# HiKapok/DAN

Hardware: AMD Instinct MI355X
Metric: 640x640 images/sec/node (train fwd+bwd) (higher is better)
Workload: dtype bf16; 1 GPU; S3FD VGG-16 backbone + 6 detection heads, 640x640 bf16 training (fwd+bwd+SGD), batch 16 per GPU; global_batch=16, parallelism=dp1, anchors_per_image=34125, step_launch=eager, rccl_ranks=1, weight_gradient_stream=True

## Files before the change

### dan_amd/_lib.py

```python
import ctypes
import os

import torch

_HERE = os.path.dirname(os.path.abspath(__file__))
ACT_NAME = os.environ.get("DANHIP_DTYPE", "bf16").lower()
if ACT_NAME not in ("bf16", "fp16"):
    raise ValueError("DANHIP_DTYPE must be bf16 or fp16, got %r" % ACT_NAME)
ACT_DTYPE = torch.float16 if ACT_NAME == "fp16" else torch.bfloat16
SO_PATH = os.path.join(_HERE, "libdanhip_f16.so" if ACT_NAME == "fp16" else "libdanhip.so")
if os.environ.get("DANHIP_LIB_PATH"):
    SO_PATH = os.path.abspath(os.environ["DANHIP_LIB_PATH"])

F32, BF16 = 0, 1
SPLIT3 = 3


class ConvDesc(ctypes.Structure):
    _fields_ = [(n, ctypes.c_int32) for n in ("N", "H", "W", "Cin", "Ho", "Wo", "Cout", "kh", "kw", "stride")]


class ConvPitch(ctypes.Structure):
    _fields_ = [(n, ctypes.c_int32) for n in ("x_pitch", "y_pitch", "aux_pitch")]


class PackEntry(ctypes.Structure):
    _fields_ = [("w_hwio", ctypes.c_void_p), ("wf_packed", ctypes.c_void_p), ("wb_packed", ctypes.c_void_p)] + \
               [(n, ctypes.c_int32) for n in ("kh", "kw", "cin", "cin_real", "cout", "rows_f", "cols_f", "rows_b", "cols_b", "co8", "first_block", "pad_")]


class JpegInfo(ctypes.Structure):
    _fields_ = [(n, ctypes.c_int32) for n in ("width", "height", "ncomp", "mode", "reason", "reserved")] + [("coef_count", ctypes.c_int64)]


class JpegDesc(ctypes.Structure):
    _fields_ = [(n, ctypes.c_int32) for n in ("width", "height", "ncomp", "mode")] + \
               [(n, ctypes.c_int32 * 3) for n in ("blocks_w", "blocks_h", "comp_w", "comp_h", "quant_index")] + \
               [(n, ctypes.c_int32) for n in ("status", "idct_groups", "rgb_groups")] + [("reserved", ctypes.c_int32 * 2)] + \
               [("coef_offset", ctypes.c_int64), ("coef_count", ctypes.c_int64), ("plane_offset", ctypes.c_int64 * 3),
                ("out_offset", ctypes.c_int64), ("quant", (ctypes.c_uint16 * 64) * 4)]


P = ctypes.c_void_p
I32 = ctypes.c_int32
I64 = ctypes.c_int64
FL = ctypes.c_float
DESC = ctypes.POINTER(ConvDesc)

SIGNATURES = {
    "danhip_conv_packed_dims": [DESC, ctypes.c_int, ctypes.POINTER(I64), ctypes.POINTER(I64)],
    "danhip_pack_conv_weight": [DESC, P, I32, P, P, P],
    "danhip_conv2d_fwd_pool": [DESC, P, P, P, P, P, P],
    "danhip_pack_entry_init": [ctypes.POINTER(PackEntry), DESC, P, I32, P, P, I32, ctypes.POINTER(ctypes.c_int32)],
    "danhip_pack_conv_weights_batched": [P, I32, I32, P],
    "danhip_conv2d_fwd": [DESC, P, P, P, P, ctypes.c_int, ctypes.c_int, P, P],
    "danhip_conv2d_fwd_ws": [DESC, P, P, P, P, ctypes.c_int, ctypes.c_int, P, P, ctypes.c_size_t, P],
    "danhip_conv2d_fwd_f32": [DESC, P, P, P, P, ctypes.c_int, P, P],
    "danhip_maxpool2x2_fwd_f32": [P, P, I32, I32, I32, I32, P],
    "danhip_split_set_range_flag": [P],
    "danhip_split3_f32": [P, P, I64, I32, I32, ctypes.c_int, I32, P],
    "danhip_unsplit3_f32": [P, P, I64, I32, I32, P],
    "danhip_unsplit3_scaled_f32": [P, P, I64, I32, I32, I32, P],
    "danhip_maxpool2x2_split3": [P, P, I32, I32, I32, I32, P],
    "danhip_l2norm_split3": [P, P, P, I64, I32, I32, I32, P],
    "danhip_conv3x3_c3_f32_split3": [P, P, P, P, I32, I32, I32, I32, ctypes.c_int, I32, P],
    "danhip_conv2d_fwd_split": [DESC, P, P, P, P, ctypes.c_int, ctypes.c_int, I32, P, ctypes.c_size_t, P],
    "danhip_l2norm_fwd_f32": [P, P, P, I64, I32, P],
    "danhip_resize_bilinear_add_fwd_f32": [P, P, P, I32, I32, I32, I32, I32, I32, P],
    "danhip_avgpool2x2s1_same_fwd_f32": [P, P, I32, I32, I32, I32, P],
    "danhip_deform_sample_fwd_f32": [P, P, P, I32, I32, I32, I32, I32, I32, I32, I32, I32, P],
    "danhip_conv2d_bwd_data": [DESC, P, P, P, P, ctypes.c_int, P],
    "danhip_conv2d_bwd_data_ws": [DESC, P, P, P, P, ctypes.c_int, P, ctypes.c_size_t, P],
    "danhip_conv2d_bwd_data_bits": [DESC, P, P, P, P, ctypes.c_int, P],
    "danhip_conv2d_bwd_data_bits_first": [DESC, P, P, P, P, I32, P, P, P],
    "danhip_relu_bits": [P, P, I64, I32, P],
    "danhip_conv2d_fwd_relu_bits": [DESC, P, P, P, P, P, P, P, P],
    "danhip_conv2d_bwd_weight": [DESC, P, P, P, P, I32, P],
    "danhip_conv2d_bwd_weight_ws": [DESC, P, P, P, P, I32, P, ctypes.c_size_t, P],
    "danhip_avgpool2x2s1_same_fwd_strided": [P, I32, P, I32, I32, I32, I32, I32, ctypes.c_int, P],
    "danhip_avgpool2x2s1_same_bwd_strided": [P, I32, P, I32, I32, I32, I32, I32, P],
    "danhip_add16": [P, P, P, I64, P],
    "danhip_residual_bwd": [P, P, P, P, P, ctypes.c_int, I64, P],
    "danhip_conv2d_fwd_strided": [DESC, P, P, P, P, ctypes.c_int, I32, ctypes.POINTER(ConvPitch), P, ctypes.c_size_t, P],
    "danhip_conv2d_bwd_data_strided": [DESC, P, P, P, P, ctypes.c_int, ctypes.POINTER(ConvPitch), P, ctypes.c_size_t, P],
    "danhip_conv2d_fwd_concat2": [DESC, P, P, I32, I32, P, P, P, ctypes.c_int, P],
    "danhip_conv2d_bwd_weight_strided": [DESC, P, P, P, P, I32, ctypes.POINTER(ConvPitch), P, ctypes.c_size_t, P],
    "danhip_relu_bwd_bias_grad": [P, P, P, I64, I32, P],
    "danhip_maxpool2x2_fwd": [P, P, I32, I32, I32, I32, P],
    "danhip_maxpool2x2_fwd_arg": [P, P, P, I32, I32, I32, I32, P],
    "danhip_maxpool2x2_bwd_arg": [P, P, P, I32, I32, I32, I32, ctypes.c_int, P],
    "danhip_conv2d_fwd_pool_arg": [DESC, P, P, P, P, P, P, P],
    "danhip_conv2d_fwd_relu_bits_arg": [DESC, P, P, P, P, P, P, P, P, P],
    "danhip_maxpool2x2_bwd": [P, P, P, I32, I32, I32, I32, ctypes.c_int, P],
    "danhip_l2norm_fwd": [P, P, P, I64, I32, P],
    "danhip_l2norm_bwd": [P, P, P, P, P, I64, I32, ctypes.c_int, ctypes.c_int, P],
    "danhip_l2norm_bwd_pool_scatter": [P, P, P, P, P, P, P, I32, I32, I32, I32, ctypes.c_int, ctypes.c_int, ctypes.c_int, P],
    "danhip_preprocess_u8": [P, P, I64, P],
    "danhip_resize_bilinear_add_fwd": [P, P, P, I32, I32, I32, I32, I32, I32, P],
    "danhip_resize_bilinear_add_bwd": [P, P, I32, I32, I32, I32, I32, I32, ctypes.c_int, P],
    "danhip_avgpool2x2s1_same_fwd": [P, P, I32, I32, I32, I32, P],
    "danhip_avgpool2x2s1_same_bwd": [P, P, P, I32, I32, I32, I32, ctypes.c_int, P],
    "danhip_slice_deliver": [P, I32, I32, I32, P, I32, P, I32, ctypes.c_int, I64, P],
    "danhip_batchnorm_fwd_train": [P, P, P, P, P, P, P, P, I64, I32, FL, FL, ctypes.c_int, P, P],
    "danhip_batchnorm_fwd_infer": [P, P, P, P, P, P, I64, I32, ctypes.c_int, P],
    "danhip_batchnorm_bwd": [P, P, P, P, P, P, P, P, I64, I32, P],
    "danhip_dynamic_anchor_routing_eval": [P, P, P, P, I64, I32, I32, I32, I32, I32, P, P, P, ctypes.c_size_t, P],
    "danhip_dynamic_anchor_routing_train": [P, P, P, P, I64, I32, I32, I32, I32, I32, FL, FL, ctypes.c_uint64, ctypes.c_uint64, P, P, P, P,
                                            ctypes.c_size_t, P],
    "danhip_nms": [P, I32, I32, I32, FL, P, P, P],
    "danhip_argsort_desc_f32": [P, I64, I32, P, P, ctypes.c_size_t, P],
    "danhip_augment_preprocess": [P, I32, I32, I32, ctypes.POINTER(ctypes.c_int32), ctypes.POINTER(ctypes.c_float), I32, I32, I32, I32, I32, P, I32, I32,
                                  P, ctypes.c_size_t, P],
    "danhip_deform_psroi_pool_fwd": [P, P, P, P, P, I32, I32, I32, I32, I32, I32, I32, I32, I32, FL, FL, I32, I32, P],
    "danhip_deform_psroi_pool_bwd": [P, P, P, P, P, P, P, I32, I32, I32, I32, I32, I32, I32, I32, I32, I32, FL, FL, I32, I32, P],
    "danhip_maxpool3x3s2_same_fwd": [P, P, I32, I32, I32, I32, P],
    "danhip_maxpool3x3s2_same_bwd": [P, P, P, I32, I32, I32, I32, P],
    "danhip_resize_u8_linear": [P, I32, I32, P, I32, I32, I32, ctypes.c_double, ctypes.c_double, P],
    "danhip_bbox_vote": [P, P, I32, I32, ctypes.c_double, I32, P, P, P, ctypes.c_size_t, P],
    "danhip_wider_quantize": [P, ctypes.c_int, P, P, I32, I32, I32, P, P, I32, I32, P, P],
    "danhip_wider_score_range": [P, I64, P, P, ctypes.c_size_t, P],
    "danhip_wider_eval": [P, P, I64, P, P, P, I64, P, I32, I32, I32, I32, ctypes.c_double, P, ctypes.c_size_t, P, P],
    "danhip_wider_ap": [P, ctypes.c_size_t, P, I64, I32, I32, I32, P, P, P, P, P, P],
    "danhip_deform_sample_fwd": [P, P, P, I32, I32, I32, I32, I32, I32, I32, I32, I32, P],
    "danhip_deform_sample_bwd": [P, P, P, P, P, I32, I32, I32, I32, I32, I32, I32, I32, I32, ctypes.c_int, P, ctypes.c_size_t, P],
    "danhip_deform_conv_fwd": [P, P, P, P, P, I32, I32, I32, I32, I32, I32, I32, I32, I32, I32, ctypes.c_int, P, ctypes.c_size_t, P],
    "danhip_deform_conv_bwd": [P, P, P, P, P, P, P, P, I32, I32, I32, I32, I32, I32, I32, I32, I32, I32, ctypes.c_int, P, ctypes.c_size_t, P],
    "danhip_deform_conv_bwd_with_col": [P, P, P, P, P, P, P, P, P, I32, I32, I32, I32, I32, I32, I32, I32, I32, I32, ctypes.c_int, P, ctypes.c_size_t, P],
    "danhip_deform_conv_bwd_deliver": [P, P, P, P, P, P, P, P, P, I32, I32, I32, I32, I32, I32, I32, I32, I32, I32, ctypes.c_int, ctypes.c_int, P, ctypes.c_size_t, P],
    "danhip_cast_pad_f32_to_bf16": [P, P, P, I64, I32, I32, P],
    "danhip_head_split_fwd": [P, P, P, I32, I32, I32, I32, I32, I32, I32, P],
    "danhip_head_split_bwd": [P, P, P, P, I32, I32, I32, I32, I32, I32, I32, P],
    "danhip_hard_neg_select": [P, P, P, P, P, P, I32, I32, FL, ctypes.c_int, P],
    "danhip_detection_loss_fwd": [P, P, P, P, P, P, P, P, I32, I32, P],
    "danhip_detection_loss_bwd": [P, P, P, P, P, P, P, FL, FL, I32, I32, P],
    "danhip_sgd_momentum_flat": [P, P, P, P, P, P, I32, I64, FL, FL, FL, P, P],
    "danhip_sgd_momentum_flat_dynamic": [P, P, P, P, P, P, I32, I64, FL, FL, P, P, P],
    "danhip_anchors_generate": [P, P, P, P, P, P, I32, I32, I32, FL, FL, FL, I32, P],
    "danhip_iou_matrix": [P, P, P, P, P, P, P, I32, I32, P],
    "danhip_dual_max_match": [P, I32, I32, FL, FL, ctypes.c_int, P, P, P, ctypes.c_size_t, P],
    "danhip_small_mining_match": [P, I32, I32, FL, FL, FL, I32, FL, P, P, P, ctypes.c_size_t, P],
    "danhip_encode_anchors": [P, P, P, P, P, P, P, P, P, I32, FL, FL, FL, FL, FL, P],
    "danhip_decode_anchors": [P, P, P, P, P, P, I32, I32, FL, FL, FL, FL, P],
    "danhip_face_scores": [P, P, P, FL, I64, P],
    "danhip_comm_load": [ctypes.c_char_p],
    "danhip_comm_rccl_version": [ctypes.POINTER(ctypes.c_int)],
    "danhip_comm_unique_id": [P],
    "danhip_comm_create": [P, I32, I32, I32, ctypes.POINTER(ctypes.c_void_p)],
    "danhip_comm_destroy": [P],
    "danhip_comm_info": [P, ctypes.POINTER(I32), ctypes.POINTER(I32), ctypes.POINTER(I32)],
    "danhip_comm_async_error": [P, ctypes.POINTER(I32)],
    "danhip_comm_abort": [P],
    "danhip_comm_allreduce_sum": [P, P, I64, ctypes.c_int, P],
    "danhip_comm_reduce_scatter_sum": [P, P, P, I64, ctypes.c_int, P],
    "danhip_comm_allgather": [P, P, P, I64, ctypes.c_int, P],
    "danhip_jpeg_entropy_decode_batch": [P, P, I32, I32, P, I64, P, P],
    "danhip_jpeg_entropy_decode_batch_ex": [P, P, I32, I32, ctypes.c_uint32, P, I64, P, P],
    "danhip_jpeg_scan_prepare_batch_ex": [P, P, I32, ctypes.c_uint32, P, ctypes.c_size_t, I64, P, P],
    "danhip_jpeg_reconstruct_batch": [P, I64, P, P, I32, P, I64, P, ctypes.c_size_t, P, P],
    "danhip_jpeg_scan_prepare_batch": [P, P, I32, P, ctypes.c_size_t, I64, P, P],
    "danhip_jpeg_huffman_decode_batch": [P, P, ctypes.c_size_t, I32, P, I64, P, P, P, ctypes.c_size_t, P, P, P],
    "danhip_jpeg_entropy_emulate_batch": [P, ctypes.c_size_t, I32, P, P, I64, I32, P, P],
    "danhip_encode_anchors_batched": [P] * 11 + [I32, I32, I32, I32, I32, FL, FL, FL, I32, FL, FL, FL, FL, FL, FL, P, P, P, P, P,
                                                 ctypes.c_size_t, P],
}

_lib = None


class DanhipError(RuntimeError):
    pass


def lib():
    global _lib
    if _lib is None:
        _lib = _load(SO_PATH, ACT_NAME)
    return _lib


_lib_f16 = None


def lib_f16():
    global _lib_f16
    if _lib_f16 is None:
        _lib_f16 = lib() if ACT_NAME == "fp16" else _load(os.path.join(_HERE, "libdanhip_f16.so"), "fp16")
    return _lib_f16


def call_f16(name, *args):
    L = lib_f16()
    rc = getattr(L, name)(*args)
    if rc != 0:
        raise DanhipError("%s (fp16 build) failed (%d): %s" % (name, rc, L.danhip_last_error().decode()))


def _load(so_path, act_name):
    if True:
        if not os.path.exists(so_path):
            raise DanhipError("libdanhip.so not found at %s — run `python -m dan_amd.build` (there is no fallback path)" % so_path)
        L = ctypes.CDLL(so_path)
        L.danhip_last_error.restype = ctypes.c_char_p
        L.danhip_last_error.argtypes = []
        L.danhip_version.restype = ctypes.c_int
        L.danhip_act_dtype.restype = ctypes.c_int
        if L.danhip_act_dtype() != (2 if act_name == "fp16" else 1):
            raise DanhipError("%s was built for another activation dtype than %s" % (so_path, act_name))
        L.danhip_match_workspace_bytes.restype = ctypes.c_size_t
        L.danhip_conv_kernel_label.restype = ctypes.c_char_p
        L.danhip_conv_kernel_label.argtypes = [DESC, ctypes.c_int]
        L.danhip_conv_wgrad_kernel_label.restype = ctypes.c_char_p
        L.danhip_conv_wgrad_kernel_label.argtypes = [DESC]
        L.danhip_conv_last_launch_label.restype = ctypes.c_char_p
        L.danhip_conv_last_launch_label.argtypes = []
        L.danhip_match_workspace_bytes.argtypes = [I32, I32]
        L.danhip_encode_anchors_batched_workspace_bytes.restype = ctypes.c_size_t
        L.danhip_encode_anchors_batched_workspace_bytes.argtypes = [I32, I32, I32]
        L.danhip_routing_workspace_bytes.restype = ctypes.c_size_t
        L.danhip_routing_workspace_bytes.argtypes = [I64, I32, ctypes.c_int]
        L.danhip_bbox_vote_workspace_bytes.restype = ctypes.c_size_t
        L.danhip_augment_workspace_bytes.restype = ctypes.c_size_t
        L.danhip_argsort_workspace_bytes.argtypes = [I64]
        L.danhip_argsort_workspace_bytes.restype = ctypes.c_size_t
        L.danhip_augment_workspace_bytes.argtypes = []
        L.danhip_set_option.restype = ctypes.c_int
        L.danhip_set_option.argtypes = [ctypes.c_char_p, ctypes.c_int]
        L.danhip_get_option.restype = ctypes.c_int
        L.danhip_get_option.argtypes = [ctypes.c_char_p]
        L.danhip_conv2d_workspace_bytes.restype = ctypes.c_size_t
        L.danhip_conv2d_workspace_bytes.argtypes = [DESC, ctypes.c_int]
        L.danhip_conv2d_bwd_weight_workspace_bytes.restype = ctypes.c_size_t
        L.danhip_conv2d_bwd_weight_workspace_bytes.argtypes = [DESC]
        L.danhip_deform_conv_workspace_bytes.restype = ctypes.c_size_t
        L.danhip_deform_conv_workspace_bytes.argtypes = [I32, I32, I32, I32, I32, I32, I32, ctypes.c_int]
        L.danhip_deform_sample_bwd_workspace_bytes.restype = ctypes.c_size_t
        L.danhip_deform_sample_bwd_workspace_bytes.argtypes = [I32, I32, I32, I32]
        L.danhip_conv2d_fwd_pool_only.restype = ctypes.c_int
        L.danhip_conv2d_fwd_pool_only.argtypes = [DESC]
        L.danhip_conv2d_fwd_concat2_supported.restype = ctypes.c_int
        L.danhip_conv2d_fwd_concat2_supported.argtypes = [DESC, I32, I32]
        L.danhip_conv2d_fwd_emits_bits.restype = ctypes.c_int
        L.danhip_conv2d_fwd_emits_bits.argtypes = [DESC, ctypes.c_int]
        L.danhip_conv2d_bwd_data_takes_bits.restype = ctypes.c_int
        L.danhip_conv2d_bwd_data_takes_bits.argtypes = [DESC]
        L.danhip_conv2d_bwd_data_first_supported.restype = ctypes.c_int
        L.danhip_conv2d_bwd_data_first_supported.argtypes = [DESC]
        L.danhip_deform_conv_fused.restype = ctypes.c_int
        L.danhip_deform_conv_fused.argtypes = [I32] * 9
        L.danhip_bbox_vote_workspace_bytes.argtypes = [I32, I32]
        L.danhip_wider_score_range_workspace_bytes.restype = ctypes.c_size_t
        L.danhip_wider_score_range_workspace_bytes.argtypes = []
        L.danhip_wider_eval_workspace_bytes.restype = ctypes.c_size_t
        L.danhip_wider_eval_workspace_bytes.argtypes = [I32, I32, I32]
        L.danhip_jpeg_inspect.restype = ctypes.c_int
        L.danhip_jpeg_inspect.argtypes = [P, I64, ctypes.POINTER(JpegInfo)]
        L.danhip_jpeg_inspect_ex.restype = ctypes.c_int
        L.danhip_jpeg_inspect_ex.argtypes = [P, I64, ctypes.c_uint32, ctypes.POINTER(JpegInfo)]
        L.danhip_jpeg_workspace_bytes.restype = ctypes.c_size_t
        L.danhip_jpeg_workspace_bytes.argtypes = [P, I32]
        L.danhip_jpeg_output_bytes.restype = I64
        L.danhip_jpeg_output_bytes.argtypes = [P, I32]
        L.danhip_jpeg_scan_staging_bytes.restype = ctypes.c_size_t
        L.danhip_jpeg_scan_staging_bytes.argtypes = [P, P, I32]
        L.danhip_jpeg_scan_device_bytes.restype = ctypes.c_size_t
        L.danhip_jpeg_scan_device_bytes.argtypes = [P]
        L.danhip_jpeg_scan_workspace_bytes.restype = ctypes.c_size_t
        L.danhip_jpeg_scan_workspace_bytes.argtypes = [P]
        for name, args in SIGNATURES.items():
            fn = getattr(L, name)
            fn.restype = ctypes.c_int
            fn.argtypes = args
    return L


def check(rc, what):
    if rc != 0:
        raise DanhipError("%s failed (%d): %s" % (what, rc, lib().danhip_last_error().decode()))


def ptr(t):
    if t is None:
        return None
    assert t.is_contiguous(), "danhip needs contiguous tensors"
    return ctypes.c_void_p(t.data_ptr())


def stream():
    return ctypes.c_void_p(torch.cuda.current_stream().cuda_stream)


def call(name, *args):
    check(getattr(lib(), name)(*args), name)
```

### dan_amd/csrc/conv_common.h

```cpp
#pragma once
#include "common.h"

struct ConvArgs {
  const bf16_t* x;
  const bf16_t* w;
  const float* bias;
  const bf16_t* mask;
  const unsigned char* mask_bits;
  const bf16_t* resid;
  void* y;
  unsigned char* bits_out;
  unsigned char* pool_bits_out;
  bf16_t* pool_y;
  unsigned char* pool_arg_out;
  int N, H, W, C;
  int Ho, Wo, Co;
  int kh, kw, stride, pad_t, pad_l;
  int M, Kpad, ktiles, taps, cpt;
  FastDiv div_wo, div_howo, div_c, div_kw;
  int relu, out_f32, accumulate;
  int dshift;
  float* splitk_ws;
  int splits, kt_per_split;
  int dstride;
  int ldx, ldy, ldm;
  int relu_co;
  bool strided() const { return ldx != C || ldy != Co || (mask && ldm != Co) || (relu && relu_co < Co); }
  const bf16_t* x2;
  int ksplit;
  int split_out;
  const bf16_t* fuse_x8;
  float* fuse_dw;
  float* fuse_db;
  int fuse_cin_real;
  int acc_exp;
  int* range_flag;
};

__device__ __forceinline__ float dh_acc_scale(const ConvArgs& a) { return __builtin_bit_cast(float, (a.acc_exp + 127) << 23); }

template <int N>
__device__ __forceinline__ void dh_range_check(const float* v, int* flag) {
  float m = fabsf(v[0]);
#pragma unroll
  for (int r = 1; r < N; ++r) m = fmaxf(m, fabsf(v[r]));
  if (!(m < 65520.f) && flag) *flag = 1;
}

__device__ __forceinline__ void dh_split4(const float v[4], uint2& hi, uint2& lo) {
  hi.x = pack2bf(v[0], v[1]);
  hi.y = pack2bf(v[2], v[3]);
  float h[4];
  unpack2bf(hi.x, h[0], h[1]);
  unpack2bf(hi.y, h[2], h[3]);
  lo.x = pack2bf(v[0] - h[0], v[1] - h[1]);
  lo.y = pack2bf(v[2] - h[2], v[3] - h[3]);
}

int* danhip_split_range_flag();

typedef __attribute__((ext_vector_type(2))) short s16x2;
__device__ __forceinline__ unsigned pkmax_relu(unsigned a, unsigned b) {
  return __builtin_bit_cast(unsigned, __builtin_elementwise_max(__builtin_bit_cast(s16x2, a), __builtin_bit_cast(s16x2, b)));
}

__device__ __forceinline__ float dh_relu(float v) {
  float r;
  asm("v_max_f32 %0, 0, %1" : "=v"(r) : "v"(v));
  return r;
}
typedef __attribute__((ext_vector_type(2))) unsigned short dh_u16x2;
typedef __attribute__((ext_vector_type(2))) unsigned dh_u32x2;
typedef __attribute__((ext_vector_type(4))) unsigned dh_u32x4;
__device__ __forceinline__ dh_u16x2 dh_pos2(unsigned packed) {
  unsigned r;
  asm("v_pk_min_u16 %0, %1, %2" : "=v"(r) : "v"(packed), "s"(0x00010001u));
  return __builtin_bit_cast(dh_u16x2, r);
}
template <int SHIFT>
__device__ __forceinline__ unsigned dh_pos_bits8_acc(const dh_u32x4& t, unsigned bits) {
  static_assert(SHIFT == 0 || SHIFT == 8, "16-bit weights");
#pragma unroll
  for (int e = 0; e < 4; ++e)
    bits = __builtin_amdgcn_udot2(dh_pos2(t[e]), dh_u16x2{(unsigned short)(1u << (SHIFT + 2 * e)), (unsigned short)(2u << (SHIFT + 2 * e))}, bits, false);
  return bits;
}
__device__ __forceinline__ unsigned dh_pk_ne(unsigned m, unsigned x) {
  unsigned d, r;
  asm("v_pk_sub_u16 %0, %1, %2" : "=v"(d) : "v"(m), "v"(x));
  asm("v_pk_min_u16 %0, %1, %2" : "=v"(r) : "v"(d), "s"(0x00010001u));
  return r;
}
__device__ __forceinline__ unsigned dh_argmax2x2_pk(unsigned a, unsigned b, unsigned c, unsigned m) {
  const unsigned na = dh_pk_ne(m, a), nb = dh_pk_ne(m, b), nc = dh_pk_ne(m, c);
  unsigned t, r;
  asm("v_pk_mad_u16 %0, %1, %2, %1" : "=v"(t) : "v"(nb), "v"(nc));
  asm("v_pk_mad_u16 %0, %1, %2, %1" : "=v"(r) : "v"(na), "v"(t));
  return r;
}
__device__ __forceinline__ unsigned dh_argmax2x2_codes16(const dh_u32x4& a, const dh_u32x4& b, const dh_u32x4& c, const dh_u32x4& m) {
  unsigned out = 0;
#pragma unroll
  for (int e = 0; e < 4; ++e) {
    const unsigned w = dh_argmax2x2_pk(a[e], b[e], c[e], m[e]);
    out |= ((w | (w >> 14)) & 0xFu) << (4 * e);
  }
  return out;
}

__device__ __forceinline__ unsigned dh_or_rows(unsigned x) {
  const dh_u32x2 a = __builtin_amdgcn_permlane16_swap(x, x, false, false);
  const unsigned y = a[0] | a[1];
  const dh_u32x2 b = __builtin_amdgcn_permlane32_swap(y, y, false, false);
  return b[0] | b[1];
}
__device__ __forceinline__ unsigned dh_lane_xor1(unsigned v) { return (unsigned)__builtin_amdgcn_mov_dpp((int)v, 0xB1, 0xF, 0xF, true); }

struct ConvInstance {
  const char* label = nullptr;
  int (*launch)(const ConvArgs&, hipStream_t) = nullptr;
  bool fuses_pool = false;
  bool skips_y = false;
  bool emits_bits = false;
  bool takes_bits = false;
  bool folds_first = false;
  explicit operator bool() const { return launch != nullptr; }
};
ConvInstance conv_c8_select(const ConvArgs& a);
ConvInstance conv_c64_select(const ConvArgs& a);
ConvInstance conv_halo_select(const ConvArgs& a);
ConvInstance conv_pointwise_select(const ConvArgs& a);

struct WgradCall {
  const danhip_conv_desc* d;
  const bf16_t* x;
  const bf16_t* dy;
  float* dw;
  float* db;
  int cin_real, ldx, ldy;
  void* ws;
  size_t ws_bytes;
};
struct WgradInstance {
  const char* label = nullptr;
  int (*launch)(const WgradCall&, hipStream_t) = nullptr;
  explicit operator bool() const { return launch != nullptr; }
};
WgradInstance wgrad_rows_select(const WgradCall& c);
WgradInstance wgrad_pw_select(const WgradCall& c);
WgradInstance wgrad_c8_select(const WgradCall& c);
size_t wgrad_rows_workspace_bytes(const danhip_conv_desc* d);
size_t wgrad_pw_workspace_bytes(const danhip_conv_desc* d);

inline const char*& dh_last_launch_label() {
  static thread_local const char* label = "";
  return label;
}
template <class Instance, class Args>
int dh_run_instance(const Instance& inst, const Args& a, hipStream_t s) {
  if (!inst) return 1;
  dh_last_launch_label() = inst.label;
  return inst.launch(a, s);
}

__device__ __forceinline__ void conv_store4(const ConvArgs& a, float v[4], size_t m, int co) {
  if (co >= a.Co) return;
  const size_t o = m * (size_t)(a.split_out ? 3 * a.ldy : a.ldy) + co;
  const size_t om = m * (size_t)a.ldm + co;
  const size_t orr = m * (size_t)a.Co + co;
  const bool full = (co + 4 <= a.Co) && ((a.Co & 3) == 0);
  if (a.bias) {
    const float sc = dh_acc_scale(a);
#pragma unroll
    for (int r = 0; r < 4; ++r) if (co + r < a.Co) v[r] = fmaf(v[r], sc, a.bias[co + r]);
  } else if (a.acc_exp) {
#pragma unroll
    for (int r = 0; r < 4; ++r) v[r] *= dh_acc_scale(a);
  }
  if (a.relu && co < a.relu_co) {
#pragma unroll
    for (int r = 0; r < 4; ++r) v[r] = fmaxf(v[r], 0.f);
  }
  if (a.out_f32) {
    float* y = reinterpret_cast<float*>(a.y) + o;
    if (full) {
      float4 t = make_float4(v[0], v[1], v[2], v[3]);
      if (a.accumulate) { float4 u = *reinterpret_cast<float4*>(y); t.x += u.x; t.y += u.y; t.z += u.z; t.w += u.w; }
      *reinterpret_cast<float4*>(y) = t;
    } else {
#pragma unroll
      for (int r = 0; r < 4; ++r) if (co + r < a.Co) y[r] = a.accumulate ? y[r] + v[r] : v[r];
    }
  } else {
    bf16_t* y = reinterpret_cast<bf16_t*>(a.y) + o;
    if (a.split_out) {
      dh_range_check<4>(v, a.range_flag);
      uint2 hi, lo;
      dh_split4(v, hi, lo);
      *reinterpret_cast<uint2*>(y) = hi;
      *reinterpret_cast<uint2*>(y + a.Co) = lo;
      *reinterpret_cast<uint2*>(y + 2 * a.Co) = hi;
      return;
    }
    if (full) {
      if (a.mask) {
        const uint2 mk = *reinterpret_cast<const uint2*>(a.mask + om);
        const bf16_t* mp = reinterpret_cast<const bf16_t*>(&mk);
#pragma unroll
        for (int r = 0; r < 4; ++r) if (!(bf2f(mp[r]) > 0.f)) v[r] = 0.f;
      }
      if (a.resid) {
        const uint2 rs = *reinterpret_cast<const uint2*>(a.resid + orr);
        const bf16_t* rp = reinterpret_cast<const bf16_t*>(&rs);
#pragma unroll
        for (int r = 0; r < 4; ++r) v[r] += bf2f(rp[r]);
      }
      if (a.accumulate) {
        const uint2 old = *reinterpret_cast<const uint2*>(y);
        const bf16_t* op = reinterpret_cast<const bf16_t*>(&old);
#pragma unroll
        for (int r = 0; r < 4; ++r) v[r] += bf2f(op[r]);
      }
      uint2 t;
      t.x = pack2bf(v[0], v[1]);
// ... 17 lines not shown
```

### dan_amd/csrc/conv_halo_c64.hip

```cpp
#include <type_traits>

#include "conv_common.h"

namespace {

struct C64Geom {
  int tiles_x, tiles_y, sp_items;
  FastDiv div_tx, div_txy;
};

template <int N>
__device__ __forceinline__ void c64_wait_vmcnt() {
  asm volatile("s_waitcnt vmcnt(%0)" ::"n"(N) : "memory");
}

template <bool DGRAD, bool FUSE8 = false>
__global__ __launch_bounds__(512, 2) __attribute__((amdgpu_waves_per_eu(2, 2))) void conv3x3_c64_kernel(const ConvArgs a, const C64Geom g) {
  static_assert(DGRAD || !FUSE8, "the folded first-layer weight gradient belongs to the data gradient");
  constexpr int TH = 8, TW = 32, PW = TW + 2;
  constexpr int PROWS = (TH + 2) * PW, PPIECES = (PROWS + 7) / 8, PBYTES = PPIECES * 1024, PL = (PPIECES + 7) / 8;
  constexpr int NPT = 4, NCT = 2;
  extern __shared__ __attribute__((aligned(16))) char smem[];

  const int tid = threadIdx.x, lane = tid & 63;
  const int wave = __builtin_amdgcn_readfirstlane(tid >> 6);
  const int wm = wave >> 1, wn = wave & 1;
  const int frow = lane & 15, fq = lane >> 4;
  const int G = gridDim.x;

  bf16x8 wr[9][2][NCT];
#pragma unroll
  for (int t = 0; t < 9; ++t)
#pragma unroll
    for (int ks = 0; ks < 2; ++ks)
#pragma unroll
      for (int ct = 0; ct < NCT; ++ct)
        wr[t][ks][ct] = *reinterpret_cast<const bf16x8*>(a.w + (size_t)(wn * 32 + (frow >> 2) * 8 + ct * 4 + (frow & 3)) * a.Kpad + t * 64 + ks * 32 + fq * 8);

  auto sp_coords = [&](int sp, int& n, int& y0, int& x0) __attribute__((always_inline)) {
    n = (int)fdiv((unsigned)sp, g.div_txy);
    const int rem = sp - n * (g.tiles_x * g.tiles_y);
    const int ty = (int)fdiv((unsigned)rem, g.div_tx);
    y0 = ty * TH;
    x0 = (rem - ty * g.tiles_x) * TW;
  };

  const unsigned npix1 = (unsigned)(a.N * a.H * a.W) - 1u;
  const unsigned px_x = (unsigned)a.ldx * 2u, px_y = (unsigned)a.ldy * 2u, px_m = (unsigned)a.ldm * 2u;
  const __amdgpu_buffer_rsrc_t rsrc_x = __builtin_amdgcn_make_buffer_rsrc(const_cast<bf16_t*>(a.x), 0, (int)(npix1 * px_x + 128u), 0x00020000);
  auto issue_patch = [&](int sp, int buf) __attribute__((always_inline)) {
    int n, y0, x0;
    sp_coords(sp, n, y0, x0);
    int ln = lane;
    asm volatile("" : "+v"(ln));
#pragma unroll
    for (int k = 0; k < PL; ++k) {
      int piece = k * 8 + wave;
      if (piece > PPIECES - 1) piece = PPIECES - 1;
      const int row = piece * 8 + (ln >> 3);
      const int hy = row / PW, hx = row - hy * PW;
      const int y = y0 - 1 + hy, x = x0 - 1 + hx;
      const bool ok = row < PROWS && (unsigned)y < (unsigned)a.H && (unsigned)x < (unsigned)a.W;
      const unsigned off = ok ? (unsigned)((n * a.H + y) * a.W + x) * px_x + (unsigned)(((ln & 7) ^ (hx & 7)) << 4) : 0xFFFFFFFFu;
      __builtin_amdgcn_raw_ptr_buffer_load_lds(rsrc_x, (LDS_AS void*)(smem + buf * PBYTES + piece * 1024), 16, off, 0, 0, 0);
    }
  };

  constexpr int RWBASE = 2 * PBYTES;
  [[maybe_unused]] const __amdgpu_buffer_rsrc_t rsrc_m =
      __builtin_amdgcn_make_buffer_rsrc(const_cast<bf16_t*>(a.mask ? a.mask : a.x), 0, (int)(npix1 * (a.mask ? px_m : px_x) + 128u), 0x00020000);
  [[maybe_unused]] const __amdgpu_buffer_rsrc_t rsrc_o =
      __builtin_amdgcn_make_buffer_rsrc(reinterpret_cast<bf16_t*>(a.y), 0, (int)(npix1 * px_y + 128u), 0x00020000);
  [[maybe_unused]] const __amdgpu_buffer_rsrc_t rsrc_b = __builtin_amdgcn_make_buffer_rsrc(
      const_cast<unsigned char*>(a.mask_bits ? a.mask_bits : reinterpret_cast<const unsigned char*>(a.x)), 0, (int)((unsigned)(a.N * a.H * a.W) * 8u),
      0x00020000);
  auto issue_bits = [&](int sp, int bbuf) __attribute__((always_inline)) {
    if (wave >= 2) return;
    int n, y0, x0;
    sp_coords(sp, n, y0, x0);
    int ln = lane;
    if constexpr (FUSE8) asm volatile("" : "+v"(ln));
    const int t = (wave * 64 + ln) * 2;
    const int y = y0 + t / TW, x = x0 + t % TW;
    const unsigned off = (y < a.H && x < a.W) ? (unsigned)((n * a.H + y) * a.W + x) * 8u : 0xFFFFFFFFu;
    __builtin_amdgcn_raw_ptr_buffer_load_lds(rsrc_b, (LDS_AS void*)(smem + RWBASE + bbuf * 2048 + wave * 1024), 16, off, 0, 0, 0);
  };
  constexpr int IMGBASE = RWBASE + 4096, IMGBYTES = 6144, DXBASE = RWBASE + 16384, C1BASE = RWBASE + 49152, FACCBASE = RWBASE + 49216;
  [[maybe_unused]] const __amdgpu_buffer_rsrc_t rsrc_i = __builtin_amdgcn_make_buffer_rsrc(
      const_cast<bf16_t*>(FUSE8 ? a.fuse_x8 : a.x), 0, (int)((unsigned)(a.N * a.H * a.W) * 16u), 0x00020000);
  [[maybe_unused]] auto issue_img = [&](int sp, int ibuf) __attribute__((always_inline)) {
    if (wave >= 6) return;
    int n, y0, x0;
    sp_coords(sp, n, y0, x0);
    int ln = lane;
    asm volatile("" : "+v"(ln));
    const int e = wave * 64 + ln;
    const int r = e / PW, c = e - r * PW;
    const int y = y0 - 1 + r, x = x0 - 1 + c;
    const bool ok = e < PROWS && (unsigned)y < (unsigned)a.H && (unsigned)x < (unsigned)a.W;
    __builtin_amdgcn_raw_ptr_buffer_load_lds(rsrc_i, (LDS_AS void*)(smem + IMGBASE + ibuf * IMGBYTES + wave * 1024), 16,
                                             ok ? (unsigned)((n * a.H + y) * a.W + x) * 16u : 0xFFFFFFFFu, 0, 0, 0);
  };
  auto issue_rw = [&](int sp) __attribute__((always_inline)) {
    int n, y0, x0;
    sp_coords(sp, n, y0, x0);
    int ln = lane;
    asm volatile("" : "+v"(ln));
#pragma unroll
    for (int k = 0; k < NPT; ++k) {
      const int t = wm * 64 + k * 16 + (ln >> 2);
      const int y = y0 + t / TW, x = x0 + t % TW;
      const bool ok = y < a.H && x < a.W;
      const unsigned pix = (unsigned)((n * a.H + y) * a.W + x), ch = (unsigned)((wn * 4 + (ln & 3)) << 4);
      if (a.mask)
        __builtin_amdgcn_raw_ptr_buffer_load_lds(rsrc_m, (LDS_AS void*)(smem + RWBASE + wave * 4096 + k * 1024), 16, ok ? pix * px_m + ch : 0xFFFFFFFFu, 0, 0, 0);
      if (a.accumulate)
        __builtin_amdgcn_raw_ptr_buffer_load_lds(rsrc_o, (LDS_AS void*)(smem + RWBASE + 32768 + wave * 4096 + k * 1024), 16, ok ? pix * px_y + ch : 0xFFFFFFFFu,
                                                 0, 0, 0);
    }
  };
  const int rwaddr = RWBASE + wave * 4096 + ((frow * 4 + fq) << 4);

  int pxaddr[3][NPT];
#pragma unroll
  for (int p = 0; p < NPT; ++p) {
    const int t = wm * 64 + p * 16 + frow;
    const int ty = t / TW, tx = t % TW;
#pragma unroll
    for (int j = 0; j < 3; ++j) pxaddr[j][p] = (ty * PW + tx + j) * 128 + ((fq ^ ((tx + j) & 7)) << 4);
  }

  f32x4 acc[NCT][NPT];
#pragma unroll
  for (int c = 0; c < NCT; ++c)
#pragma unroll
    for (int p = 0; p < NPT; ++p) acc[c][p] = f32x4{0.f, 0.f, 0.f, 0.f};

  [[maybe_unused]] const int faddr = FACCBASE + (wave * 3 * 64 + lane) * 16;
  if constexpr (FUSE8) {
#pragma unroll
    for (int mt = 0; mt < 3; ++mt) *reinterpret_cast<f32x4*>(smem + faddr + mt * 1024) = f32x4{0.f, 0.f, 0.f, 0.f};
    if (tid < 16) reinterpret_cast<bf16_t*>(smem + C1BASE)[tid] = tid == 0 ? f2bf(1.0f) : (bf16_t)0;
  }

  bf16x8 xa[NPT], xb[NPT], xc[NPT];
  auto read_px = [&](bf16x8 (&x)[NPT], auto tapc, int ks) __attribute__((always_inline)) {
    constexpr int TAP = decltype(tapc)::value;
    constexpr int TI = TAP / 3, TJ = TAP % 3;
#pragma unroll
    for (int p = 0; p < NPT; ++p) x[p] = *reinterpret_cast<const bf16x8*>(smem + (ks ? (pxaddr[TJ][p] ^ 64) : pxaddr[TJ][p]) + TI * PW * 128);
  };
  auto mma = [&](const bf16x8 (&w)[NCT], const bf16x8 (&x)[NPT]) __attribute__((always_inline)) {
#pragma unroll
    for (int c = 0; c < NCT; ++c)
#pragma unroll
      for (int p = 0; p < NPT; ++p) acc[c][p] = DH_MFMA_16x16x32(w[c], x[p], acc[c][p]);
  };

  const bool xcd_walk = (G & 7) == 0;
  const int GS = xcd_walk ? (G >> 3) : G;
  const int per_xcd = (g.sp_items + 7) >> 3;
  const int xbase = xcd_walk ? (int)(blockIdx.x & 7u) * per_xcd : 0;
  const int xend = xcd_walk ? (xbase + per_xcd < g.sp_items ? xbase + per_xcd : g.sp_items) : g.sp_items;
  int sp = xcd_walk ? xbase + (int)(blockIdx.x >> 3) : (int)blockIdx.x;
  if (sp >= xend) return;
  issue_patch(sp, 0);
  if constexpr (!DGRAD) {
    if (tid < 64) reinterpret_cast<float*>(smem + RWBASE)[tid] = a.bias ? a.bias[tid] : 0.f;
    __builtin_amdgcn_s_waitcnt(0xC07F);
  }
  c64_wait_vmcnt<0>();
  __builtin_amdgcn_s_barrier();
  int buf = 0;
  for (;;) {
    const int nsp = sp + GS;
    const bool has_next = nsp < xend;
    if constexpr (DGRAD) {
      issue_rw(sp);
      if (a.mask_bits) issue_bits(sp, buf);
      if constexpr (FUSE8) issue_img(sp, buf);
    }
    if (has_next) issue_patch(nsp, buf ^ 1);
    auto rd = [&](bf16x8 (&x)[NPT], auto hc) __attribute__((always_inline)) {
      constexpr int H = decltype(hc)::value;
      read_px(x, std::integral_constant<int, H / 2>{}, H & 1);
    };
    auto half = [&](auto hc, bf16x8 (&cur)[NPT], bf16x8 (&)[NPT]) __attribute__((always_inline)) {
      constexpr int H = decltype(hc)::value;
      mma(wr[H / 2][H & 1], cur);
      if constexpr (H + 3 < 18) rd(cur, std::integral_constant<int, H + 3>{});
    };
    rd(xa, std::integral_constant<int, 0>{});
    rd(xb, std::integral_constant<int, 1>{});
    rd(xc, std::integral_constant<int, 2>{});
#define C64_H(H, X) half(std::integral_constant<int, H>{}, X, X)
    C64_H(0, xa); C64_H(1, xb); C64_H(2, xc); C64_H(3, xa); C64_H(4, xb); C64_H(5, xc);
    C64_H(6, xa); C64_H(7, xb); C64_H(8, xc); C64_H(9, xa); C64_H(10, xb); C64_H(11, xc);
    C64_H(12, xa); C64_H(13, xb); C64_H(14, xc); C64_H(15, xa); C64_H(16, xb); C64_H(17, xc);
#undef C64_H
    c64_wait_vmcnt<0>();
    __builtin_amdgcn_s_barrier();
    {
      int n, y0, x0;
      sp_coords(sp, n, y0, x0);
      static_assert(NCT == 2, "epilogue packs the two channel tiles of a lane into one 16-byte vector");
      const int cbase = wn * 32 + fq * 8;
      float bv[8];
#pragma unroll
      for (int r = 0; r < 8; ++r) bv[r] = DGRAD ? 0.f : reinterpret_cast<const float*>(smem + RWBASE)[cbase + r];
      typedef __attribute__((ext_vector_type(4))) unsigned u32x4;
      u32x4 pk[NPT];
#pragma unroll
      for (int p = 0; p < NPT; ++p) pk[p] = u32x4{0u, 0u, 0u, 0u};
      if constexpr (DGRAD) {
        if (a.mask_bits) {
          unsigned w4[NPT];
#pragma unroll
          for (int p = 0; p < NPT; ++p) w4[p] = *reinterpret_cast<const unsigned*>(smem + RWBASE + buf * 2048 + (wm * 64 + p * 16 + frow) * 8 + wn * 4);
#pragma unroll
          for (int p = 0; p < NPT; ++p) {
            const int byte = (int)(w4[p] >> (8 * fq));
#pragma unroll
            for (int r = 0; r < 8; ++r) {
              const float v = acc[r >> 2][p][r & 3];
              acc[r >> 2][p][r & 3] = __builtin_bit_cast(float, __builtin_bit_cast(int, v) & __builtin_amdgcn_sbfe(byte, r, 1));
            }
          }
        }
        if (a.mask) {
          uint4 m[NPT];
#pragma unroll
          for (int p = 0; p < NPT; ++p) m[p] = *reinterpret_cast<const uint4*>(smem + rwaddr + p * 1024);
#pragma unroll
          for (int p = 0; p < NPT; ++p) {
            const bf16_t* mp = reinterpret_cast<const bf16_t*>(&m[p]);
#pragma unroll
            for (int r = 0; r < 8; ++r) if (!(bf2f(mp[r]) > 0.f)) acc[r >> 2][p][r & 3] = 0.f;
          }
        }
        if (a.accumulate) {
          uint4 o[NPT];
#pragma unroll
          for (int p = 0; p < NPT; ++p) o[p] = *reinterpret_cast<const uint4*>(smem + rwaddr + 32768 + p * 1024);
#pragma unroll
          for (int p = 0; p < NPT; ++p) {
            const bf16_t* op = reinterpret_cast<const bf16_t*>(&o[p]);
#pragma unroll
            for (int r = 0; r < 8; ++r) acc[r >> 2][p][r & 3] += bf2f(op[r]);
          }
        }
        __builtin_amdgcn_sched_barrier(0);
      }
#pragma unroll
      for (int p = 0; p < NPT; ++p) {
        const int t = wm * 64 + p * 16 + frow;
        const int y = y0 + t / TW, x = x0 + t % TW;
        const bool ok = y < a.H && x < a.W;
        const size_t o0 = (size_t)((n * a.H + y) * a.W + x) * (size_t)a.ldy + cbase;
        if (ok) {
          float v[8] = {acc[0][p][0], acc[0][p][1], acc[0][p][2], acc[0][p][3], acc[1][p][0], acc[1][p][1], acc[1][p][2], acc[1][p][3]};
          if (!DGRAD) {
#pragma unroll
            for (int r = 0; r < 8; ++r) v[r] += bv[r];
            if (a.relu) {
#pragma unroll
              for (int r = 0; r < 8; ++r) v[r] = dh_relu(v[r]);
            }
            if (a.resid) {
              const uint4 in = *reinterpret_cast<const uint4*>(a.resid + o0);
              const bf16_t* rp = reinterpret_cast<const bf16_t*>(&in);
#pragma unroll
              for (int r = 0; r < 8; ++r) v[r] += bf2f(rp[r]);
            }
          } else {
          }
          const u32x4 tt = {pack2bf(v[0], v[1]), pack2bf(v[2], v[3]), pack2bf(v[4], v[5]), pack2bf(v[6], v[7])};
          if (a.y)
            __builtin_nontemporal_store(tt, reinterpret_cast<u32x4*>(reinterpret_cast<bf16_t*>(a.y) + o0));
          pk[p] = tt;
        }
        if constexpr (FUSE8) {
          const int fz = (t & 7) ^ (((t >> 3) & 1) << 2);
          *reinterpret_cast<u32x4*>(smem + DXBASE + t * 128 + (((cbase >> 3) ^ fz) << 4)) = pk[p];
// ... 20 lines not shown
#pragma unroll
          for (int h = 0; h < 2; ++h) {
#pragma unroll
            for (int mt = 0; mt < 3; ++mt) {
              const int tap = mt * 4 + pp;
              const int ti = tap / 3, tj = tap - ti * 3;
              const char* ad = tap < 9 ? im + ((row + ti) * PW + 8 * gg + qq + tj + 4 * h) * 16 : smem + C1BASE + (tap == 9 ? 0 : 8);
              xh[rr][h][mt] = __builtin_amdgcn_ds_read_tr16_b64_v4i16((LDS_AS s16x4*)ad);
            }
            const int pix = row * 32 + ypix + 4 * h;
            const int fz = (pix & 7) ^ (((pix >> 3) & 1) << 2);
            yh[rr][h] = __builtin_amdgcn_ds_read_tr16_b64_v4i16((LDS_AS s16x4*)(smem + DXBASE + pix * 128 + (((2 * nt + (pp >> 1)) ^ fz) << 4) + (pp & 1) * 8));
          }
        }
#pragma unroll
        for (int rr = 0; rr < 4; ++rr) {
          const bf16x8 yf = __builtin_bit_cast(bf16x8, __builtin_shufflevector(yh[rr][0], yh[rr][1], 0, 1, 2, 3, 4, 5, 6, 7));
#pragma unroll
          for (int mt = 0; mt < 3; ++mt) {
            const bf16x8 xf = __builtin_bit_cast(bf16x8, __builtin_shufflevector(xh[rr][0][mt], xh[rr][1][mt], 0, 1, 2, 3, 4, 5, 6, 7));
            facc[mt] = DH_MFMA_16x16x32(xf, yf, facc[mt]);
          }
        }
#pragma unroll
        for (int mt = 0; mt < 3; ++mt) *reinterpret_cast<f32x4*>(smem + faddr + mt * 1024) = facc[mt];
      }
      if (!DGRAD && a.pool_y) {
        const int Hp = (a.H + 1) >> 1, Wp = (a.W + 1) >> 1;
#pragma unroll
        for (int p = 0; p < 2; ++p) {
          const int t = wm * 64 + p * 16 + frow;
          const int y = y0 + t / TW, x = x0 + t % TW;
          u32x4 m;
#pragma unroll
          for (int e = 0; e < 4; ++e) {
            const unsigned v = pkmax_relu(pk[p][e], pk[p + 2][e]);
            m[e] = pkmax_relu(v, dh_lane_xor1(v));
          }
          if (y < a.H && x < a.W && (frow & 1) == 0)
            *reinterpret_cast<u32x4*>(a.pool_y + ((size_t)((n * Hp + (y >> 1)) * Wp + (x >> 1))) * 64 + cbase) = m;
          if (a.pool_arg_out) {
            u32x4 tr;
#pragma unroll
            for (int e = 0; e < 4; ++e) tr[e] = dh_lane_xor1(pk[p][e]);
            const unsigned codes = dh_argmax2x2_codes16(pk[p], tr, pk[p + 2], m);
            if (y < a.H && x < a.W && (frow & 1) == 0)
              *reinterpret_cast<unsigned short*>(a.pool_arg_out + ((size_t)((n * Hp + (y >> 1)) * Wp + (x >> 1))) * 16 + cbase / 4) = (unsigned short)codes;
          }
        }
      }
    }
    if (!has_next) break;
    sp = nsp;
    buf ^= 1;
    const int dir = buf ? PBYTES : -PBYTES;
#pragma unroll
    for (int j = 0; j < 3; ++j)
#pragma unroll
      for (int p = 0; p < NPT; ++p) pxaddr[j][p] += dir;
  }
  if constexpr (FUSE8) {
    f32x4 facc[3];
#pragma unroll
    for (int mt = 0; mt < 3; ++mt) facc[mt] = *reinterpret_cast<const f32x4*>(smem + faddr + mt * 1024);
    __builtin_amdgcn_s_waitcnt(0xC07F);
    __builtin_amdgcn_s_barrier();
    float* red = reinterpret_cast<float*>(smem);
    for (int i = tid; i < 12 * 4 * 64; i += 512) red[i] = 0.f;
    __syncthreads();
    const int gg = lane >> 4;
#pragma unroll
    for (int mt = 0; mt < 3; ++mt)
#pragma unroll
      for (int r = 0; r < 4; ++r) atomicAdd(&red[((mt * 4 + gg) * 4 + r) * 64 + (wave & 3) * 16 + (lane & 15)], facc[mt][r]);
    __syncthreads();
    for (int i = tid; i < 9 * 4 * 64; i += 512) {
      const int co = i & 63, c = (i >> 6) & 3, slot = i >> 8;
      if (c < a.fuse_cin_real) atomicAdd(a.fuse_dw + (size_t)(slot * a.fuse_cin_real + c) * 64 + co, red[i]);
    }
    if (a.fuse_db && tid < 64) atomicAdd(a.fuse_db + tid, red[(9 * 4 + 0) * 64 + tid]);
  }
}

bool c64_eligible(const ConvArgs& a) {
  if (!(a.kh == 3 && a.kw == 3 && a.stride == 1 && a.dstride == 1 && a.pad_t == 1 && a.pad_l == 1)) return false;
  if (a.H != a.Ho || a.W != a.Wo || a.C != 64 || a.Co != 64 || a.out_f32 || a.Kpad != 576) return false;
  if (a.relu && a.relu_co < a.Co) return false;
  if (a.strided() && (a.resid || a.pool_y || a.mask_bits || a.bits_out)) return false;
  const int ldmax = a.ldx > a.ldy ? (a.ldx > a.ldm ? a.ldx : a.ldm) : (a.ldy > a.ldm ? a.ldy : a.ldm);
  if ((a.ldx | a.ldy | a.ldm) & 7) return false;
  const double util = (double)a.H * a.W / ((double)((a.H + 7) / 8 * 8) * (double)((a.W + 31) / 32 * 32));
  return util >= 0.78 && (int64_t)a.N * a.H * a.W * ldmax * 2 < (1ll << 32);
}

template <bool DGRAD, bool FUSE8 = false>
int launch_c64(const ConvArgs& a, hipStream_t s) {
  constexpr int LDS = 2 * ((10 * 34 + 7) / 8) * 1024 + (FUSE8 ? 75776 : (DGRAD ? 65536 : 256));
  static_assert(LDS <= 160 * 1024, "LDS budget");
  static const bool attr_ok =
      hipFuncSetAttribute(reinterpret_cast<const void*>(&conv3x3_c64_kernel<DGRAD, FUSE8>), hipFuncAttributeMaxDynamicSharedMemorySize, LDS) == hipSuccess;
  (void)attr_ok;
  C64Geom g{};
  g.tiles_x = (a.W + 31) / 32;
  g.tiles_y = (a.H + 7) / 8;
  g.sp_items = a.N * g.tiles_x * g.tiles_y;
  g.div_tx = make_fastdiv(g.tiles_x);
  g.div_txy = make_fastdiv(g.tiles_x * g.tiles_y);
  int G = dh_cu_count();
  if (g.sp_items < G) G = g.sp_items;
  hipLaunchKernelGGL((conv3x3_c64_kernel<DGRAD, FUSE8>), dim3(G), dim3(512), LDS, s, a, g);
  DH_LAUNCH_CHECK();
  return DANHIP_OK;
}

template <bool DGRAD, bool FUSE8 = false>
ConvInstance c64_instance(const char* label) {
  ConvInstance i;
  i.label = label;
  i.launch = &launch_c64<DGRAD, FUSE8>;
  return i;
}

}

ConvInstance conv_c64_select(const ConvArgs& a) {
  if (!c64_eligible(a)) return {};
  const bool dgrad = !a.bias && !a.relu && !a.resid;
  if (!dgrad && (a.accumulate || a.mask || a.mask_bits)) return {};
  if (a.mask && a.mask_bits) return {};
  ConvInstance i;
  if (a.fuse_dw) {
    if (!dgrad || !a.mask_bits || a.accumulate || a.strided() || !a.fuse_x8 || a.fuse_cin_real < 1 || a.fuse_cin_real > 4) return {};
    i = c64_instance<true, true>("conv3x3_c64_kernel<true, true>");
    i.folds_first = a.W % 2 == 0 && (int64_t)a.N * a.H * a.W * 16 < (1ll << 31);
  } else {
    i = dgrad ? c64_instance<true>("conv3x3_c64_kernel<true>") : c64_instance<false>("conv3x3_c64_kernel<false>");
  }
  i.takes_bits = dgrad && a.W % 2 == 0;
  i.fuses_pool = i.skips_y = !dgrad && a.pool_y && a.bias && a.relu && !a.resid;
  return i;
}
```

### dan_amd/csrc/conv_igemm.hip

```cpp
#include <cstdlib>

#include "conv_common.h"

namespace {


template <int BM, int BN, int WN_WAVES, bool FAST>
__global__ __launch_bounds__(256, 2) void conv_igemm_kernel(const ConvArgs a) {
  constexpr int RA = BM / 32;
  constexpr int RB = (BN + 31) / 32;
  constexpr int STAGE = (BM + BN) * 128;
  constexpr int WM_WAVES = 4 / WN_WAVES;
  constexpr int TP = BM / WM_WAVES;
  constexpr int TC = BN / WN_WAVES;
  constexpr int NPT = TP / 16, NCT = TC / 16;
  static_assert(TP % 16 == 0 && TC % 16 == 0, "wave tile must be MFMA-tile aligned");

  extern __shared__ __attribute__((aligned(16))) char smem[];

  const int tid = threadIdx.x;
  const int lane = tid & 63;
  const int wave = __builtin_amdgcn_readfirstlane(tid >> 6);
  const int wm = wave / WN_WAVES, wn = wave % WN_WAVES;

// ... 303 lines not shown
  if (co % 64 == 0) return 64;
  if (co <= 16) return 16;
  if (co <= 32) return 32;
  return 64;
}

inline int igemm_bm(const ConvArgs& a) {
  const int bn = pick_bn(a.Co);
  if (bn == 128) return 128;
  if (bn == 16) return a.M <= 256 * 128 ? 64 : 256;
  return 256;
}

int plan_splitk(const ConvArgs& a, int* kt_per_split) {
  *kt_per_split = a.ktiles;
  if (!danhip_option("splitk") || a.pool_y || a.bits_out || a.mask_bits) return 1;
  const int bm = igemm_bm(a), bn = pick_bn(a.Co);
  const long tiles = (long)cdiv(a.M, bm) * cdiv(a.Co, bn);
  const int cus = dh_cu_count();
  const long target = (bn == 16 ? 8l : 2l) * cus;
  if (tiles * 2 > target || a.ktiles < 8) return 1;
  int splits = (int)((target + tiles - 1) / tiles);
  if (splits > a.ktiles / 4) splits = a.ktiles / 4;
  if (splits > 36) splits = 36;
  if (splits < 2) return 1;
  const int per = (a.ktiles + splits - 1) / splits;
  *kt_per_split = per;
  return (a.ktiles + per - 1) / per;
}

bool wants_splitk(const ConvArgs& a) {
  int per;
  if (plan_splitk(a, &per) < 2) return false;
  return (long)cdiv(a.M, 128) * cdiv(a.Co, 128) * 2 <= dh_cu_count();
}
bool prefer_splitk(const ConvArgs& a) { return a.splitk_ws && wants_splitk(a); }

template <int BM, int BN, int WN_WAVES>
int launch_cfg(const ConvArgs& a0, hipStream_t s) {
  ConvArgs a = a0;
  const bool fast = (a.C % 64 == 0);
  int per = a.ktiles;
  const int splits = a.splitk_ws ? plan_splitk(a, &per) : 1;
  if (splits < 2) a.splitk_ws = nullptr;
  a.splits = splits; a.kt_per_split = per;
  dim3 grid((unsigned)cdiv(a.M, BM), (unsigned)cdiv(a.Co, BN), (unsigned)splits);
  const size_t lds = 2 * (size_t)(BM + BN) * 128;
  static const bool attr_ok =
      hipFuncSetAttribute(reinterpret_cast<const void*>(&conv_igemm_kernel<BM, BN, WN_WAVES, true>), hipFuncAttributeMaxDynamicSharedMemorySize,
                          (int)(2 * (BM + BN) * 128)) == hipSuccess &&
      hipFuncSetAttribute(reinterpret_cast<const void*>(&conv_igemm_kernel<BM, BN, WN_WAVES, false>), hipFuncAttributeMaxDynamicSharedMemorySize,
                          (int)(2 * (BM + BN) * 128)) == hipSuccess;
  (void)attr_ok;
  if (fast)
    hipLaunchKernelGGL((conv_igemm_kernel<BM, BN, WN_WAVES, true>), grid, dim3(256), lds, s, a);
  else
    hipLaunchKernelGGL((conv_igemm_kernel<BM, BN, WN_WAVES, false>), grid, dim3(256), lds, s, a);
  DH_LAUNCH_CHECK();
  if (a.splitk_ws) {
    const long threads = (long)a.M * ((a.Co + 3) / 4);
    hipLaunchKernelGGL(conv_splitk_finish_kernel, dim3((unsigned)((threads + 255) / 256)), dim3(256), 0, s, a);
    DH_LAUNCH_CHECK();
  }
  return DANHIP_OK;
}

template <int BM, int BN, int WN_WAVES>
ConvInstance flat_instance(const ConvArgs& a, const char* fast_label, const char* slow_label) {
  ConvInstance i;
  i.label = a.C % 64 == 0 ? fast_label : slow_label;
  i.launch = &launch_cfg<BM, BN, WN_WAVES>;
  return i;
}

int launch_direct_dgrad(const ConvArgs& a, hipStream_t s);

ConvInstance select_conv(const ConvArgs& a) {
  if (a.dstride & (a.dstride - 1)) {
    ConvInstance i;
    i.label = "conv_bwd_data_strided_kernel";
    i.launch = &launch_direct_dgrad;
    return i;
  }
  const bool view = a.strided();
  const bool limbs = a.split_out != 0;
  if (!view && !limbs)
    if (ConvInstance i = conv_c8_select(a)) return i;
  if (!limbs)
    if (ConvInstance i = conv_c64_select(a)) return i;
  if (!prefer_splitk(a)) {
    if (!view)
      if (ConvInstance i = conv_halo_select(a)) return i;
    if (!limbs)
      if (ConvInstance i = conv_pointwise_select(a)) return i;
  }
  switch (pick_bn(a.Co)) {
    case 128: return flat_instance<128, 128, 2>(a, "conv_igemm_kernel<128, 128, 2, true>", "conv_igemm_kernel<128, 128, 2, false>");
    case 64: return flat_instance<256, 64, 1>(a, "conv_igemm_kernel<256, 64, 1, true>", "conv_igemm_kernel<256, 64, 1, false>");
    case 32: return flat_instance<256, 32, 1>(a, "conv_igemm_kernel<256, 32, 1, true>", "conv_igemm_kernel<256, 32, 1, false>");
    default:
      if (a.M <= 256 * 128) return flat_instance<64, 16, 1>(a, "conv_igemm_kernel<64, 16, 1, true>", "conv_igemm_kernel<64, 16, 1, false>");
      return flat_instance<256, 16, 1>(a, "conv_igemm_kernel<256, 16, 1, true>", "conv_igemm_kernel<256, 16, 1, false>");
  }
}

int launch_conv(const ConvArgs& a, hipStream_t s) { return dh_run_instance(select_conv(a), a, s); }

inline int same_pad_before(int in, int out, int k, int s) {
  int total = (out - 1) * s + k - in;
  if (total < 0) total = 0;
  return total / 2;
}

int check_desc(const danhip_conv_desc* d) {
  DH_REQUIRE(d != nullptr, DANHIP_EINVAL, "conv: null descriptor");
  DH_REQUIRE(d->N > 0 && d->H > 0 && d->W > 0 && d->Cin > 0 && d->Cout > 0, DANHIP_EINVAL, "conv: non-positive dims");
  DH_REQUIRE(d->Cin % 8 == 0, DANHIP_EINVAL, "conv: Cin=%d must be a multiple of 8 (pad the activation)", d->Cin);
  DH_REQUIRE(d->kh >= 1 && d->kh <= 7 && d->kw >= 1 && d->kw <= 7, DANHIP_EINVAL, "conv: kernel %dx%d unsupported", d->kh, d->kw);
  DH_REQUIRE(d->stride >= 1 && d->stride <= 4, DANHIP_EINVAL, "conv: stride %d unsupported", d->stride);
  {
    const bool same = d->Ho == (d->H + d->stride - 1) / d->stride && d->Wo == (d->W + d->stride - 1) / d->stride;
    const bool valid = d->H >= d->kh && d->W >= d->kw && d->Ho == (d->H - d->kh) / d->stride + 1 && d->Wo == (d->W - d->kw) / d->stride + 1;
    DH_REQUIRE(same || valid, DANHIP_EINVAL, "conv: Ho/Wo (%d,%d) is neither the 'same' nor the 'valid' output size", d->Ho, d->Wo);
  }
  DH_REQUIRE((int64_t)d->N * d->H * d->W * d->Cin < (1ll << 31) && (int64_t)d->N * d->Ho * d->Wo * (int64_t)((d->Cout + 7) / 8 * 8) < (1ll << 31),
             DANHIP_EINVAL, "conv: tensor exceeds 2^31 elements");
  return DANHIP_OK;
}

inline int round_up(int v, int m) { return (v + m - 1) / m * m; }

}

extern "C" int danhip_conv_packed_dims(const danhip_conv_desc* d, int which, int64_t* rows, int64_t* cols) {
  int rc = check_desc(d);
  if (rc) return rc;
  DH_REQUIRE(rows && cols, DANHIP_EINVAL, "conv_packed_dims: null output");
  const int taps = d->kh * d->kw;
  if (which == 0) {
    *rows = round_up(d->Cout, pick_bn(d->Cout));
    *cols = round_up(taps * d->Cin, 64);
  } else {
    const int co8 = round_up(d->Cout, 8);
    *rows = round_up(d->Cin, pick_bn(d->Cin));
    *cols = round_up(taps * co8, 64);
  }
  return DANHIP_OK;
}

namespace {
__device__ __forceinline__ void pack_entry_block(const danhip_pack_entry& e, int lb, int nb, float (*tile)[33]) {
  const float* __restrict__ w = e.w_hwio;
  const int taps = e.kh * e.kw;
  const int tid = threadIdx.x;
  if (lb < e.pad_) {
    bf16_t* __restrict__ wf = e.wf_packed;
    const int ctiles = (e.rows_f + 31) / 32;
    const int tco = lb % ctiles, tk = lb / ctiles;
    const int co0 = tco * 32, k0 = tk * 64;
    const int tx = tid & 31, ty = tid >> 5;
#pragma unroll
    for (int r = 0; r < 8; ++r) {
      const int kl = ty + 8 * r, k = k0 + kl;
      const int tap = k / e.cin, c = k - tap * e.cin;
      float v = 0.f;
      if (co0 + tx < e.cout && tap < taps && c < e.cin_real) v = w[((long)tap * e.cin_real + c) * e.cout + co0 + tx];
// ... 379 lines not shown
        const int wo = wn / stride;
        if (wo >= Wo) continue;
        const bf16_t* g = dy + ((long)(n * Ho + ho) * Wo + wo) * co8;
        const int tapf = (kh - 1 - i) * kw + (kw - 1 - j);
        for (int co = 0; co < co8; ++co) {
          const float gv = bf2f(g[co]);
#pragma unroll
          for (int r = 0; r < 8; ++r) acc[r] += gv * bf2f(wb[(long)(cg * 8 + r) * kpad_b + tapf * co8 + co]);
        }
      }
    }
    const long o = ((long)(n * H + hi) * W + wi) * Cin + cg * 8;
#pragma unroll
    for (int r = 0; r < 8; ++r) {
      float v = acc[r];
      if (mask && !(bf2f(mask[o + r]) > 0.f)) v = 0.f;
      if (accumulate) v += bf2f(dx[o + r]);
      dx[o + r] = f2bf(v);
    }
  }
}

int launch_direct_dgrad(const ConvArgs& a, hipStream_t s) {
  const long total = (long)a.N * a.Ho * a.Wo * (a.Co / 8);
  int blocks = (int)((total + 255) / 256);
  if (blocks > 8192) blocks = 8192;
  hipLaunchKernelGGL(conv_bwd_data_strided_kernel, dim3(blocks), dim3(256), 0, s, a.x, a.w, a.mask, reinterpret_cast<bf16_t*>(a.y), a.N, a.Ho, a.Wo, a.Co,
                     a.H, a.W, a.C, a.kh, a.kw, a.dstride, a.kh - 1 - a.pad_t, a.kw - 1 - a.pad_l, a.Kpad, a.accumulate);
  DH_LAUNCH_CHECK();
  return DANHIP_OK;
}
}

extern "C" int danhip_conv2d_bwd_data(const danhip_conv_desc* d, const uint16_t* dy, const uint16_t* wb_packed, const uint16_t* relu_mask,
                                      uint16_t* dx, int accumulate, void* stream) {
  return danhip_conv2d_bwd_data_ws(d, dy, wb_packed, relu_mask, dx, accumulate, nullptr, 0, stream);
}

extern "C" int danhip_conv2d_bwd_data_ws(const danhip_conv_desc* d, const uint16_t* dy, const uint16_t* wb_packed, const uint16_t* relu_mask,
                                         uint16_t* dx, int accumulate, void* ws, size_t ws_bytes, void* stream) {
  int rc = check_desc(d);
  if (rc) return rc;
  DH_REQUIRE(dy && wb_packed && dx, DANHIP_EINVAL, "conv2d_bwd_data: null pointer");
  ConvArgs a = bwd_args(d);
  a.x = dy; a.w = wb_packed; a.bias = nullptr; a.mask = relu_mask; a.resid = nullptr; a.y = dx;
  a.relu = 0; a.out_f32 = 0; a.accumulate = accumulate;
  if (ws && ws_bytes >= danhip_conv2d_workspace_bytes(d, 1) && ws_bytes > 0) a.splitk_ws = reinterpret_cast<float*>(ws);
  return launch_conv(a, (hipStream_t)stream);
}

extern "C" int danhip_conv2d_bwd_data_takes_bits(const danhip_conv_desc* d) {
  if (!d || check_desc(d) != DANHIP_OK) return 0;
  if (d->stride != 1) return 0;
  ConvArgs a = bwd_args(d);
  a.mask_bits = &g_rep_bits;
  return select_conv(a).takes_bits ? 1 : 0;
}

extern "C" int danhip_conv2d_bwd_data_first_supported(const danhip_conv_desc* d) {
  if (!d || check_desc(d) != DANHIP_OK || d->stride != 1) return 0;
  ConvArgs a = bwd_args(d);
  a.mask_bits = &g_rep_bits;
  a.fuse_x8 = &g_rep_act; a.fuse_dw = &g_rep_f32; a.fuse_cin_real = 3;
  return select_conv(a).folds_first ? 1 : 0;
}

extern "C" int danhip_conv2d_bwd_data_bits_first(const danhip_conv_desc* d, const uint16_t* dy, const uint16_t* wb_packed, const uint8_t* relu_bits,
                                                 const uint16_t* x8, int32_t cin_real, float* dw8, float* db8, void* stream) {
  int rc = check_desc(d);
  if (rc) return rc;
  DH_REQUIRE(dy && wb_packed && relu_bits && x8 && dw8, DANHIP_EINVAL, "conv2d_bwd_data_bits_first: null pointer");
  DH_REQUIRE(cin_real >= 1 && cin_real <= 4, DANHIP_EINVAL, "conv2d_bwd_data_bits_first: cin_real = %d (1..4 real channels of the 8-channel image)", cin_real);
  DH_REQUIRE(danhip_conv2d_bwd_data_first_supported(d), DANHIP_EINVAL, "conv2d_bwd_data_bits_first: not the 64 -> 64 3x3 shape the folded kernel takes "
             "(ask danhip_conv2d_bwd_data_first_supported first)");
  ConvArgs a = bwd_args(d);
  a.x = dy; a.w = wb_packed; a.bias = nullptr; a.mask = nullptr; a.mask_bits = relu_bits; a.resid = nullptr; a.y = nullptr;
  a.relu = 0; a.out_f32 = 0; a.accumulate = 0;
  a.fuse_x8 = x8; a.fuse_dw = dw8; a.fuse_db = db8; a.fuse_cin_real = cin_real;
  rc = dh_run_instance(conv_c64_select(a), a, (hipStream_t)stream);
  DH_REQUIRE(rc <= 0, DANHIP_EINVAL, "conv2d_bwd_data_bits_first: the folded kernel declined the call");
  return rc;
}

extern "C" int danhip_conv2d_bwd_data_bits(const danhip_conv_desc* d, const uint16_t* dy, const uint16_t* wb_packed, const uint8_t* relu_bits,
                                           uint16_t* dx, int accumulate, void* stream) {
  int rc = check_desc(d);
  if (rc) return rc;
  DH_REQUIRE(dy && wb_packed && dx && relu_bits, DANHIP_EINVAL, "conv2d_bwd_data_bits: null pointer");
  DH_REQUIRE(danhip_conv2d_bwd_data_takes_bits(d), DANHIP_EINVAL, "conv2d_bwd_data_bits: the data-gradient kernel of this shape takes the 16-bit mask "
             "(ask danhip_conv2d_bwd_data_takes_bits first)");
  ConvArgs a = bwd_args(d);
  a.x = dy; a.w = wb_packed; a.bias = nullptr; a.mask = nullptr; a.mask_bits = relu_bits; a.resid = nullptr; a.y = dx;
  a.relu = 0; a.out_f32 = 0; a.accumulate = accumulate;
  const ConvInstance c64 = conv_c64_select(a);
  return dh_run_instance(c64 ? c64 : conv_halo_select(a), a, (hipStream_t)stream);
}
```

### dan_amd/csrc/conv_wgrad.hip

```cpp
#include <cstdlib>

#include "conv_common.h"

namespace {

struct WgradArgs {
  const bf16_t* x;
  const bf16_t* dy;
  float* dw;
  float* db;
  int N, H, W, C, Ho, Wo, Co8, Cout, cin_real;
  int ldx, ldy;
  int kh, kw, stride, pad_t, pad_l;
  int M, ktiles, kt_per_split;
  int linear;
  int ci_tiles;
  int tapcols;
  FastDiv div_wo, div_howo;
};

template <int RB>
__device__ __forceinline__ int swz(int pix) {
  if (RB == 256) return ((pix & 3) | (((pix >> 3) & 1) << 2)) << 1;
  if (RB == 128) return (((pix >> 1) & 1) | (((pix >> 3) & 1) << 1)) << 1;
// ... 133 lines not shown
      if (do_bias) {
#pragma unroll
        for (int o = 0; o < NO; ++o) accb[o] = DH_MFMA_16x16x32(ones, yf[o], accb[o]);
      }
    }
  }
  if (do_bias && g == 0) {
#pragma unroll
    for (int o = 0; o < NO; ++o) {
      const int co = co0 + wco * TCO + o * 16 + (lane & 15);
      if (co < a.Cout) atomicAdd(a.db + co, accb[o][0]);
    }
  }

#pragma unroll
  for (int i = 0; i < NI; ++i) {
#pragma unroll
    for (int r = 0; r < 4; ++r) {
      const int cil = wci * TCI + i * 16 + g * 4 + r;
      int t = tap, ci = ci0 + cil;
      if (a.tapcols) { t = cil / 8; ci = cil % 8; if (t >= a.kh * a.kw) continue; }
      if (ci >= a.cin_real) continue;
#pragma unroll
      for (int o = 0; o < NO; ++o) {
        const int co = co0 + wco * TCO + o * 16 + (lane & 15);
        if (co < a.Cout) atomicAdd(a.dw + ((size_t)(t * a.cin_real + ci) * a.Cout + co), acc[i][o][r]);
      }
    }
  }
}

bool wgrad_tapcols(const WgradCall& c) {
  return c.d->Cin == 8 && c.d->kh * c.d->kw <= 16 && c.ldx == c.d->Cin && c.ldy == (c.d->Cout + 7) / 8 * 8;
}

template <int BCI, int BCO, int WCI_WAVES>
int launch_wgrad(const WgradCall& c, hipStream_t s) {
  const danhip_conv_desc* d = c.d;
  WgradArgs a{};
  a.x = c.x; a.dy = c.dy; a.dw = c.dw; a.db = c.db;
  a.N = d->N; a.H = d->H; a.W = d->W; a.C = d->Cin; a.Ho = d->Ho; a.Wo = d->Wo; a.Cout = d->Cout; a.Co8 = (d->Cout + 7) / 8 * 8;
  a.ldx = c.ldx; a.ldy = c.ldy;
  a.cin_real = c.cin_real;
  a.kh = d->kh; a.kw = d->kw; a.stride = d->stride;
  int total = (d->Ho - 1) * d->stride + d->kh - d->H; if (total < 0) total = 0; a.pad_t = total / 2;
  total = (d->Wo - 1) * d->stride + d->kw - d->W; if (total < 0) total = 0; a.pad_l = total / 2;
  a.M = d->N * d->Ho * d->Wo;
  a.ktiles = (a.M + 63) / 64;
  a.div_wo = make_fastdiv(a.Wo); a.div_howo = make_fastdiv(a.Ho * a.Wo);
  a.tapcols = wgrad_tapcols(c) ? 1 : 0;
  a.linear = !a.tapcols && d->kh == 1 && d->kw == 1 && d->stride == 1 && d->Ho == d->H && d->Wo == d->W;
  static const bool attr_ok = (hipFuncSetAttribute(reinterpret_cast<const void*>(&conv_wgrad_kernel<BCI, BCO, WCI_WAVES>),
                                                   hipFuncAttributeMaxDynamicSharedMemorySize, 2 * 64 * (BCI + BCO) * 2) == hipSuccess);
  (void)attr_ok;
  const int co_tiles = cdiv(a.Co8, BCO);
  a.ci_tiles = a.tapcols ? 1 : cdiv(a.C, BCI);
  const int taps = a.tapcols ? 1 : a.kh * a.kw;
  const int base_blocks = co_tiles * a.ci_tiles * taps;
  const int lds_block = 2 * 64 * (BCI + BCO) * 2;
  int per_cu = (160 * 1024) / lds_block;
  if (per_cu > 4) per_cu = 4;
  const int slots = per_cu * dh_cu_count();
  int splits = slots / base_blocks;
  const int max_splits = (a.ktiles + 7) / 8;
  if (splits > max_splits) splits = max_splits;
  if (splits < 1) splits = 1;
  a.kt_per_split = (a.ktiles + splits - 1) / splits;
  splits = (a.ktiles + a.kt_per_split - 1) / a.kt_per_split;
  dim3 grid((unsigned)(co_tiles * a.ci_tiles), (unsigned)taps, (unsigned)splits);
  hipLaunchKernelGGL((conv_wgrad_kernel<BCI, BCO, WCI_WAVES>), grid, dim3(256), 2 * 64 * (BCI + BCO) * 2, s, a);
  DH_LAUNCH_CHECK();
  return DANHIP_OK;
}

template <int BCI, int BCO, int WCI_WAVES>
WgradInstance wgrad_instance(const char* label) {
  WgradInstance i;
  i.label = label;
  i.launch = &launch_wgrad<BCI, BCO, WCI_WAVES>;
  return i;
}

WgradInstance select_wgrad(const WgradCall& c) {
  if (WgradInstance i = wgrad_rows_select(c)) return i;
  if (WgradInstance i = wgrad_pw_select(c)) return i;
  if (WgradInstance i = wgrad_c8_select(c)) return i;
  const int co8 = (c.d->Cout + 7) / 8 * 8;
  const bool ci_wide = c.d->Cin > 64 || wgrad_tapcols(c), co_wide = co8 > 64;
  if (ci_wide && co_wide) return wgrad_instance<128, 128, 2>("conv_wgrad_kernel<128, 128, 2>");
  if (ci_wide) return wgrad_instance<128, 64, 2>("conv_wgrad_kernel<128, 64, 2>");
  if (!co_wide) return wgrad_instance<64, 64, 2>("conv_wgrad_kernel<64, 64, 2>");
  return wgrad_instance<64, 128, 2>("conv_wgrad_kernel<64, 128, 2>");
}

}

extern "C" const char* danhip_conv_wgrad_kernel_label(const danhip_conv_desc* d) {
  if (!d) return "";
  const WgradCall c{d, nullptr, nullptr, nullptr, nullptr, 3, d->Cin, (d->Cout + 7) / 8 * 8, nullptr, 0};
  return select_wgrad(c).label;
}

extern "C" size_t danhip_conv2d_bwd_weight_workspace_bytes(const danhip_conv_desc* d) {
  if (!d) return 0;
  if (!danhip_option("wgrad_slab")) return 0;
  const size_t r = wgrad_rows_workspace_bytes(d);
  return r ? r : wgrad_pw_workspace_bytes(d);
}

static int bwd_weight_impl(const danhip_conv_desc* d, const uint16_t* x, const uint16_t* dy, float* dw_hwio, float* db, int32_t cin_real, int ldx, int ldy,
                           void* ws, size_t ws_bytes, void* stream) {
  DH_REQUIRE(d && x && dy && dw_hwio, DANHIP_EINVAL, "conv2d_bwd_weight: null pointer");
  DH_REQUIRE(d->Cin % 8 == 0, DANHIP_EINVAL, "conv2d_bwd_weight: Cin=%d must be a multiple of 8", d->Cin);
  DH_REQUIRE(cin_real > 0 && cin_real <= d->Cin, DANHIP_EINVAL, "conv2d_bwd_weight: cin_real out of range");
  const int co8 = (d->Cout + 7) / 8 * 8;
  DH_REQUIRE(ldx >= d->Cin && ldy >= co8 && ((ldx | ldy) & 7) == 0, DANHIP_EINVAL, "conv2d_bwd_weight: pitches must be multiples of 8 and cover the channels");
  DH_REQUIRE((int64_t)d->N * d->H * d->W * ldx < (1ll << 31) && (int64_t)d->N * d->Ho * d->Wo * (int64_t)ldy < (1ll << 31),
             DANHIP_EINVAL, "conv2d_bwd_weight: tensor exceeds 2^31 elements (4 GiB): split the batch");
  {
    const bool same = d->Ho == (d->H + d->stride - 1) / d->stride && d->Wo == (d->W + d->stride - 1) / d->stride;
    const bool valid = d->H >= d->kh && d->W >= d->kw && d->Ho == (d->H - d->kh) / d->stride + 1 && d->Wo == (d->W - d->kw) / d->stride + 1;
    DH_REQUIRE(same || valid, DANHIP_EINVAL, "conv: Ho/Wo (%d,%d) is neither the 'same' nor the 'valid' output size", d->Ho, d->Wo);
  }
  const WgradCall c{d, x, dy, dw_hwio, db, cin_real, ldx, ldy, ws, ws_bytes};
  return dh_run_instance(select_wgrad(c), c, (hipStream_t)stream);
}

extern "C" int danhip_conv2d_bwd_weight(const danhip_conv_desc* d, const uint16_t* x, const uint16_t* dy, float* dw_hwio, float* db,
                                        int32_t cin_real, void* stream) {
  return danhip_conv2d_bwd_weight_ws(d, x, dy, dw_hwio, db, cin_real, nullptr, 0, stream);
}

extern "C" int danhip_conv2d_bwd_weight_ws(const danhip_conv_desc* d, const uint16_t* x, const uint16_t* dy, float* dw_hwio, float* db,
                                           int32_t cin_real, void* ws, size_t ws_bytes, void* stream) {
  DH_REQUIRE(d != nullptr, DANHIP_EINVAL, "conv2d_bwd_weight: null pointer");
  return bwd_weight_impl(d, x, dy, dw_hwio, db, cin_real, d->Cin, (d->Cout + 7) / 8 * 8, ws, ws_bytes, stream);
}

extern "C" int danhip_conv2d_bwd_weight_strided(const danhip_conv_desc* d, const uint16_t* x, const uint16_t* dy, float* dw_hwio, float* db,
                                                int32_t cin_real, const danhip_conv_pitch* pitch, void* ws, size_t ws_bytes, void* stream) {
  DH_REQUIRE(d != nullptr && pitch != nullptr, DANHIP_EINVAL, "conv2d_bwd_weight_strided: null pointer");
  return bwd_weight_impl(d, x, dy, dw_hwio, db, cin_real, pitch->x_pitch, pitch->y_pitch, ws, ws_bytes, stream);
}
```

### dan_amd/csrc/conv_wgrad_rows.hip

```cpp
#include <cstdlib>
#include <type_traits>

#include "conv_common.h"

namespace {

struct WgRowsArgs {
  const bf16_t* x;
  const bf16_t* dy;
  float* dw;
  float* db;
  int N, H, W, C, Co8, Cout, cin_real;
  int ldx, ldy;
  int tiles_x, total_rows, rows_per_split;
  int ci_tiles, co_tiles, xcd_grouped;
  int ablate;
  int b2;
  float* slab;
  int splits;
  FastDiv div_tx, div_h, div_ci, div_pairs;
#ifdef WR_TRACE
  unsigned* trace;
#endif
#ifdef WR_CLOCK
  unsigned long long* clk;
#endif
};

#ifdef WR_CLOCK
#define WR_CLK(slot)                                                                                                   \
  do {                                                                                                                 \
    if (tid == 0) {                                                                                                    \
      a.clk[(size_t)blockIdx.x * 8 + 2 * (slot)] = __builtin_amdgcn_s_memtime();                                       \
      a.clk[(size_t)blockIdx.x * 8 + 2 * (slot) + 1] = __builtin_amdgcn_s_memrealtime();                               \
    }                                                                                                                  \
  } while (0)
#else
#define WR_CLK(slot) do { } while (0)
#endif

#ifdef WR_TRACE
#define WR_STAMP(slot)                                                                                              \
  do {                                                                                                              \
    if (blockIdx.x == 0 && (wave & 3) == 0 && tr_step < 128) {                                                       \
      const unsigned t_ = (unsigned)__builtin_readcyclecounter();                                                   \
      const unsigned sa_ = (unsigned)(XBASE + DEPTH * XS + (((wave >> 2) * 128 + tr_step) * 4 + (slot)) * 4);       \
      unsigned va_, vd_;                                                                                            \
      asm volatile("v_mov_b32 %0, %2\n\tv_mov_b32 %1, %3\n\tds_write_b32 %0, %1" : "=&v"(va_), "=&v"(vd_) : "s"(sa_), "s"(t_) : "memory"); \
    }                                                                                                               \
  } while (0)
#define WR_STEP_DONE() (++tr_step)
#else
#define WR_STAMP(slot) do { } while (0)
#define WR_STEP_DONE() do { } while (0)
#endif

template <int N>
__device__ __forceinline__ void wr_wait_vmcnt() {
  asm volatile("s_waitcnt vmcnt(%0)" ::"n"(N) : "memory");
}
typedef __attribute__((ext_vector_type(4))) unsigned wr_u32x4;
__device__ __forceinline__ void wr_dma16(wr_u32x4 rsrc, unsigned voff, unsigned lds_addr) {
  unsigned keep;
  asm volatile("s_mov_b32 %0, m0\n\ts_mov_b32 m0, %3\n\ts_nop 0\n\tbuffer_load_dwordx4 %1, %2, 0 offen lds\n\ts_mov_b32 m0, %0"
               : "=&s"(keep) : "v"(voff), "s"(rsrc), "s"(lds_addr) : "memory");
}
__device__ __forceinline__ wr_u32x4 wr_make_rsrc(const void* p, unsigned bytes) {
  const unsigned long long a = (unsigned long long)p;
  return wr_u32x4{(unsigned)a, (unsigned)(a >> 32) & 0xFFFFu, bytes, 0x00020000u};
}
__device__ __forceinline__ int wr_f128(int pc) { return ((pc >> 1) & 1) | (((pc >> 3) & 1) << 1); }
__device__ __forceinline__ int wr_f256(int px) { return (px & 3) | (((px >> 3) & 1) << 2); }

struct RowGen {
  int strip, n, x0, y, warm, left;
};
struct RowStep {
  int n, x0, xrow, yrow;
  bool xvalid, yvalid;
};

template <int COT>
__global__ __launch_bounds__(512, 2) __attribute__((amdgpu_waves_per_eu(2, 2))) void conv_wgrad_rows_kernel(const WgRowsArgs a) {
  constexpr int TW = 32;
  constexpr int PITCH = 40;
  constexpr int XS = PITCH * 128;
  constexpr int RBY = COT * 2;
  constexpr int YS = TW * RBY;
  constexpr int DEPTH = 6;
  constexpr int P = 4;
  constexpr int YBASE = 0, XBASE = DEPTH * YS;
  constexpr int NO = COT / 32;
  constexpr int YPIECES = YS / 1024;
  static_assert(XBASE + DEPTH * XS <= 160 * 1024, "LDS budget");

  extern __shared__ __attribute__((aligned(16))) char smem[];
  const int tid = threadIdx.x, lane = tid & 63;
  const int wave = __builtin_amdgcn_readfirstlane(tid >> 6);
  const int wci = wave & 3;
  const int grp = wave >> 2;
  const int wco = grp;
  WR_CLK(0);

  const int pairs = a.ci_tiles * a.co_tiles;
  int split, pair;
  if (a.xcd_grouped) {
    const int xcd = blockIdx.x & 7, slot = blockIdx.x >> 3;
    const int sq = (int)fdiv((unsigned)slot, a.div_pairs);
    pair = slot - sq * pairs;
    split = sq * 8 + xcd;
  } else {
    split = (int)fdiv(blockIdx.x, a.div_pairs);
    pair = (int)blockIdx.x - split * pairs;
  }
  const int co_tile = (int)fdiv((unsigned)pair, a.div_ci);
  const int ci_tile = pair - co_tile * a.ci_tiles;
  const int ci0 = ci_tile * 64, co0 = co_tile * COT;
  const int k_begin = split * a.rows_per_split;
  const int k_end = min(a.total_rows, k_begin + a.rows_per_split);
  if (k_begin >= k_end) return;
  const int strip_first = (int)fdiv((unsigned)k_begin, a.div_h), strip_last = (int)fdiv((unsigned)(k_end - 1), a.div_h);
  const int steps = (k_end - k_begin) + 2 * (strip_last - strip_first + 1);
  const int V = (steps + DEPTH - 1) / DEPTH * DEPTH;

  const wr_u32x4 rsrc_x = wr_make_rsrc(a.x, ((unsigned)(a.N * a.H * a.W - 1) * (unsigned)a.ldx + (unsigned)a.C) * 2u);
  const wr_u32x4 rsrc_y = wr_make_rsrc(a.dy, ((unsigned)(a.N * a.H * a.W - 1) * (unsigned)a.ldy + (unsigned)a.Co8) * 2u);
  const unsigned lds0 = __builtin_amdgcn_readfirstlane((unsigned)(size_t)(LDS_AS char*)smem);

  RowGen gen;
  auto gen_strip = [&](RowGen& g) __attribute__((always_inline)) {
    g.n = (int)fdiv((unsigned)g.strip, a.div_tx);
    g.x0 = (g.strip - g.n * a.tiles_x) * TW;
  };
  gen.strip = strip_first;
  gen.y = k_begin - strip_first * a.H;
  gen.warm = 2;
  gen.left = k_end - k_begin;
  gen_strip(gen);
  unsigned long long flags = 0;
  auto gen_next = [&](RowStep& s, int bit) __attribute__((always_inline)) {
    s.n = gen.n; s.x0 = gen.x0;
    if (gen.left == 0) {
      s.xvalid = false; s.yvalid = false; s.xrow = 0; s.yrow = 0;
    } else if (gen.warm > 0) {
      s.xrow = gen.y - gen.warm + 1; s.xvalid = true; s.yvalid = false; s.yrow = 0;
      gen.warm -= 1;
    } else {
      s.xrow = gen.y + 1; s.yrow = gen.y; s.xvalid = true; s.yvalid = true;
      flags |= 1ull << bit;
      gen.y += 1; gen.left -= 1;
      if (gen.y == a.H) { gen.strip += 1; gen.y = 0; gen.warm = 2; gen_strip(gen); }
    }
  };

  const int pc5 = wave < 4 ? wave : 4;
  constexpr int CPP = RBY / 16;
  constexpr int PXP = 1024 / RBY;
  const int ypiece = wave & (YPIECES - 1);
  const int l8 = lane >> 3, lp = lane / CPP;
  unsigned vx, vy;
  {
    const int xA = (lane & 7) ^ (((l8 >> 1) & 1) << 1);
    const int chunk = xA ^ ((pc5 & 1) << 2);
    vx = __umul24((unsigned)l8, (unsigned)(a.ldx * 2)) + (unsigned)(chunk << 4);
    const int cpos = lane % CPP, pxb = ypiece * PXP;
    const int yB = COT == 128 ? (cpos ^ (lp << 1)) : (cpos ^ (((lp >> 1) & 1) << 1));
    const int sb = (pxb >> 3) & 1;
    const int ychunk = yB ^ (COT == 128 ? (sb << 3) : (sb << 2));
    vy = __umul24((unsigned)lp, (unsigned)(a.ldy * 2)) + (unsigned)(ychunk << 4);
    if (!(co0 + ychunk * 8 < a.Co8)) vy = 0xFFFFFFFFu;
  }
  unsigned vxbad = 0, vybad = 0;
  int dma_x0 = -1;
  auto dma_step = [&](auto slc, const RowStep& s) __attribute__((always_inline)) {
    constexpr int SL = decltype(slc)::value;
    if (s.x0 != dma_x0) {
      dma_x0 = s.x0;
      const int x = s.x0 - 1 + pc5 * 8 + l8;
      vxbad = (l8 < (pc5 == 4 ? 2 : 8) && (unsigned)x < (unsigned)a.W) ? 0u : 0xFFFFFFFFu;
      vybad = (s.x0 + ypiece * PXP + lp < a.W) ? 0u : 0xFFFFFFFFu;
    }
    {
      const int xs = s.x0 - 1 + pc5 * 8;
      const unsigned bady = (s.xvalid && (unsigned)s.xrow < (unsigned)a.H) ? 0u : 0xFFFFFFFFu;
      const unsigned sbase = (unsigned)(((s.n * a.H + s.xrow) * a.W + xs) * a.ldx + ci0) * 2u;
      const unsigned voff = (vx + sbase) | vxbad | bady;
      wr_dma16(rsrc_x, voff, lds0 + XBASE + SL * XS + pc5 * 1024);
    }
    {
      const int xs = s.x0 + ypiece * PXP;
      const unsigned bady = (s.yvalid && (unsigned)s.yrow < (unsigned)a.H) ? 0u : 0xFFFFFFFFu;
      const unsigned sbase = (unsigned)(((s.n * a.H + s.yrow) * a.W + xs) * a.ldy + co0) * 2u;
      const unsigned voff = (vy + sbase) | vybad | bady;
      wr_dma16(rsrc_y, voff, lds0 + YBASE + SL * YS + ypiece * 1024);
    }
  };

  const int g = lane >> 4, q = (lane & 15) >> 2, p = lane & 3;
  int xaddr[3][2];
#pragma unroll
  for (int j = 0; j < 3; ++j)
#pragma unroll
    for (int h = 0; h < 2; ++h) {
      const int pcol = j + 8 * g + 4 * h + q;
      const int ch = (wci * 2 + (p >> 1)) ^ (wr_f128(pcol) << 1);
      xaddr[j][h] = XBASE + pcol * 128 + (ch << 4) + (p & 1) * 8;
    }
  int yaddr[NO];
#pragma unroll
  for (int o = 0; o < NO; ++o) {
    const int px = 8 * g + q;
    const int ch = ((wco * NO + o) * 2 + (p >> 1)) ^ ((COT == 128 ? wr_f256(px) : wr_f128(px)) << 1);
    yaddr[o] = YBASE + px * RBY + (ch << 4) + (p & 1) * 8;
  }

  f32x4 acc[9][NO];
#pragma unroll
  for (int t = 0; t < 9; ++t)
#pragma unroll
    for (int o = 0; o < NO; ++o) acc[t][o] = f32x4{0.f, 0.f, 0.f, 0.f};
  const bool do_bias = a.db != nullptr && ci_tile == 0 && wci < NO;
  f32x4 accb = f32x4{0.f, 0.f, 0.f, 0.f};

  bf16x8 win[3][3], yf[NO];
#pragma unroll
  for (int s = 0; s < 3; ++s)
#pragma unroll
    for (int j = 0; j < 3; ++j) win[s][j] = bf16x8{0, 0, 0, 0, 0, 0, 0, 0};
  auto tr2 = [&](int addr) __attribute__((always_inline)) {
    const s16x4 lo = __builtin_amdgcn_ds_read_tr16_b64_v4i16((LDS_AS s16x4*)(smem + addr));
    return lo;
  };
  auto mem = [&](auto uc) __attribute__((always_inline)) {
    constexpr int U = decltype(uc)::value;
#pragma unroll
    for (int o = 0; o < NO; ++o) {
      const s16x4 lo = tr2(yaddr[o] + U * YS), hi = tr2(yaddr[o] + 4 * RBY + U * YS);
      yf[o] = __builtin_bit_cast(bf16x8, __builtin_shufflevector(lo, hi, 0, 1, 2, 3, 4, 5, 6, 7));
    }
#pragma unroll
    for (int j = 0; j < 3; ++j) {
      const s16x4 lo = tr2(xaddr[j][0] + U * XS), hi = tr2(xaddr[j][1] + U * XS);
      win[U % 3][j] = __builtin_bit_cast(bf16x8, __builtin_shufflevector(lo, hi, 0, 1, 2, 3, 4, 5, 6, 7));
    }
  };
  auto mma = [&](auto uc) __attribute__((always_inline)) {
    constexpr int U = decltype(uc)::value;
#pragma unroll
    for (int i = 0; i < 3; ++i)
#pragma unroll
      for (int j = 0; j < 3; ++j)
#pragma unroll
        for (int o = 0; o < NO; ++o) acc[i * 3 + j][o] = DH_MFMA_16x16x32(win[(U + 1 + i) % 3][j], yf[o], acc[i * 3 + j][o]);
    if (do_bias) {
      const act16_t one = (act16_t)1.0f;
      const bf16x8 ones = {one, one, one, one, one, one, one, one};
#pragma unroll
      for (int o = 0; o < NO; ++o)
        if (wci == o) {
          accb = DH_MFMA_16x16x32(ones, yf[o], accb);
          asm volatile("" : "+v"(accb));
        }
    }
  };

  {
    RowStep s;
    gen_next(s, 0); dma_step(std::integral_constant<int, 0>{}, s);
    gen_next(s, 1); dma_step(std::integral_constant<int, 1>{}, s);
    gen_next(s, 2); dma_step(std::integral_constant<int, 2>{}, s);
    gen_next(s, 3); dma_step(std::integral_constant<int, 3>{}, s);
    static_assert(P == 4, "prologue issues P steps");
  }
  WR_CLK(1);
  wr_wait_vmcnt<0>();
  __builtin_amdgcn_s_barrier();

  RowStep nxt;
  [[maybe_unused]] int tr_step = 0;
  if (grp == 0) {
    gen_next(nxt, P);
    for (int v = 0; v < V; v += DEPTH) {
      auto step = [&](auto uc) __attribute__((always_inline)) {
        constexpr int U = decltype(uc)::value;
        WR_STAMP(0);
        dma_step(std::integral_constant<int, (U + P) % DEPTH>{}, nxt);
        __builtin_amdgcn_sched_barrier(0);
        mem(uc);
        __builtin_amdgcn_sched_barrier(0);
        gen_next(nxt, P + 1);
        wr_wait_vmcnt<2 * (P - 1)>();
        __builtin_amdgcn_s_waitcnt(0xC07F);
        WR_STAMP(1);
        __builtin_amdgcn_s_barrier();
        WR_STAMP(2);
        __builtin_amdgcn_sched_barrier(0);
        if (flags & 1ull) mma(uc);
        flags >>= 1;
        __builtin_amdgcn_sched_barrier(0);
        WR_STAMP(3);
        if (a.b2) __builtin_amdgcn_s_barrier();
        WR_STEP_DONE();
      };
      step(std::integral_constant<int, 0>{}); step(std::integral_constant<int, 1>{}); step(std::integral_constant<int, 2>{});
      step(std::integral_constant<int, 3>{}); step(std::integral_constant<int, 4>{}); step(std::integral_constant<int, 5>{});
    }
  } else {
    {
      mem(std::integral_constant<int, 0>{});
      gen_next(nxt, P);
      dma_step(std::integral_constant<int, P % DEPTH>{}, nxt);
      gen_next(nxt, P + 1);
    }
    for (int v = 0; v < V; v += DEPTH) {
      auto step = [&](auto uc) __attribute__((always_inline)) {
        constexpr int U = decltype(uc)::value;
        __builtin_amdgcn_s_waitcnt(0xC07F);
        WR_STAMP(0);
        __builtin_amdgcn_sched_barrier(0);
        if (flags & 1ull) mma(uc);
        flags >>= 1;
        __builtin_amdgcn_sched_barrier(0);
        WR_STAMP(1);
        wr_wait_vmcnt<2 * (P - 1)>();
        __builtin_amdgcn_s_barrier();
        WR_STAMP(2);
        dma_step(std::integral_constant<int, (U + 1 + P) % DEPTH>{}, nxt);
        __builtin_amdgcn_sched_barrier(0);
        mem(std::integral_constant<int, (U + 1) % DEPTH>{});
        __builtin_amdgcn_sched_barrier(0);
        gen_next(nxt, P + 1);
        __builtin_amdgcn_s_waitcnt(0xC07F);
        WR_STAMP(3);
        if (a.b2) __builtin_amdgcn_s_barrier();
        WR_STEP_DONE();
      };
      step(std::integral_constant<int, 0>{}); step(std::integral_constant<int, 1>{}); step(std::integral_constant<int, 2>{});
      step(std::integral_constant<int, 3>{}); step(std::integral_constant<int, 4>{}); step(std::integral_constant<int, 5>{});
    }
  }
  wr_wait_vmcnt<0>();
  WR_CLK(2);
#ifdef WR_TRACE
  __syncthreads();
  if (blockIdx.x == 0)
    for (int i = tid; i < 1024; i += 512) a.trace[i] = reinterpret_cast<const unsigned*>(smem + XBASE + DEPTH * XS)[i];
#endif

  if (a.ablate) {
#pragma unroll
    for (int t = 0; t < 9; ++t)
#pragma unroll
      for (int o = 0; o < NO; ++o) asm volatile("" ::"v"(acc[t][o]));
    WR_CLK(3);
    return;
  }
  if (a.slab) {
    f32x4* dst = reinterpret_cast<f32x4*>(a.slab) + (size_t)blockIdx.x * (9 * NO * 512) + wave * 64 + lane;
#pragma unroll
    for (int t = 0; t < 9; ++t)
#pragma unroll
      for (int o = 0; o < NO; ++o) __builtin_nontemporal_store(acc[t][o], dst + (t * NO + o) * 512);
    if (do_bias) {
      const int co = co0 + wco * NO * 16 + wci * 16 + (lane & 15);
      if (lane < 16 && co < a.Cout) atomicAdd(a.db + co, accb[0]);
    }
    WR_CLK(3);
    return;
  }
#pragma unroll
  for (int t = 0; t < 9; ++t)
#pragma unroll
    for (int r = 0; r < 4; ++r) {
      const int ci = ci0 + wci * 16 + g * 4 + r;
      if (ci >= a.cin_real) continue;
#pragma unroll
      for (int o = 0; o < NO; ++o) {
        const int co = co0 + wco * NO * 16 + o * 16 + (lane & 15);
        if (co < a.Cout) atomicAdd(a.dw + ((size_t)(t * a.cin_real + ci) * a.Cout + co), acc[t][o][r]);
      }
    }
  if (do_bias) {
    const int co = co0 + wco * NO * 16 + wci * 16 + (lane & 15);
    if (lane < 16 && co < a.Cout) atomicAdd(a.db + co, accb[0]);
  }
#ifdef WR_CLOCK
  asm volatile("s_waitcnt vmcnt(0)" ::: "memory");
  WR_CLK(3);
#endif
}

template <int COT>
__global__ __launch_bounds__(256) void wg_rows_reduce_kernel(const WgRowsArgs a) {
  constexpr int NO = COT / 32, TILE = 9 * NO * 512;
  __shared__ f32x4 part[4][64];
  const int pairs = a.ci_tiles * a.co_tiles;
  const int lane = threadIdx.x & 63, w = threadIdx.x >> 6;
  const int chunk = blockIdx.x;
  const int pair = chunk / (TILE / 64), q = (chunk - pair * (TILE / 64)) * 64 + lane;
  const f32x4* src = reinterpret_cast<const f32x4*>(a.slab) + q;
  auto blk = [&](int split) -> size_t {
    return a.xcd_grouped ? (size_t)(((split >> 3) * pairs + pair) * 8 + (split & 7)) : (size_t)(split * pairs + pair);
  };
  f32x4 s0 = {0.f, 0.f, 0.f, 0.f}, s1 = s0;
  int sp = w;
  for (; sp + 28 < a.splits; sp += 32) {
    f32x4 v[8];
#pragma unroll
    for (int e = 0; e < 8; ++e) v[e] = __builtin_nontemporal_load(src + blk(sp + 4 * e) * TILE);
    s0 += (v[0] + v[1]) + (v[2] + v[3]);
    s1 += (v[4] + v[5]) + (v[6] + v[7]);
  }
  for (; sp < a.splits; sp += 4) s0 += __builtin_nontemporal_load(src + blk(sp) * TILE);
  part[w][lane] = s0 + s1;
  __syncthreads();
  if (w != 0) return;
  const f32x4 sum = (part[0][lane] + part[1][lane]) + (part[2][lane] + part[3][lane]);
  const int to = q >> 9, wave = (q >> 6) & 7;
  const int t = to / NO, o = to - t * NO;
  const int wci = wave & 3, wco = wave >> 2, g = lane >> 4;
  const int co_tile = pair / a.ci_tiles, ci_tile = pair - co_tile * a.ci_tiles;
  const int co = co_tile * COT + wco * NO * 16 + o * 16 + (lane & 15);
  if (co >= a.Cout) return;
#pragma unroll
  for (int r = 0; r < 4; ++r) {
    const int ci = ci_tile * 64 + wci * 16 + g * 4 + r;
    if (ci < a.cin_real) a.dw[(size_t)(t * a.cin_real + ci) * a.Cout + co] += sum[r];
  }
}

#ifdef WR_CLOCK
static int g_wr_clock_blocks = 0, g_wr_clock_steps = 0;
unsigned long long* wr_clock_buffer() {
  static unsigned long long* p = [] { void* q = nullptr; (void)hipMalloc(&q, 4096 * 64); (void)hipMemset(q, 0, 4096 * 64); return (unsigned long long*)q; }();
  return p;
}
int wr_clock_blocks() { return g_wr_clock_blocks; }
int wr_clock_steps() { return g_wr_clock_steps; }
#endif

#ifdef WR_TRACE
unsigned* wr_trace_buffer() {
  static unsigned* p = [] { void* q = nullptr; (void)hipMalloc(&q, 4096 + 64); (void)hipMemset(q, 0, 4096 + 64); return (unsigned*)q; }();
  return p;
}
#endif

int wg_rows_cot(const danhip_conv_desc* d) { return ((d->Cout + 63) / 64 * 64) % 128 == 0 ? 128 : 64; }

bool wg_rows_eligible(const danhip_conv_desc* d) {
  if (!(d->kh == 3 && d->kw == 3 && d->stride == 1 && d->Ho == d->H && d->Wo == d->W)) return false;
  if (d->Cin % 64 != 0) return false;
  const int tw = 32;
  const double util = (double)d->W / (double)((d->W + tw - 1) / tw * tw);
  return util >= 0.6;
}

struct WgRowsPlan {
  int co8, ci_tiles, co_tiles, pairs, tiles_x, total_rows, splits, rows_per_split;
  bool slab;
  size_t slab_bytes;
};
WgRowsPlan plan_wg_rows(const danhip_conv_desc* d) {
  WgRowsPlan p{};
  const int cot = wg_rows_cot(d);
  p.co8 = (d->Cout + 7) / 8 * 8;
  p.ci_tiles = d->Cin / 64;
  p.co_tiles = (p.co8 + cot - 1) / cot;
  p.pairs = p.ci_tiles * p.co_tiles;
  p.tiles_x = (d->W + 31) / 32;
  p.total_rows = d->N * p.tiles_x * d->H;
  int splits = dh_cu_count() / p.pairs;
  if (splits < 1) splits = 1;
  if (splits > p.total_rows) splits = p.total_rows;
  p.rows_per_split = (p.total_rows + splits - 1) / splits;
  p.splits = (p.total_rows + p.rows_per_split - 1) / p.rows_per_split;
  p.slab = p.splits >= 2 && (danhip_option("wgrad_slab") == 2 || p.rows_per_split <= 192);
  p.slab_bytes = (size_t)dh_cu_count() * 9 * (cot / 32) * 512 * 16;
  return p;
}

template <int COT>
int launch_wg_rows(const WgradCall& c, hipStream_t s) {
  const danhip_conv_desc* d = c.d;
  const WgRowsPlan p = plan_wg_rows(d);
  WgRowsArgs a{};
  a.x = c.x; a.dy = c.dy; a.dw = c.dw; a.db = c.db;
  a.N = d->N; a.H = d->H; a.W = d->W; a.C = d->Cin; a.Co8 = p.co8; a.Cout = d->Cout; a.cin_real = c.cin_real;
  a.ldx = c.ldx ? c.ldx : d->Cin; a.ldy = c.ldy ? c.ldy : p.co8;
  a.tiles_x = p.tiles_x;
  a.total_rows = p.total_rows;
  a.div_tx = make_fastdiv(a.tiles_x);
  a.div_h = make_fastdiv(d->H);
  a.slab = (c.ws && p.slab && c.ws_bytes >= p.slab_bytes) ? reinterpret_cast<float*>(c.ws) : nullptr;
#ifdef WR_TRACE
  constexpr int LDS = 6 * (32 * COT * 2) + 6 * 40 * 128 + 4096;
  a.trace = wr_trace_buffer();
#else
  constexpr int LDS = 6 * (32 * COT * 2) + 6 * 40 * 128;
#endif
  static const bool attr_ok = hipFuncSetAttribute(reinterpret_cast<const void*>(&conv_wgrad_rows_kernel<COT>),
                                                  hipFuncAttributeMaxDynamicSharedMemorySize, LDS) == hipSuccess;
  (void)attr_ok;
  a.ci_tiles = p.ci_tiles;
  a.co_tiles = p.co_tiles;
  const int pairs = p.pairs, splits = p.splits;
  a.rows_per_split = p.rows_per_split;
  a.div_ci = make_fastdiv(a.ci_tiles);
  a.div_pairs = make_fastdiv(pairs);
  a.xcd_grouped = (splits % 8 == 0 && pairs > 1) ? 1 : 0;
  static const int ablate = [] { const char* e = getenv("DANHIP_WGRAD_ABLATE"); return e ? atoi(e) : 0; }();
  a.ablate = ablate;
  a.b2 = danhip_option("wgrad_b2");
  a.splits = splits;
#ifdef WR_CLOCK
  a.clk = wr_clock_buffer();
  g_wr_clock_blocks = pairs * splits;
  g_wr_clock_steps = a.rows_per_split;
#endif
  hipLaunchKernelGGL((conv_wgrad_rows_kernel<COT>), dim3(pairs * splits), dim3(512), LDS, s, a);
  DH_LAUNCH_CHECK();
  if (a.slab) {
    const int chunks = pairs * 9 * (COT / 32) * 512 / 64;
    hipLaunchKernelGGL((wg_rows_reduce_kernel<COT>), dim3(chunks), dim3(256), 0, s, a);
    DH_LAUNCH_CHECK();
  }
  return DANHIP_OK;
}

}

size_t wgrad_rows_workspace_bytes(const danhip_conv_desc* d) {
  if (!wg_rows_eligible(d)) return 0;
  const WgRowsPlan p = plan_wg_rows(d);
  return p.slab ? p.slab_bytes : 0;
}

WgradInstance wgrad_rows_select(const WgradCall& c) {
  if (!wg_rows_eligible(c.d)) return {};
  if (c.ldx > 0xFFFF || c.ldy > 0xFFFF) return {};
  WgradInstance i;
  if (wg_rows_cot(c.d) == 128) { i.label = "conv_wgrad_rows_kernel<128>"; i.launch = &launch_wg_rows<128>; }
  else { i.label = "conv_wgrad_rows_kernel<64>"; i.launch = &launch_wg_rows<64>; }
  return i;
}
```

### dan_amd/ops.py

```python
import contextlib
import ctypes
import os

import torch

from . import _lib
from ._lib import ACT_DTYPE as ACT, BF16, F32, SPLIT3, ConvDesc, call, ptr, stream


class OpsContext(object):
    __slots__ = ("USE_SPLITK", "USE_SLOTS", "USE_RELU_BITS", "USE_POOL_ARG", "USE_JUNCTION", "POOL_ONLY_TRAIN", "KEEP_DEFORM_COL", "WGRAD_STREAM", "WGRAD_FIRST", "FUSE_FIRST_WGRAD", "SPLIT_EVAL", "TRACE",
                 "PROFILE", "PROFILE_BYTES", "GRAD_READY_HOOK", "LOSS_SCALE_DEV", "wgrad")

    def __init__(self, **overrides):
        env = os.environ.get
        self.USE_SPLITK = True
        self.USE_SLOTS = True
        self.USE_RELU_BITS = env("DANHIP_RELU_BITS", "1") == "1"
        self.USE_POOL_ARG = env("DANHIP_POOL_ARG", "1") == "1"
        self.USE_JUNCTION = env("DANHIP_JUNCTION", "1") == "1"
        self.POOL_ONLY_TRAIN = env("DANHIP_POOL_ONLY_TRAIN", "1") == "1"
        self.KEEP_DEFORM_COL = True
        self.WGRAD_STREAM = env("DANHIP_WGRAD_STREAM", "1") == "1"
        self.WGRAD_FIRST = env("DANHIP_WGRAD_FIRST", "0") == "1"
        self.FUSE_FIRST_WGRAD = env("DANHIP_FUSE_FIRST_WGRAD", "1") == "1"
        self.SPLIT_EVAL = False
        self.TRACE = self.PROFILE = self.PROFILE_BYTES = None
        self.GRAD_READY_HOOK = self.LOSS_SCALE_DEV = None
        self.wgrad = {"on": False, "side": None, "main": None, "keep": []}
        for k, v in overrides.items():
            setattr(self, k, v)


_CTX = OpsContext()
_CTX_FIELDS = frozenset(OpsContext.__slots__) - {"wgrad"}


def context():
    return _CTX


@contextlib.contextmanager
def use_context(ctx):
    global _CTX
    prev, _CTX = _CTX, ctx
    try:
        yield ctx
    finally:
        _CTX = prev



def _desc(N, H, W, Cin, Cout, kh, kw, stride, valid=False):
    d = ConvDesc()
    d.N, d.H, d.W, d.Cin, d.Cout, d.kh, d.kw, d.stride = N, H, W, Cin, Cout, kh, kw, stride
    if valid:
        d.Ho, d.Wo = (H - kh) // stride + 1, (W - kw) // stride + 1
    else:
        d.Ho, d.Wo = -(-H // stride), -(-W // stride)
    return d


def packed_dims(d, which):
    r, c = ctypes.c_int64(), ctypes.c_int64()
    call("danhip_conv_packed_dims", ctypes.byref(d), which, ctypes.byref(r), ctypes.byref(c))
    return r.value, c.value


def pack_conv_weight(d, w_hwio, need_bwd=True):
    assert w_hwio.dtype == torch.float32 and w_hwio.is_contiguous()
    rf, cf = packed_dims(d, 0)
    wf = torch.empty((rf, cf), dtype=ACT, device=w_hwio.device)
    wb = None
    if need_bwd:
        rb, cb = packed_dims(d, 1)
        wb = torch.empty((rb, cb), dtype=ACT, device=w_hwio.device)
    call("danhip_pack_conv_weight", ctypes.byref(d), ptr(w_hwio), w_hwio.shape[2], ptr(wf), ptr(wb), stream())
    return wf, wb


WEIGHT_EPOCH = 0
_PACKED = {}
_PACK_TABLE_OF = {}


class _Packed(object):
    __slots__ = ("ref", "key", "d", "wf", "wb", "stamp")


def _stamp(p):
    return (WEIGHT_EPOCH, p._version, p.data_ptr())


def _drop_packed(pid):
    _PACKED.pop(pid, None)
    _PACK_TABLE_OF.clear()


def packed_weights(d, w, w_param, need_bwd):
    if w_param is None:
        return pack_conv_weight(d, w.detach(), need_bwd=need_bwd)
    import weakref
    key = (d.kh, d.kw, d.Cin, d.Cout, w.shape[2])
    pid = id(w_param)
    e = _PACKED.get(pid)
    if e is None or e.key != key or e.ref() is not w_param:
        e = _Packed()
        e.ref = weakref.ref(w_param, lambda _r, pid=pid: _drop_packed(pid))
        e.key, e.stamp, e.wb = key, None, None
        e.d = _desc(1, 8, 8, d.Cin, d.Cout, d.kh, d.kw, 1)
        rf, cf = packed_dims(e.d, 0)
        e.wf = torch.empty((rf, cf), dtype=ACT, device=w.device)
        _PACKED[pid] = e
        _PACK_TABLE_OF.clear()
    if need_bwd and e.wb is None:
        rb, cb = packed_dims(e.d, 1)
        e.wb = torch.empty((rb, cb), dtype=ACT, device=w.device)
        e.stamp = None
        _PACK_TABLE_OF.clear()
    st = _stamp(w_param)
    if e.stamp != st:
        wd = w_param.detach()
        if not (wd.dtype == torch.float32 and wd.is_contiguous()):
            raise RuntimeError("packed_weights: a kernel variable of shape %s arrives as a non-contiguous view (strides %s): it is a member of a "
                               "fused parameter block, which only the fused op consumes - set the fused / unfused switches BEFORE the "
                               "trainer (FlatParams) is built, not between calls" % (tuple(wd.shape), tuple(wd.stride())))
        call("danhip_pack_conv_weight", ctypes.byref(e.d), ptr(wd), wd.shape[2], ptr(e.wf), ptr(e.wb), stream())
        e.stamp = st
    return e.wf, (e.wb if need_bwd else None)


def repack_all(key=None, select=None):
    entries = [(e, e.ref()) for e in _PACKED.values()]
    entries = [(e, p) for e, p in entries if p is not None and (select is None or select(p))]
    if not entries:
        return
    tabs = _PACK_TABLE_OF
    tab = tabs.get(key)
    ids, ptrs = [id(p) for _, p in entries], [p.data_ptr() for _, p in entries]
    if tab is None or tab[3] != ids or tab[4] != ptrs:
        arr = (_lib.PackEntry * len(entries))()
        first = 0
        nb = ctypes.c_int32()
        for i, (e, p) in enumerate(entries):
            call("danhip_pack_entry_init", ctypes.byref(arr[i]), ctypes.byref(e.d), ptr(p.detach()), p.shape[2], ptr(e.wf), ptr(e.wb), first,
                 ctypes.byref(nb))
            first += nb.value
        host = torch.frombuffer(bytearray(bytes(arr)), dtype=torch.uint8)
        tab = tabs[key] = (len(entries), host.to(entries[0][1].device), first, ids, ptrs)
    n, dev_tab, blocks, _, _ = tab
    call("danhip_pack_conv_weights_batched", ptr(dev_tab), n, blocks, stream())
    for e, p in entries:
        e.stamp = _stamp(p)


def _grad_sink(p):
    return getattr(p, "_danhip_grad", None)


def _sink_trainable(t):
    ms = getattr(t, "_danhip_members", None)
    return ms is not None and any(m.requires_grad for m in ms)




def _prof_begin(st=None):
    if _CTX.PROFILE is None:
        return None
    e = torch.cuda.Event(enable_timing=True)
    e.record(st if st is not None else torch.cuda.current_stream())
    return e


def _prof_end(e0, d, which, st=None, wrote_y=True, pooled=False):
    if e0 is None:
        return
    e1 = torch.cuda.Event(enable_timing=True)
    e1.record(st if st is not None else torch.cuda.current_stream())
    if which == 2:
        label = _lib.lib().danhip_conv_wgrad_kernel_label(ctypes.byref(d)).decode()
    else:
        label = _lib.lib().danhip_conv_kernel_label(ctypes.byref(d), which).decode()
    cin = d.Cin
    flops = 2.0 * d.N * d.Ho * d.Wo * cin * d.Cout * d.kh * d.kw
    _CTX.PROFILE.setdefault(label, []).append((e0, e1, flops))
    if _CTX.PROFILE_BYTES is not None:
        co8 = (d.Cout + 7) // 8 * 8
        out_px = (d.Ho * d.Wo if wrote_y else 0) + (((d.Ho + 1) // 2) * ((d.Wo + 1) // 2) if pooled else 0)
        nbytes = 2.0 * d.N * (d.H * d.W * cin + out_px * co8) + 2.0 * d.kh * d.kw * cin * d.Cout
        _CTX.PROFILE_BYTES.setdefault(label, []).append(nbytes)




def wgrad_overlap_begin():
    if not torch.cuda.is_available():
        return
    if not _CTX.WGRAD_STREAM:
        return
    if _CTX.wgrad["side"] is None:
        _CTX.wgrad["side"] = torch.cuda.Stream()
    _CTX.wgrad["main"] = torch.cuda.current_stream()
    _CTX.wgrad["on"] = True


def wgrad_overlap_join():
    if _CTX.wgrad["on"]:
        torch.cuda.current_stream().wait_stream(_CTX.wgrad["side"])
    _CTX.wgrad["on"] = False
    _CTX.wgrad["keep"].clear()


def wgrad_streams():
    return [_CTX.wgrad["main"], _CTX.wgrad["side"]] if _CTX.wgrad["on"] else []





class GradSlot(object):

    __slots__ = ("shape", "dtype", "device", "is_relu", "buf", "count", "taps", "pending")

    def __init__(self, t, is_relu, channels=None):
        self.shape, self.dtype, self.device, self.is_relu = t.shape, t.dtype, t.device, is_relu
        if channels is not None:
            self.shape = tuple(t.shape[:-1]) + (channels,)
        self.buf, self.count = None, 0
        self.taps, self.pending = 0, None

    def defer(self, kind, alone, payload):
        buf, acc = self.target()
        self.pending = (kind, acc, alone, payload)

    def pop_pending(self, kind):
        p = self.pending
        if p is None or p[0] != kind:
            return None
        self.pending = None
        return p[1], p[3]

    def flush(self):
        p, self.pending = self.pending, None
        if p is not None:
            p[2](self.buf, p[1])

    def target(self):
        self.flush()
        if self.buf is None:
            self.buf = torch.empty(self.shape, dtype=self.dtype, device=self.device)
            self.count = 0
        acc = 1 if self.count > 0 else 0
        self.count += 1
        return self.buf, acc

    def take(self):
        self.flush()
        b, n = self.buf, self.count
        self.buf, self.count = None, 0
        return b if n > 0 else None




TAP_L2NORM, TAP_POOL = 1, 2


def _junction_ok(slot, dy, C):
    return _CTX.USE_JUNCTION and slot.taps == (TAP_L2NORM | TAP_POOL) and dy is None and C in (64, 128, 256, 512)


def _slot_of(t):
    return getattr(t, "_dh_slot", None) if _CTX.USE_SLOTS else None


def _new_slot(track):
    return GradSlot.__new__(GradSlot) if (track and _CTX.USE_SLOTS) else None


def _attach_slot(t, is_relu):
    s = GradSlot(t, is_relu)
    t._dh_slot = s
    return s




def _bits_holder(x):
    h = getattr(x, "_dh_bits", None)
    if h is None:
        h = [None]
        x._dh_bits = h
    return h


def relu_bits(x, holder):
    if holder[0] is None:
        C = x.shape[-1]
        M = x.numel() // C
        b = torch.empty((M, C // 8), dtype=torch.uint8, device=x.device)
        call("danhip_relu_bits", ptr(x), ptr(b), M, C, stream())
        holder[0] = b
    return holder[0]





def _conv_scratch(d, which, dev):
    M, co = (d.N * d.Ho * d.Wo, d.Cout) if which == 0 else (d.N * d.H * d.W, d.Cin)
    if not _CTX.USE_SPLITK or -(-M // 128) * -(-co // 128) > 160:
        return None, 0
    key = (which, d.N, d.H, d.W, d.Cin, d.Cout, d.kh, d.kw, d.stride, d.Ho)
    n = _SCRATCH_BYTES.get(key)
    if n is None:
        n = _SCRATCH_BYTES[key] = _lib.lib().danhip_conv2d_workspace_bytes(ctypes.byref(d), which)
    return (torch.empty(n, dtype=torch.uint8, device=dev), n) if n else (None, 0)


_SCRATCH_BYTES = {}


def _wgrad_scratch(d, dev):
    key = (2, d.N, d.H, d.W, d.Cin, d.Cout, d.kh, d.kw, d.stride, d.Ho)
    n = _SCRATCH_BYTES.get(key)
    if n is None:
        n = _SCRATCH_BYTES[key] = _lib.lib().danhip_conv2d_bwd_weight_workspace_bytes(ctypes.byref(d))
    return (torch.empty(n, dtype=torch.uint8, device=dev), n) if n else (None, 0)






def _pool_arg_buffer(pooled, need_bwd):
    if not (_CTX.USE_POOL_ARG and need_bwd):
        return None
    c = pooled.shape[-1]
    return torch.empty((pooled.numel() // c, c // 4), dtype=torch.uint8, device=pooled.device)


class _Conv2d(torch.autograd.Function):

    @staticmethod
    def forward(ctx, x, w, b, stride, relu, out_f32, residual, w_param, b_param, xslot, yslot, pool_out=None, valid=False, block_grads=0, xbits=None, bits_out=None,
                pool_only=False, tracked=True, first=None):
        N, H, W, C = x.shape
        kh, kw, cin_real, cout = w.shape
        ctx.first = first
        assert x.dtype == ACT and x.is_contiguous(), "conv input must be contiguous NHWC bf16"
        assert C % 8 == 0 and cin_real <= C
        d = _desc(N, H, W, C, cout, kh, kw, stride, valid)
        need_bwd = w.requires_grad or x.requires_grad or bool(block_grads)
        wf, wb = packed_weights(d, w, w_param, need_bwd)
        if pool_only == 1 and pool_out is not None and _lib.lib().danhip_conv2d_fwd_pool_only(ctypes.byref(d)):
            pooled = torch.empty((N, (d.Ho + 1) // 2, (d.Wo + 1) // 2, cout), dtype=ACT, device=x.device)
            e0 = _prof_begin()
            call("danhip_conv2d_fwd_pool", ctypes.byref(d), ptr(x), ptr(wf), ptr(b.detach()), None, ptr(pooled), stream())
            _prof_end(e0, d, 4, wrote_y=False, pooled=True)
            pooled._dh_already_pooled = True
            return pooled
        skip_y = (pool_only == 2 and pool_out is not None and _CTX.USE_POOL_ARG and need_bwd and b is not None
                  and bool(_lib.lib().danhip_conv2d_fwd_pool_only(ctypes.byref(d)))
                  and _conv_scratch(d, 0, x.device)[1] == 0)
        if skip_y:
            y = torch.empty((1,), dtype=ACT, device=x.device).expand(N, d.Ho, d.Wo, cout)
        else:
            y = torch.empty((N, d.Ho, d.Wo, cout), dtype=torch.float32 if out_f32 else ACT, device=x.device)
        yp = None if skip_y else ptr(y)
        e0 = _prof_begin()
        emit = (bits_out is not None and relu and not out_f32 and residual is None and b is not None
                and _lib.lib().danhip_conv2d_fwd_emits_bits(ctypes.byref(d), 1 if pool_out is not None else 0))
        if emit:
            ybits = torch.empty((N * d.Ho * d.Wo, cout // 8), dtype=torch.uint8, device=x.device)
            pooled = pbits = parg = None
            if pool_out is not None:
                pooled = torch.empty((N, (d.Ho + 1) // 2, (d.Wo + 1) // 2, cout), dtype=ACT, device=x.device)
                pbits = torch.empty((pooled.numel() // cout, cout // 8), dtype=torch.uint8, device=x.device)
                parg = _pool_arg_buffer(pooled, need_bwd and tracked)
                pool_out.extend([pooled, parg])
            call("danhip_conv2d_fwd_relu_bits_arg", ctypes.byref(d), ptr(x), ptr(wf), ptr(b.detach()), yp, ptr(ybits), ptr(pooled), ptr(pbits), ptr(parg),
                 stream())
            bits_out.extend([ybits, pbits])
        elif pool_out is not None:
            assert relu and not out_f32 and residual is None and b is not None and cout % 8 == 0
            pooled = torch.empty((N, (d.Ho + 1) // 2, (d.Wo + 1) // 2, cout), dtype=ACT, device=x.device)
            parg = _pool_arg_buffer(pooled, need_bwd and tracked)
            ws, nws = _conv_scratch(d, 0, x.device)
            if nws:
                assert not skip_y
                call("danhip_conv2d_fwd_ws", ctypes.byref(d), ptr(x), ptr(wf), ptr(b.detach()), ptr(y), BF16, 1, None, ptr(ws), nws, stream())
                call("danhip_maxpool2x2_fwd_arg", ptr(y), ptr(pooled), ptr(parg), N, d.Ho, d.Wo, cout, stream())
            else:
                call("danhip_conv2d_fwd_pool_arg", ctypes.byref(d), ptr(x), ptr(wf), ptr(b.detach()), yp, ptr(pooled), ptr(parg), stream())
            pool_out.extend([pooled, parg])
        else:
            ws, nws = _conv_scratch(d, 0, x.device)
            call("danhip_conv2d_fwd_ws", ctypes.byref(d), ptr(x), ptr(wf), ptr(b.detach()) if b is not None else None, ptr(y),
                 F32 if out_f32 else BF16, int(relu), ptr(residual), ptr(ws), nws, stream())
        _prof_end(e0, d, 4 if pool_out is not None else 0, wrote_y=not skip_y, pooled=pool_out is not None)
        ctx.d, ctx.relu, ctx.cin_real = d, relu, cin_real
        ctx.xslot, ctx.yslot, ctx.xbits = xslot, yslot, xbits
        ctx.set_materialize_grads(False)
        ctx.has_res = residual is not None
        ctx.w_param, ctx.b_param = w_param, b_param
        ctx.save_for_backward(x, wb, y if (relu and not skip_y) else None)
        ctx.y_unwritten = skip_y
        ctx.has_bias = b is not None
        ctx.block_w, ctx.block_b = bool(block_grads & 1), bool(block_grads & 2)
        return y

    @staticmethod
    def backward(ctx, dy):
        x, wb, y = ctx.saved_tensors
        d = ctx.d
        co8 = (d.Cout + 7) // 8 * 8
        M = d.N * d.Ho * d.Wo
        wp, bp = ctx.w_param, ctx.b_param
        need_dw = ctx.needs_input_grad[1] or ctx.block_w
        need_db = ctx.has_bias and (ctx.needs_input_grad[2] or ctx.block_b)
        db_sink = _grad_sink(bp) if bp is not None else None
        db = None
        if need_db:
            db = db_sink if db_sink is not None else torch.zeros(d.Cout, dtype=torch.float32, device=x.device)
        g = ctx.yslot.take() if ctx.yslot is not None else None
        dres = None
        if dy is not None and ctx.y_unwritten:
            raise RuntimeError("conv2d(pool_only=True): the full-resolution activation was never written, but a gradient reached it outside the "
                               "fused pool's direct hand-off (some op other than max_pool_2x2 consumed it)")
        if dy is not None:
            if ctx.has_res:
                dres = dy
            if dy.dtype != ACT or dy.shape[-1] != co8:
                src = dy.contiguous().to(torch.float32)
                dyp = torch.empty((d.N, d.Ho, d.Wo, co8), dtype=ACT, device=dy.device)
                call("danhip_cast_pad_f32_to_bf16", ptr(src), ptr(y) if (ctx.relu and d.Cout != co8) else None, ptr(dyp), M, d.Cout, co8, stream())
                dy, owned = dyp, True
                masked = ctx.relu and d.Cout != co8
            else:
                dy, owned = dy.contiguous(), False
                masked = False
            if ctx.relu and not masked:
                if not owned:
                    dy = dy.clone()
                call("danhip_relu_bwd_bias_grad", ptr(dy), ptr(y), None, M, co8, stream())
            g = dy if g is None else g.add_(dy)
        if g is None:
            return (None,) * 19
        db_in_wgrad = need_db and need_dw
        if need_db and not db_in_wgrad:
            if co8 == d.Cout:
                call("danhip_relu_bwd_bias_grad", ptr(g), None, ptr(db), M, co8, stream())
            else:
                db.add_(g.view(M, co8)[:, :d.Cout].to(torch.float32).sum(0))
        dx = None
        dw = None
        hooked = False
        fused_first = False

        def launch_dx():
            nonlocal dx, fused_first
            if ctx.needs_input_grad[0]:
                xs = ctx.xslot
                fi = ctx.first
                if (fi is not None and _CTX.FUSE_FIRST_WGRAD and xs is not None and xs.is_relu and xs.count == 0 and ctx.xbits is not None
                        and _grad_sink(fi[1]) is not None and (fi[2] is None or _grad_sink(fi[2]) is not None)
                        and _lib.lib().danhip_conv2d_bwd_data_first_supported(ctypes.byref(d))):
                    e0 = _prof_begin()
                    call("danhip_conv2d_bwd_data_bits_first", ctypes.byref(d), ptr(g), ptr(wb), ptr(relu_bits(x, ctx.xbits)), ptr(fi[0]), int(fi[3]),
                         ptr(_grad_sink(fi[1])), ptr(_grad_sink(fi[2])) if fi[2] is not None else None, stream())
                    _prof_end(e0, d, 5, wrote_y=False)
                    fused_first = True
                    return
                if xs is not None:
                    buf, acc = xs.target()
                    e0 = _prof_begin()
                    if xs.is_relu and ctx.xbits is not None and _lib.lib().danhip_conv2d_bwd_data_takes_bits(ctypes.byref(d)):
                        call("danhip_conv2d_bwd_data_bits", ctypes.byref(d), ptr(g), ptr(wb), ptr(relu_bits(x, ctx.xbits)), ptr(buf), acc, stream())
                    else:
                        ws, nws = _conv_scratch(d, 1, g.device)
                        call("danhip_conv2d_bwd_data_ws", ctypes.byref(d), ptr(g), ptr(wb), ptr(x) if xs.is_relu else None, ptr(buf), acc, ptr(ws), nws,
                             stream())
                    _prof_end(e0, d, 5 if xs.is_relu else 1)
                else:
                    dx = torch.empty_like(x)
                    e0 = _prof_begin()
                    ws, nws = _conv_scratch(d, 1, g.device)
                    call("danhip_conv2d_bwd_data_ws", ctypes.byref(d), ptr(g), ptr(wb), None, ptr(dx), 0, ptr(ws), nws, stream())
                    _prof_end(e0, d, 1)

        def launch_dw():
            nonlocal dw, hooked
            if need_dw:
                sink = _grad_sink(wp) if wp is not None else None
                dw = sink if sink is not None else torch.zeros((d.kh, d.kw, ctx.cin_real, d.Cout), dtype=torch.float32, device=g.device)
                ws, nws = _wgrad_scratch(d, g.device)
                if _CTX.wgrad["on"] and sink is not None:
                    side = _CTX.wgrad["side"]
                    ev = torch.cuda.Event()
                    ev.record(torch.cuda.current_stream())
                    side.wait_event(ev)
                    e0 = _prof_begin(side)
                    call("danhip_conv2d_bwd_weight_ws", ctypes.byref(d), ptr(x), ptr(g), ptr(dw), ptr(db) if db_in_wgrad else None, ctx.cin_real,
                         ptr(ws), nws, ctypes.c_void_p(side.cuda_stream))
                    _prof_end(e0, d, 2, side)
                    if _CTX.GRAD_READY_HOOK is not None and wp is not None:
                        _CTX.GRAD_READY_HOOK(wp)
                    _CTX.wgrad["keep"].append((g, x, ws))
                    hooked = True
                else:
                    e0 = _prof_begin()
                    call("danhip_conv2d_bwd_weight_ws", ctypes.byref(d), ptr(x), ptr(g), ptr(dw), ptr(db) if db_in_wgrad else None, ctx.cin_real,
                         ptr(ws), nws, stream())
                    _prof_end(e0, d, 2)
                if sink is not None:
                    dw = None

        if _CTX.WGRAD_FIRST:
            launch_dw()
            launch_dx()
        else:
            launch_dx()
            launch_dw()
        if db_sink is not None:
            db = None
        if _CTX.GRAD_READY_HOOK is not None and wp is not None and not hooked:
            _CTX.GRAD_READY_HOOK(wp)
        if fused_first and _CTX.GRAD_READY_HOOK is not None:
            _CTX.GRAD_READY_HOOK(ctx.first[1])
        return dx, dw, db, None, None, None, dres, None, None, None, None, None, None, None, None, None, None, None, None


def _f32_infer(x):
    if x.dtype != torch.float32:
        return False
    if torch.is_grad_enabled() and x.requires_grad:
        raise RuntimeError("the fp32 path is inference only (run it under torch.no_grad())")
    return True


def _conv2d_f32(x, w, b, stride, relu, residual, padding):
    N, H, W, C = x.shape
    kh, kw, cin, cout = w.shape
    assert cin == C and x.is_contiguous(), "fp32 conv: input channels must match the kernel (no channel padding on this path)"
    d = _desc(N, H, W, C, cout, kh, kw, stride, padding == "valid")
    y = torch.empty((N, d.Ho, d.Wo, cout), dtype=torch.float32, device=x.device)
    call("danhip_conv2d_fwd_f32", ctypes.byref(d), ptr(x), ptr(w.detach().contiguous()), ptr(b.detach()) if b is not None else None, ptr(y), int(relu),
         ptr(residual.contiguous()) if residual is not None else None, stream())
    return y


LIMB_EXP = 2
_SPLIT_W = {}
_RANGE_FLAG = [None]


class SplitRangeError(FloatingPointError):
    """A split-operand evaluation met a value outside the limbs' range (|x| >= 65520 * 2^exponent of its map, or NaN): its result is void."""


def _range_flag(device):
    f = _RANGE_FLAG[0]
    if f is None or f.device != device:
        f = torch.zeros(1, dtype=torch.int32, device=device)
        call("danhip_split_set_range_flag", ptr(f))
        _lib.call_f16("danhip_split_set_range_flag", ptr(f))
        _RANGE_FLAG[0] = f
    return f


def split_range_reset():
    f = _RANGE_FLAG[0]
    if f is not None:
        f.zero_()


def split_range_check():
    f = _RANGE_FLAG[0]
    if f is not None and int(f.item()):
        f.zero_()
        raise SplitRangeError("split-operand evaluation: a value outside the half limbs' range (|x| >= 65520 * 2^exponent of its map, or NaN); "
                              "the result would be silently wrong - evaluate with precision='fp32'")


def _weight_exp(w):
    import math
    m = float(w.detach().abs().max())
    if m == 0.0 or not math.isfinite(m):
        return 0
    return 14 - math.frexp(m)[1]


def _split_weight(d3, w, cin):
    import weakref
    key = id(w)
    stamp = (WEIGHT_EPOCH, w._version, w.data_ptr(), d3.Cin)
    e = _SPLIT_W.get(key)
# ... 136 lines not shown
    if _f32_infer(x):
        return _conv2d_f32(x, w, b, stride, relu, _f32_in(residual), padding)
    wp = w if (isinstance(w, torch.nn.Parameter) or hasattr(w, "_danhip_grad")) else None
    bp = b if (isinstance(b, torch.nn.Parameter) or hasattr(b, "_danhip_grad")) else None
    track = torch.is_grad_enabled() and (x.requires_grad or w.requires_grad or _sink_trainable(w))
    if track and relu and residual is not None:
        raise NotImplementedError("relu + fused residual needs a separate ReLU mask in backward (y > 0 is not the mask)")
    yslot = _new_slot(track and not out_f32)
    pool_out = [] if (pool and relu and not out_f32 and residual is None and b is not None and w.shape[-1] % 8 == 0) else None
    if padding not in ("same", "valid"):
        raise ValueError("padding must be 'same' or 'valid'")
    blk = 0
    if torch.is_grad_enabled():
        blk = (1 if _sink_trainable(w) else 0) | (2 if (b is not None and _sink_trainable(b)) else 0)
    xs = _slot_of(x) if track else None
    xbits = _bits_holder(x) if (xs is not None and xs.is_relu and _CTX.USE_RELU_BITS) else None
    bits_out = [] if (track and relu and _CTX.USE_RELU_BITS) else None
    po = (1 if not track else (2 if (_CTX.POOL_ONLY_TRAIN and _CTX.TRACE is None and _CTX.USE_SLOTS and yslot is not None) else 0)) if pool_only else 0
    y = _Conv2d.apply(x, w, b, stride, relu, out_f32, residual, wp, bp, xs, yslot, pool_out, padding == "valid", blk, xbits, bits_out,
                      po, bool(track), getattr(x, "_dh_first", None) if track else None)
    if (track and relu and not x.requires_grad and wp is not None and x.shape[-1] == 8 and w.shape[2] <= 4 and w.shape[3] == 64 and w.shape[0] == 3
            and w.shape[1] == 3 and stride == 1 and padding == "same" and residual is None and not out_f32):
        y._dh_first = (x, wp, bp, w.shape[2])
    if getattr(y, "_dh_already_pooled", False):
        return y
    if _CTX.TRACE is not None and relu and wp is not None:
        _CTX.TRACE[id(wp)] = y.detach()
    if bits_out:
        y._dh_bits = [bits_out[0]]
    if yslot is not None:
        cout = w.shape[-1]
        if cout % 8 == 0:
            yslot.__init__(y, relu)
            y._dh_slot = yslot
        else:
            yslot.__init__(y, relu, (cout + 7) // 8 * 8)
            y._dh_pslot = yslot
    if pool_out:
        y._dh_pooled = pool_out[0]
        y._dh_pool_arg = pool_out[1]
        if bits_out and bits_out[1] is not None:
            y._dh_pooled_bits = bits_out[1]
    return y


class _MaxPool(torch.autograd.Function):

    @staticmethod
    def forward(ctx, x, xslot, yslot, pre=None, arg=None):
        N, H, W, C = x.shape
        if pre is not None:
            y = pre
        else:
            y = torch.empty((N, (H + 1) // 2, (W + 1) // 2, C), dtype=x.dtype, device=x.device)
            arg = _pool_arg_buffer(y, x.requires_grad and C % 8 == 0)
            call("danhip_maxpool2x2_fwd_arg", ptr(x), ptr(y), ptr(arg), N, H, W, C, stream())
        ctx.arg = arg
        ctx.save_for_backward(x if arg is None else None)
        ctx.dims = (N, H, W, C)
        ctx.xslot, ctx.yslot = xslot, yslot
        if xslot is not None and arg is not None:
            xslot.taps |= TAP_POOL
        ctx.set_materialize_grads(False)
        return y

    @staticmethod
    def backward(ctx, dy):
        (x,) = ctx.saved_tensors
        N, H, W, C = ctx.dims
        g = ctx.yslot.take() if ctx.yslot is not None else None
        if dy is not None:
            g = dy.contiguous() if g is None else g.add_(dy)
        if g is None:
            return None, None, None, None, None

        def scatter(dst, acc):
            if ctx.arg is not None:
                call("danhip_maxpool2x2_bwd_arg", ptr(ctx.arg), ptr(g), ptr(dst), N, H, W, C, acc, stream())
            else:
                call("danhip_maxpool2x2_bwd", ptr(x), ptr(g), ptr(dst), N, H, W, C, acc, stream())

        if ctx.xslot is not None:
            xs = ctx.xslot
            if ctx.arg is not None and _pool_deliver_ok(ctx, dy) and _junction_ok(xs, dy, C):
                first = xs.pop_pending(TAP_L2NORM)
                if first is not None:
                    buf, _ = xs.target()
                    _junction(first[1], (ctx.arg, g, (N, H, W, C)), buf, first[0], xs.is_relu, 0)
                elif xs.pending is None:
                    xs.defer(TAP_POOL, scatter, (ctx.arg, g, (N, H, W, C)))
                else:
                    scatter(*xs.target())
                return None, None, None, None, None
            buf, acc = xs.target() if _pool_deliver_ok(ctx, dy) else (None, 0)
            if buf is not None:
                scatter(buf, acc)
                return None, None, None, None, None
        dx = torch.empty((N, H, W, C), dtype=g.dtype, device=g.device)
        scatter(dx, 0)
        return dx, None, None, None, None


def _junction(l2, pool, buf, acc, is_relu, pool_first):
    x, gamma, g, dg = l2
    arg, pg, (N, H, W, C) = pool
    call("danhip_l2norm_bwd_pool_scatter", ptr(x), ptr(gamma), ptr(g), ptr(arg), ptr(pg), ptr(buf), ptr(dg), N, H, W, C, acc, 1 if is_relu else 0,
         pool_first, stream())


def _pool_deliver_ok(ctx, dy):
    return not (ctx.xslot.is_relu and dy is not None)


def max_pool_2x2(x):
    if getattr(x, "_dh_already_pooled", False):
        return x
    if _is_limbs(x):
        N, H, W, C = x.shape
        if C % 8 == 0 and x._dh_split3.shape[-1] == 3 * C:
            y3 = torch.empty((N, (H + 1) // 2, (W + 1) // 2, 3 * C), dtype=torch.float16, device=x.device)
            call("danhip_maxpool2x2_split3", ptr(x._dh_split3), ptr(y3), N, H, W, C, stream())
            return _limb_view(y3, C, _limb_exp(x))
        x = unsplit3(x)
    if _f32_infer(x):
        N, H, W, C = x.shape
        y = torch.empty((N, (H + 1) // 2, (W + 1) // 2, C), dtype=torch.float32, device=x.device)
        call("danhip_maxpool2x2_fwd_f32", ptr(x.contiguous()), ptr(y), N, H, W, C, stream())
        return y
    if _CTX.TRACE is not None:
        _CTX.TRACE.setdefault("pools", []).append(x.detach())
    track = torch.is_grad_enabled() and x.requires_grad
    xs = _slot_of(x) if track else None
    yslot = _new_slot(track)
    y = _MaxPool.apply(x, xs, yslot, getattr(x, "_dh_pooled", None), getattr(x, "_dh_pool_arg", None))
    pbits = getattr(x, "_dh_pooled_bits", None)
    if pbits is not None and getattr(x, "_dh_pooled", None) is not None:
        y._dh_bits = [pbits]
    if yslot is not None:
        yslot.__init__(y, xs.is_relu if xs is not None else False)
        y._dh_slot = yslot
    return y


class _MaxPool3x3S2(torch.autograd.Function):

    @staticmethod
    def forward(ctx, x):
        N, H, W, C = x.shape
        y = torch.empty((N, (H + 1) // 2, (W + 1) // 2, C), dtype=x.dtype, device=x.device)
        call("danhip_maxpool3x3s2_same_fwd", ptr(x), ptr(y), N, H, W, C, stream())
        ctx.save_for_backward(x)
        return y

    @staticmethod
    def backward(ctx, dy):
        (x,) = ctx.saved_tensors
        N, H, W, C = x.shape
        dx = torch.empty_like(x)
        call("danhip_maxpool3x3s2_same_bwd", ptr(x), ptr(dy.contiguous()), ptr(dx), N, H, W, C, stream())
        return dx


def max_pool_3x3_s2(x):
    return _MaxPool3x3S2.apply(_f32_in(x))


# ... 874 lines not shown
```

### include/danhip.h

```cpp
#ifndef DANHIP_H_
#define DANHIP_H_
#include <stddef.h>
#include <stdint.h>

#ifdef __cplusplus
extern "C" {
#endif

#define DANHIP_OK 0
#define DANHIP_EINVAL (-1)
#define DANHIP_ELAUNCH (-2)
#define DANHIP_EWORKSPACE (-3)

#define DANHIP_F32 0
#define DANHIP_BF16 1
#define DANHIP_F16 2
#define DANHIP_SPLIT3 3

const char* danhip_last_error(void);
int danhip_version(void);
int danhip_set_option(const char* name, int value);
int danhip_get_option(const char* name);
int danhip_act_dtype(void);

typedef struct {
  int32_t N, H, W, Cin;
  int32_t Ho, Wo, Cout;
  int32_t kh, kw, stride;
} danhip_conv_desc;

int danhip_conv_packed_dims(const danhip_conv_desc* d, int which, int64_t* rows, int64_t* cols);
int danhip_pack_conv_weight(const danhip_conv_desc* d, const float* w_hwio, int32_t cin_real,
                            uint16_t* wf_packed, uint16_t* wb_packed, void* stream);

typedef struct {
  const float* w_hwio;
  uint16_t* wf_packed;
  uint16_t* wb_packed;
  int32_t kh, kw, cin, cin_real, cout, rows_f, cols_f, rows_b, cols_b, co8, first_block, pad_;
} danhip_pack_entry;
int danhip_pack_entry_init(danhip_pack_entry* e, const danhip_conv_desc* d, const float* w_hwio, int32_t cin_real,
                           uint16_t* wf_packed, uint16_t* wb_packed, int32_t first_block, int32_t* blocks);
int danhip_pack_conv_weights_batched(const danhip_pack_entry* table_dev, int32_t n, int32_t total_blocks, void* stream);

int danhip_conv2d_fwd(const danhip_conv_desc* d, const uint16_t* x, const uint16_t* wf_packed, const float* bias,
                      void* y, int out_dtype, int relu, const uint16_t* residual, void* stream);

int danhip_conv2d_fwd_pool(const danhip_conv_desc* d, const uint16_t* x, const uint16_t* wf_packed, const float* bias, uint16_t* y,
                           uint16_t* pool_y, void* stream);
int danhip_conv2d_fwd_pool_arg(const danhip_conv_desc* d, const uint16_t* x, const uint16_t* wf_packed, const float* bias, uint16_t* y,
                               uint16_t* pool_y, uint8_t* pool_arg, void* stream);
int danhip_conv2d_fwd_relu_bits_arg(const danhip_conv_desc* d, const uint16_t* x, const uint16_t* wf_packed, const float* bias, uint16_t* y,
                                    uint8_t* y_bits, uint16_t* pool_y, uint8_t* pool_bits, uint8_t* pool_arg, void* stream);
int danhip_conv2d_fwd_pool_only(const danhip_conv_desc* d);

int danhip_conv2d_bwd_data(const danhip_conv_desc* d, const uint16_t* dy, const uint16_t* wb_packed,
                           const uint16_t* relu_mask, uint16_t* dx, int accumulate, void* stream);

size_t danhip_conv2d_workspace_bytes(const danhip_conv_desc* d, int which);
int danhip_conv2d_fwd_ws(const danhip_conv_desc* d, const uint16_t* x, const uint16_t* wf_packed, const float* bias, void* y,
                         int out_dtype, int relu, const uint16_t* residual, void* ws, size_t ws_bytes, void* stream);
int danhip_conv2d_bwd_data_ws(const danhip_conv_desc* d, const uint16_t* dy, const uint16_t* wb_packed, const uint16_t* relu_mask,
                              uint16_t* dx, int accumulate, void* ws, size_t ws_bytes, void* stream);
int danhip_relu_bits(const uint16_t* x, uint8_t* bits, int64_t M, int32_t C, void* stream);
int danhip_conv2d_fwd_emits_bits(const danhip_conv_desc* d, int with_pool);
int danhip_conv2d_fwd_relu_bits(const danhip_conv_desc* d, const uint16_t* x, const uint16_t* wf_packed, const float* bias, uint16_t* y,
                                uint8_t* y_bits, uint16_t* pool_y, uint8_t* pool_bits, void* stream);
int danhip_conv2d_bwd_data_takes_bits(const danhip_conv_desc* d);
int danhip_conv2d_bwd_data_first_supported(const danhip_conv_desc* d);
int danhip_conv2d_bwd_data_bits_first(const danhip_conv_desc* d, const uint16_t* dy, const uint16_t* wb_packed, const uint8_t* relu_bits,
                                      const uint16_t* x8, int32_t cin_real, float* dw8, float* db8, void* stream);
int danhip_conv2d_bwd_data_bits(const danhip_conv_desc* d, const uint16_t* dy, const uint16_t* wb_packed, const uint8_t* relu_bits,
                                uint16_t* dx, int accumulate, void* stream);

int danhip_conv2d_fwd_concat2_supported(const danhip_conv_desc* d, int32_t c1, int32_t src_pitch);
int danhip_conv2d_fwd_concat2(const danhip_conv_desc* d, const uint16_t* x1, const uint16_t* x2, int32_t c1, int32_t src_pitch,
                              const uint16_t* wf_packed, const float* bias, uint16_t* y, int relu, void* stream);

typedef struct { int32_t x_pitch, y_pitch, aux_pitch; } danhip_conv_pitch;
int danhip_conv2d_fwd_strided(const danhip_conv_desc* d, const uint16_t* x, const uint16_t* wf_packed, const float* bias, uint16_t* y,
                              int relu, int32_t relu_channels, const danhip_conv_pitch* pitch, void* ws, size_t ws_bytes, void* stream);
int danhip_conv2d_bwd_data_strided(const danhip_conv_desc* d, const uint16_t* dy, const uint16_t* wb_packed, const uint16_t* relu_mask,
                                   uint16_t* dx, int accumulate, const danhip_conv_pitch* pitch, void* ws, size_t ws_bytes, void* stream);
int danhip_conv2d_bwd_weight_strided(const danhip_conv_desc* d, const uint16_t* x, const uint16_t* dy, float* dw_hwio, float* db,
                                     int32_t cin_real, const danhip_conv_pitch* pitch, void* ws, size_t ws_bytes, void* stream);

int danhip_conv2d_bwd_weight(const danhip_conv_desc* d, const uint16_t* x, const uint16_t* dy, float* dw_hwio, float* db,
                             int32_t cin_real, void* stream);
size_t danhip_conv2d_bwd_weight_workspace_bytes(const danhip_conv_desc* d);
int danhip_conv2d_bwd_weight_ws(const danhip_conv_desc* d, const uint16_t* x, const uint16_t* dy, float* dw_hwio, float* db,
                                int32_t cin_real, void* ws, size_t ws_bytes, void* stream);

int danhip_relu_bwd_bias_grad(uint16_t* dy, const uint16_t* y, float* db, int64_t M, int32_t C, void* stream);

const char* danhip_conv_kernel_label(const danhip_conv_desc* d, int which);
const char* danhip_conv_wgrad_kernel_label(const danhip_conv_desc* d);
const char* danhip_conv_last_launch_label(void);

int danhip_maxpool2x2_fwd(const uint16_t* x, uint16_t* y, int32_t N, int32_t H, int32_t W, int32_t C, void* stream);
int danhip_maxpool2x2_bwd(const uint16_t* x, const uint16_t* dy, uint16_t* dx, int32_t N, int32_t H, int32_t W, int32_t C,
                          int accumulate, void* stream);
int danhip_maxpool2x2_fwd_arg(const uint16_t* x, uint16_t* y, uint8_t* arg, int32_t N, int32_t H, int32_t W, int32_t C, void* stream);
int danhip_maxpool2x2_bwd_arg(const uint8_t* arg, const uint16_t* dy, uint16_t* dx, int32_t N, int32_t H, int32_t W, int32_t C,
                              int accumulate, void* stream);
int danhip_l2norm_fwd(const uint16_t* x, const float* gamma, uint16_t* y, int64_t M, int32_t C, void* stream);
int danhip_l2norm_bwd(const uint16_t* x, const float* gamma, const uint16_t* dy, uint16_t* dx, float* dgamma, int64_t M,
                      int32_t C, int accumulate, int relu_mask, void* stream);
int danhip_l2norm_bwd_pool_scatter(const uint16_t* x, const float* gamma, const uint16_t* dy, const uint8_t* arg, const uint16_t* pooled_dy,
                                   uint16_t* dx, float* dgamma, int32_t N, int32_t H, int32_t W, int32_t C, int accumulate, int relu_mask,
                                   int pool_first, void* stream);
int danhip_resize_bilinear_add_fwd(const uint16_t* up, const uint16_t* lateral, uint16_t* out, int32_t N, int32_t Hi, int32_t Wi,
                                   int32_t Ho, int32_t Wo, int32_t C, void* stream);
int danhip_resize_bilinear_add_bwd(const uint16_t* dout, uint16_t* dup, int32_t N, int32_t Hi, int32_t Wi, int32_t Ho, int32_t Wo,
                                   int32_t C, int accumulate, void* stream);
int danhip_avgpool2x2s1_same_fwd(const uint16_t* x, uint16_t* y, int32_t N, int32_t H, int32_t W, int32_t C, void* stream);
int danhip_avgpool2x2s1_same_bwd(const uint16_t* dy, const uint16_t* x_mask, uint16_t* dx, int32_t N, int32_t H, int32_t W, int32_t C,
                                 int accumulate, void* stream);
int danhip_add16(const uint16_t* a, const uint16_t* b, uint16_t* out, int64_t n, void* stream);
int danhip_residual_bwd(const uint16_t* dy, const uint16_t* r, const uint16_t* x_mask, uint16_t* dr, uint16_t* dx, int accumulate, int64_t n,
                        void* stream);
int danhip_avgpool2x2s1_same_fwd_strided(const uint16_t* x, int32_t x_pitch, uint16_t* y, int32_t y_pitch, int32_t N, int32_t H, int32_t W,
                                         int32_t C, int relu, void* stream);
int danhip_avgpool2x2s1_same_bwd_strided(const uint16_t* dy, int32_t y_pitch, uint16_t* dx, int32_t x_pitch, int32_t N, int32_t H, int32_t W,
                                         int32_t C, void* stream);
int danhip_slice_deliver(const uint16_t* dy, int32_t ldy, int32_t c0, int32_t C, const uint16_t* mask, int32_t ldm, uint16_t* out, int32_t Cpad,
                         int accumulate, int64_t M, void* stream);
int danhip_batchnorm_fwd_train(const uint16_t* x, const float* gamma, const float* beta, uint16_t* y, float* save_mean,
                               float* save_rstd, float* moving_mean, float* moving_var, int64_t M, int32_t C, float eps,
                               float momentum, int relu, float* workspace, void* stream);
int danhip_batchnorm_fwd_infer(const uint16_t* x, const float* gamma, const float* beta, const float* mean, const float* rstd,
                               uint16_t* y, int64_t M, int32_t C, int relu, void* stream);
int danhip_batchnorm_bwd(const uint16_t* x, const uint16_t* dy, const float* gamma, const float* save_mean, const float* save_rstd,
                         uint16_t* dx, float* dgamma, float* dbeta, int64_t M, int32_t C, void* stream);
int danhip_preprocess_u8(const uint8_t* img_rgb, uint16_t* out, int64_t npix, void* stream);
int danhip_cast_pad_f32_to_bf16(const float* src, const uint16_t* relu_y, uint16_t* dst, int64_t rows, int32_t c_src, int32_t c_dst,
                                void* stream);

int danhip_head_split_fwd(const float* h, float* loc, float* cls, int32_t B, int32_t HW, int32_t Ch, int32_t nneg, int32_t npos,
                          int32_t A, int32_t anchor_offset, void* stream);
int danhip_head_split_bwd(const float* h, const float* dloc, const float* dcls, float* dy, int32_t B, int32_t HW, int32_t Ch,
                          int32_t nneg, int32_t npos, int32_t A, int32_t anchor_offset, void* stream);
int danhip_hard_neg_select(const float* cls, const int32_t* labels, float* score, int32_t* counts, float* thr, int32_t* k_out,
                           int32_t B, int32_t A, float negative_ratio, int at_least_one, void* stream);
int danhip_detection_loss_fwd(const float* cls, const float* loc, const int32_t* labels, const float* loc_targets,
                              const float* score, const float* thr, uint8_t* sel, float* acc4, int32_t B, int32_t A,
                              void* stream);
int danhip_detection_loss_bwd(const float* cls, const float* loc, const float* loc_targets, const uint8_t* sel,
                              const float* acc4, float* dcls, float* dloc, float ce_scale, float loc_scale, int32_t B,
                              int32_t A, void* stream);
int danhip_sgd_momentum_flat(float* w, const float* g, float* v, const int64_t* seg_starts, const float* gmult,
                             const float* wd_coef, int32_t nseg, int64_t total, float lr, float momentum, float grad_scale,
                             float* l2_out, void* stream);
int danhip_sgd_momentum_flat_dynamic(float* w, const float* g, float* v, const int64_t* seg_starts, const float* gmult,
                                     const float* wd_coef, int32_t nseg, int64_t total, float lr, float momentum,
                                     float* loss_scale_state, float* l2_out, void* stream);

int danhip_anchors_generate(float* ymin, float* xmin, float* ymax, float* xmax, const float* anchor_h, const float* anchor_w,
                            int32_t depth, int32_t layer_h, int32_t layer_w, float stride, float offset_h, float offset_w,
                            int32_t out_offset, void* stream);
int danhip_iou_matrix(const float* ymin, const float* xmin, const float* ymax, const float* xmax, const uint8_t* inside_mask,
                      const float* gt_boxes, float* overlaps, int32_t A, int32_t G, void* stream);
size_t danhip_match_workspace_bytes(int32_t A, int32_t G);
int danhip_dual_max_match(const float* overlaps, int32_t A, int32_t G, float low_thres, float high_thres, int ignore_between,
                          int32_t* match_indices, float* match_scores, void* workspace, size_t workspace_bytes, void* stream);
int danhip_small_mining_match(const float* overlaps, int32_t A, int32_t G, float negative_low_thres, float negative_high_thres,
                              float positive_thres, int32_t min_match, float stop_positive_thres, int32_t* match_indices,
// ... 221 lines not shown
```

Before: 1263 images/sec.

## Fuse maxpool backward into following conv dgrad and wgrad via pooled codes

Maxpool backward no longer writes the full-resolution gradient. The next conv's data-gradient kernel (c64) and weight-gradient kernel (rows) now read the pooled gradient plus the 2-bit argmax codes, and expand them in LDS inside the kernel. This removes a full-resolution dY write and its re-read for the 64-channel VGG layers. The cost is extra LDS expansion work, extra barriers in the c64 pipeline, and new dispatch paths gated by a USE_POOL_CODES option.

Result: slower. 1249 images/sec (-1.1%).

```diff
diff --git a/dan_amd/_lib.py b/dan_amd/_lib.py
--- a/dan_amd/_lib.py
+++ b/dan_amd/_lib.py
@@ -76,6 +76,9 @@
     "danhip_relu_bits": [P, P, I64, I32, P],
     "danhip_conv2d_fwd_relu_bits": [DESC, P, P, P, P, P, P, P, P],
     "danhip_conv2d_bwd_weight": [DESC, P, P, P, P, I32, P],
+    "danhip_conv2d_bwd_data_bits_pooled": [DESC, P, P, P, P, P, ctypes.c_int, P],
+    "danhip_conv2d_bwd_data_bits_first_pooled": [DESC, P, P, P, P, P, I32, P, P, P],
+    "danhip_conv2d_bwd_weight_pooled": [DESC, P, P, P, P, P, I32, P, ctypes.c_size_t, P],
     "danhip_conv2d_bwd_weight_ws": [DESC, P, P, P, P, I32, P, ctypes.c_size_t, P],
     "danhip_avgpool2x2s1_same_fwd_strided": [P, I32, P, I32, I32, I32, I32, I32, ctypes.c_int, P],
     "danhip_avgpool2x2s1_same_bwd_strided": [P, I32, P, I32, I32, I32, I32, I32, P],
@@ -211,6 +214,14 @@
         L.danhip_conv_kernel_label.argtypes = [DESC, ctypes.c_int]
         L.danhip_conv_wgrad_kernel_label.restype = ctypes.c_char_p
         L.danhip_conv_wgrad_kernel_label.argtypes = [DESC]
+        L.danhip_conv_pooled_kernel_label.restype = ctypes.c_char_p
+        L.danhip_conv_pooled_kernel_label.argtypes = [DESC, ctypes.c_int]
+        L.danhip_conv_wgrad_pooled_kernel_label.restype = ctypes.c_char_p
+        L.danhip_conv_wgrad_pooled_kernel_label.argtypes = [DESC]
+        L.danhip_conv2d_bwd_data_pooled_supported.restype = ctypes.c_int
+        L.danhip_conv2d_bwd_data_pooled_supported.argtypes = [DESC, ctypes.c_int]
+        L.danhip_conv2d_bwd_weight_pooled_supported.restype = ctypes.c_int
+        L.danhip_conv2d_bwd_weight_pooled_supported.argtypes = [DESC]
         L.danhip_conv_last_launch_label.restype = ctypes.c_char_p
         L.danhip_conv_last_launch_label.argtypes = []
         L.danhip_match_workspace_bytes.argtypes = [I32, I32]
diff --git a/dan_amd/csrc/conv_common.h b/dan_amd/csrc/conv_common.h
--- a/dan_amd/csrc/conv_common.h
+++ b/dan_amd/csrc/conv_common.h
@@ -35,6 +35,7 @@
   int fuse_cin_real;
   int acc_exp;
   int* range_flag;
+  const unsigned char* dy_pool_codes;
 };
 
 __device__ __forceinline__ float dh_acc_scale(const ConvArgs& a) { return __builtin_bit_cast(float, (a.acc_exp + 127) << 23); }
@@ -124,6 +125,7 @@
   bool emits_bits = false;
   bool takes_bits = false;
   bool folds_first = false;
+  bool takes_pooled = false;
   explicit operator bool() const { return launch != nullptr; }
 };
 ConvInstance conv_c8_select(const ConvArgs& a);
@@ -140,6 +142,7 @@
   int cin_real, ldx, ldy;
   void* ws;
   size_t ws_bytes;
+  const unsigned char* pool_codes;
 };
 struct WgradInstance {
   const char* label = nullptr;
diff --git a/dan_amd/csrc/conv_halo_c64.hip b/dan_amd/csrc/conv_halo_c64.hip
--- a/dan_amd/csrc/conv_halo_c64.hip
+++ b/dan_amd/csrc/conv_halo_c64.hip
@@ -14,9 +14,10 @@
   asm volatile("s_waitcnt vmcnt(%0)" ::"n"(N) : "memory");
 }
 
-template <bool DGRAD, bool FUSE8 = false>
-__global__ __launch_bounds__(512, 2) __attribute__((amdgpu_waves_per_eu(2, 2))) void conv3x3_c64_kernel(const ConvArgs a, const C64Geom g) {
+template <bool DGRAD, bool FUSE8, bool POOL>
+__device__ __forceinline__ void c64_body(const ConvArgs& a, const C64Geom& g) {
   static_assert(DGRAD || !FUSE8, "the folded first-layer weight gradient belongs to the data gradient");
+  static_assert(DGRAD || !POOL, "the pooled operand is a data gradient's dY");
   constexpr int TH = 8, TW = 32, PW = TW + 2;
   constexpr int PROWS = (TH + 2) * PW, PPIECES = (PROWS + 7) / 8, PBYTES = PPIECES * 1024, PL = (PPIECES + 7) / 8;
   constexpr int NPT = 4, NCT = 2;
@@ -47,7 +48,67 @@
 
   const unsigned npix1 = (unsigned)(a.N * a.H * a.W) - 1u;
   const unsigned px_x = (unsigned)a.ldx * 2u, px_y = (unsigned)a.ldy * 2u, px_m = (unsigned)a.ldm * 2u;
-  const __amdgpu_buffer_rsrc_t rsrc_x = __builtin_amdgcn_make_buffer_rsrc(const_cast<bf16_t*>(a.x), 0, (int)(npix1 * px_x + 128u), 0x00020000);
+  [[maybe_unused]] const int Hp = a.H >> 1, Wp = a.W >> 1;
+  const __amdgpu_buffer_rsrc_t rsrc_x =
+      __builtin_amdgcn_make_buffer_rsrc(const_cast<bf16_t*>(a.x), 0, POOL ? (int)((unsigned)(a.N * Hp * Wp) * 128u) : (int)(npix1 * px_x + 128u), 0x00020000);
+  [[maybe_unused]] const __amdgpu_buffer_rsrc_t rsrc_c = __builtin_amdgcn_make_buffer_rsrc(
+      const_cast<unsigned char*>(POOL ? a.dy_pool_codes : reinterpret_cast<const unsigned char*>(a.x)), 0, (int)((unsigned)(a.N * Hp * Wp) * 16u), 0x00020000);
+  [[maybe_unused]] auto issue_pool = [&](int sp, int buf) __attribute__((always_inline)) {
+    if (wave >= 6) return;
+    int n, y0, x0;
+    sp_coords(sp, n, y0, x0);
+    int ln = lane;
+    asm volatile("" : "+v"(ln));
+    const int Y = (y0 >> 1) - 1 + wave;
+    const bool yok = (unsigned)Y < (unsigned)Hp;
+    char* const st = smem + buf * PBYTES + (wave ? (2 * wave - 1) * PW * 128 : 0);
+#pragma unroll
+    for (int k = 0; k < 3; ++k) {
+      const int wx = k * 8 + (ln >> 3), X = (x0 >> 1) - 1 + wx;
+      const bool ok = yok && wx < PW / 2 + 1 && (unsigned)X < (unsigned)Wp;
+      __builtin_amdgcn_raw_ptr_buffer_load_lds(rsrc_x, (LDS_AS void*)(st + k * 1024), 16,
+                                               ok ? (unsigned)((n * Hp + Y) * Wp + X) * 128u + (unsigned)((ln & 7) << 4) : 0xFFFFFFFFu, 0, 0, 0);
+    }
+    const int X = (x0 >> 1) - 1 + ln;
+    const bool ok = yok && ln < PW / 2 + 1 && (unsigned)X < (unsigned)Wp;
+    __builtin_amdgcn_raw_ptr_buffer_load_lds(rsrc_c, (LDS_AS void*)(st + 3072), 16, ok ? (unsigned)((n * Hp + Y) * Wp + X) * 16u : 0xFFFFFFFFu, 0, 0, 0);
+  };
+  [[maybe_unused]] auto expand_pool = [&](int buf) __attribute__((always_inline)) {
+    if (wave >= 6) return;
+    typedef __attribute__((ext_vector_type(4))) unsigned u32x4;
+    int ln = lane;
+    asm volatile("" : "+v"(ln));
+    char* const pb = smem + buf * PBYTES;
+    const char* const st = pb + (wave ? (2 * wave - 1) * PW * 128 : 0);
+    u32x4 v[3];
+    unsigned cd[3];
+#pragma unroll
+    for (int r = 0; r < 3; ++r) {
+      const int i = r * 64 + ln < 144 ? r * 64 + ln : 143;
+      v[r] = *reinterpret_cast<const u32x4*>(st + i * 16);
+      cd[r] = *reinterpret_cast<const unsigned short*>(st + 3072 + (i >> 3) * 16 + (i & 7) * 2);
+    }
+    __builtin_amdgcn_s_waitcnt(0xC07F);
+    __builtin_amdgcn_sched_barrier(0);
+#pragma unroll
+    for (int r = 0; r < 3; ++r) {
+      const int i = r * 64 + ln, wx = i >> 3, c = i & 7;
+#pragma unroll
+      for (int pos = 0; pos < 4; ++pos) {
+        const int hy = 2 * wave - 1 + (pos >> 1), hx = 2 * wx - 1 + (pos & 1);
+        if ((unsigned)hy >= (unsigned)(TH + 2)) continue;
+        const unsigned t = cd[r] ^ (0x5555u * pos);
+        const unsigned keep = ((t | (t >> 1)) & 0x5555u) ^ 0x5555u;
+        u32x4 o;
+#pragma unroll
+        for (int e = 0; e < 4; ++e) {
+          const unsigned b = ((((keep >> (4 * e)) & 5u) * 0x4001u) & 0x10001u) * 0xFFFFu;
+          o[e] = v[r][e] & b;
+        }
+        if (i < 144 && (unsigned)hx < (unsigned)PW) *reinterpret_cast<u32x4*>(pb + (hy * PW + hx) * 128 + ((c ^ (hx & 7)) << 4)) = o;
+      }
+    }
+  };
   auto issue_patch = [&](int sp, int buf) __attribute__((always_inline)) {
     int n, y0, x0;
     sp_coords(sp, n, y0, x0);
@@ -164,12 +225,16 @@
   const int xend = xcd_walk ? (xbase + per_xcd < g.sp_items ? xbase + per_xcd : g.sp_items) : g.sp_items;
   int sp = xcd_walk ? xbase + (int)(blockIdx.x >> 3) : (int)blockIdx.x;
   if (sp >= xend) return;
-  issue_patch(sp, 0);
+  if constexpr (POOL) issue_pool(sp, 0); else issue_patch(sp, 0);
   if constexpr (!DGRAD) {
     if (tid < 64) reinterpret_cast<float*>(smem + RWBASE)[tid] = a.bias ? a.bias[tid] : 0.f;
     __builtin_amdgcn_s_waitcnt(0xC07F);
   }
   c64_wait_vmcnt<0>();
+  if constexpr (POOL) {
+    expand_pool(0);
+    __builtin_amdgcn_s_waitcnt(0xC07F);
+  }
   __builtin_amdgcn_s_barrier();
   int buf = 0;
   for (;;) {
@@ -180,7 +245,9 @@
       if (a.mask_bits) issue_bits(sp, buf);
       if constexpr (FUSE8) issue_img(sp, buf);
     }
-    if (has_next) issue_patch(nsp, buf ^ 1);
+    if (has_next) {
+      if constexpr (POOL) issue_pool(nsp, buf ^ 1); else issue_patch(nsp, buf ^ 1);
+    }
     auto rd = [&](bf16x8 (&x)[NPT], auto hc) __attribute__((always_inline)) {
       constexpr int H = decltype(hc)::value;
       read_px(x, std::integral_constant<int, H / 2>{}, H & 1);
@@ -199,6 +266,11 @@
     C64_H(12, xa); C64_H(13, xb); C64_H(14, xc); C64_H(15, xa); C64_H(16, xb); C64_H(17, xc);
 #undef C64_H
     c64_wait_vmcnt<0>();
+    if constexpr (POOL) {
+      __builtin_amdgcn_sched_barrier(0);
+      if (has_next) expand_pool(buf ^ 1);
+      __builtin_amdgcn_s_waitcnt(0xC07F);
+    }
     __builtin_amdgcn_s_barrier();
     {
       int n, y0, x0;
@@ -385,6 +457,15 @@
   }
 }
 
+template <bool DGRAD, bool FUSE8 = false>
+__global__ __launch_bounds__(512, 2) __attribute__((amdgpu_waves_per_eu(2, 2))) void conv3x3_c64_kernel(const ConvArgs a, const C64Geom g) {
+  c64_body<DGRAD, FUSE8, false>(a, g);
+}
+template <bool FUSE8>
+__global__ __launch_bounds__(512, 2) __attribute__((amdgpu_waves_per_eu(2, 2))) void conv3x3_c64_pool_kernel(const ConvArgs a, const C64Geom g) {
+  c64_body<true, FUSE8, true>(a, g);
+}
+
 bool c64_eligible(const ConvArgs& a) {
   if (!(a.kh == 3 && a.kw == 3 && a.stride == 1 && a.dstride == 1 && a.pad_t == 1 && a.pad_l == 1)) return false;
   if (a.H != a.Ho || a.W != a.Wo || a.C != 64 || a.Co != 64 || a.out_f32 || a.Kpad != 576) return false;
@@ -396,12 +477,13 @@
   return util >= 0.78 && (int64_t)a.N * a.H * a.W * ldmax * 2 < (1ll << 32);
 }
 
-template <bool DGRAD, bool FUSE8 = false>
+template <bool DGRAD, bool FUSE8 = false, bool POOL = false>
 int launch_c64(const ConvArgs& a, hipStream_t s) {
   constexpr int LDS = 2 * ((10 * 34 + 7) / 8) * 1024 + (FUSE8 ? 75776 : (DGRAD ? 65536 : 256));
   static_assert(LDS <= 160 * 1024, "LDS budget");
-  static const bool attr_ok =
-      hipFuncSetAttribute(reinterpret_cast<const void*>(&conv3x3_c64_kernel<DGRAD, FUSE8>), hipFuncAttributeMaxDynamicSharedMemorySize, LDS) == hipSuccess;
+  void (*kernel)(const ConvArgs, const C64Geom);
+  if constexpr (POOL) kernel = &conv3x3_c64_pool_kernel<FUSE8>; else kernel = &conv3x3_c64_kernel<DGRAD, FUSE8>;
+  static const bool attr_ok = hipFuncSetAttribute(reinterpret_cast<const void*>(kernel), hipFuncAttributeMaxDynamicSharedMemorySize, LDS) == hipSuccess;
   (void)attr_ok;
   C64Geom g{};
   g.tiles_x = (a.W + 31) / 32;
@@ -411,16 +493,16 @@
   g.div_txy = make_fastdiv(g.tiles_x * g.tiles_y);
   int G = dh_cu_count();
   if (g.sp_items < G) G = g.sp_items;
-  hipLaunchKernelGGL((conv3x3_c64_kernel<DGRAD, FUSE8>), dim3(G), dim3(512), LDS, s, a, g);
+  hipLaunchKernelGGL(kernel, dim3(G), dim3(512), LDS, s, a, g);
   DH_LAUNCH_CHECK();
   return DANHIP_OK;
 }
 
-template <bool DGRAD, bool FUSE8 = false>
+template <bool DGRAD, bool FUSE8 = false, bool POOL = false>
 ConvInstance c64_instance(const char* label) {
   ConvInstance i;
   i.label = label;
-  i.launch = &launch_c64<DGRAD, FUSE8>;
+  i.launch = &launch_c64<DGRAD, FUSE8, POOL>;
   return i;
 }
 
@@ -431,14 +513,19 @@
   const bool dgrad = !a.bias && !a.relu && !a.resid;
   if (!dgrad && (a.accumulate || a.mask || a.mask_bits)) return {};
   if (a.mask && a.mask_bits) return {};
+  const bool pool = a.dy_pool_codes != nullptr;
+  if (pool && (!dgrad || a.strided() || ((a.H | a.W) & 1))) return {};
   ConvInstance i;
   if (a.fuse_dw) {
     if (!dgrad || !a.mask_bits || a.accumulate || a.strided() || !a.fuse_x8 || a.fuse_cin_real < 1 || a.fuse_cin_real > 4) return {};
-    i = c64_instance<true, true>("conv3x3_c64_kernel<true, true>");
+    i = pool ? c64_instance<true, true, true>("conv3x3_c64_pool_kernel<true>") : c64_instance<true, true>("conv3x3_c64_kernel<true, true>");
     i.folds_first = a.W % 2 == 0 && (int64_t)a.N * a.H * a.W * 16 < (1ll << 31);
+  } else if (pool) {
+    i = c64_instance<true, false, true>("conv3x3_c64_pool_kernel<false>");
   } else {
     i = dgrad ? c64_instance<true>("conv3x3_c64_kernel<true>") : c64_instance<false>("conv3x3_c64_kernel<false>");
   }
+  i.takes_pooled = pool;
   i.takes_bits = dgrad && a.W % 2 == 0;
   i.fuses_pool = i.skips_y = !dgrad && a.pool_y && a.bias && a.relu && !a.resid;
   return i;
diff --git a/dan_amd/csrc/conv_igemm.hip b/dan_amd/csrc/conv_igemm.hip
--- a/dan_amd/csrc/conv_igemm.hip
+++ b/dan_amd/csrc/conv_igemm.hip
@@ -409,6 +409,7 @@
     i.launch = &launch_direct_dgrad;
     return i;
   }
+  if (a.dy_pool_codes) return conv_c64_select(a);
   const bool view = a.strided();
   const bool limbs = a.split_out != 0;
   if (!view && !limbs)
@@ -954,6 +955,54 @@
   return rc;
 }
 
+namespace {
+ConvArgs pooled_rep_args(const danhip_conv_desc* d, int first) {
+  ConvArgs a = bwd_args(d);
+  a.mask_bits = &g_rep_bits; a.dy_pool_codes = &g_rep_bits;
+  if (first) { a.fuse_x8 = &g_rep_act; a.fuse_dw = &g_rep_f32; a.fuse_cin_real = 3; }
+  return a;
+}
+}
+
+extern "C" int danhip_conv2d_bwd_data_pooled_supported(const danhip_conv_desc* d, int first) {
+  if (!d || check_desc(d) != DANHIP_OK || d->stride != 1) return 0;
+  const ConvInstance i = select_conv(pooled_rep_args(d, first));
+  return i.takes_pooled && (!first || i.folds_first) ? 1 : 0;
+}
+
+extern "C" const char* danhip_conv_pooled_kernel_label(const danhip_conv_desc* d, int first) {
+  if (!d || check_desc(d) != DANHIP_OK || d->stride != 1) return "";
+  const char* l = select_conv(pooled_rep_args(d, first)).label;
+  return l ? l : "";
+}
+
+extern "C" int danhip_conv2d_bwd_data_bits_pooled(const danhip_conv_desc* d, const uint16_t* pooled_dy, const uint8_t* pool_arg, const uint16_t* wb_packed,
+                                                  const uint8_t* relu_bits, uint16_t* dx, int accumulate, void* stream) {
+  int rc = check_desc(d);
+  if (rc) return rc;
+  DH_REQUIRE(pooled_dy && pool_arg && wb_packed && dx && relu_bits, DANHIP_EINVAL, "conv2d_bwd_data_bits_pooled: null pointer");
+  DH_REQUIRE(danhip_conv2d_bwd_data_pooled_supported(d, 0), DANHIP_EINVAL, "conv2d_bwd_data_bits_pooled: not a shape whose data gradient reads the "
+             "pooled pair (ask danhip_conv2d_bwd_data_pooled_supported first)");
+  ConvArgs a = bwd_args(d);
+  a.x = pooled_dy; a.dy_pool_codes = pool_arg; a.w = wb_packed; a.mask_bits = relu_bits; a.y = dx; a.accumulate = accumulate;
+  return launch_conv(a, (hipStream_t)stream);
+}
+
+extern "C" int danhip_conv2d_bwd_data_bits_first_pooled(const danhip_conv_desc* d, const uint16_t* pooled_dy, const uint8_t* pool_arg,
+                                                        const uint16_t* wb_packed, const uint8_t* relu_bits, const uint16_t* x8, int32_t cin_real,
+                                                        float* dw8, float* db8, void* stream) {
+  int rc = check_desc(d);
+  if (rc) return rc;
+  DH_REQUIRE(pooled_dy && pool_arg && wb_packed && relu_bits && x8 && dw8, DANHIP_EINVAL, "conv2d_bwd_data_bits_first_pooled: null pointer");
+  DH_REQUIRE(cin_real >= 1 && cin_real <= 4, DANHIP_EINVAL, "conv2d_bwd_data_bits_first_pooled: cin_real = %d (1..4 real channels of the 8-channel image)", cin_real);
+  DH_REQUIRE(danhip_conv2d_bwd_data_pooled_supported(d, 1), DANHIP_EINVAL, "conv2d_bwd_data_bits_first_pooled: not a shape whose folded data gradient reads "
+             "the pooled pair (ask danhip_conv2d_bwd_data_pooled_supported first)");
+  ConvArgs a = bwd_args(d);
+  a.x = pooled_dy; a.dy_pool_codes = pool_arg; a.w = wb_packed; a.mask_bits = relu_bits; a.y = nullptr;
+  a.fuse_x8 = x8; a.fuse_dw = dw8; a.fuse_db = db8; a.fuse_cin_real = cin_real;
+  return launch_conv(a, (hipStream_t)stream);
+}
+
 extern "C" int danhip_conv2d_bwd_data_bits(const danhip_conv_desc* d, const uint16_t* dy, const uint16_t* wb_packed, const uint8_t* relu_bits,
                                            uint16_t* dx, int accumulate, void* stream) {
   int rc = check_desc(d);
diff --git a/dan_amd/csrc/conv_wgrad.hip b/dan_amd/csrc/conv_wgrad.hip
--- a/dan_amd/csrc/conv_wgrad.hip
+++ b/dan_amd/csrc/conv_wgrad.hip
@@ -239,6 +239,7 @@
 }
 
 WgradInstance select_wgrad(const WgradCall& c) {
+  if (c.pool_codes) return wgrad_rows_select(c);
   if (WgradInstance i = wgrad_rows_select(c)) return i;
   if (WgradInstance i = wgrad_pw_select(c)) return i;
   if (WgradInstance i = wgrad_c8_select(c)) return i;
@@ -283,6 +284,33 @@
   return dh_run_instance(select_wgrad(c), c, (hipStream_t)stream);
 }
 
+static WgradCall pooled_rep_call(const danhip_conv_desc* d) {
+  static const unsigned char rep = 0;
+  return WgradCall{d, nullptr, nullptr, nullptr, nullptr, d->Cin, d->Cin, (d->Cout + 7) / 8 * 8, nullptr, 0, &rep};
+}
+
+extern "C" int danhip_conv2d_bwd_weight_pooled_supported(const danhip_conv_desc* d) {
+  if (!d || d->N <= 0 || d->Cin % 8 != 0) return 0;
+  if ((int64_t)d->N * d->H * d->W * d->Cin >= (1ll << 31)) return 0;
+  return select_wgrad(pooled_rep_call(d)) ? 1 : 0;
+}
+
+extern "C" const char* danhip_conv_wgrad_pooled_kernel_label(const danhip_conv_desc* d) {
+  if (!d) return "";
+  const char* l = select_wgrad(pooled_rep_call(d)).label;
+  return l ? l : "";
+}
+
+extern "C" int danhip_conv2d_bwd_weight_pooled(const danhip_conv_desc* d, const uint16_t* x, const uint16_t* pooled_dy, const uint8_t* pool_arg,
+                                               float* dw_hwio, float* db, int32_t cin_real, void* ws, size_t ws_bytes, void* stream) {
+  DH_REQUIRE(d && x && pooled_dy && pool_arg && dw_hwio, DANHIP_EINVAL, "conv2d_bwd_weight_pooled: null pointer");
+  DH_REQUIRE(cin_real > 0 && cin_real <= d->Cin, DANHIP_EINVAL, "conv2d_bwd_weight_pooled: cin_real out of range");
+  DH_REQUIRE(danhip_conv2d_bwd_weight_pooled_supported(d), DANHIP_EINVAL, "conv2d_bwd_weight_pooled: not a shape whose weight gradient reads the "
+             "pooled pair (ask danhip_conv2d_bwd_weight_pooled_supported first)");
+  const WgradCall c{d, x, pooled_dy, dw_hwio, db, cin_real, d->Cin, (d->Cout + 7) / 8 * 8, ws, ws_bytes, pool_arg};
+  return dh_run_instance(select_wgrad(c), c, (hipStream_t)stream);
+}
+
 extern "C" int danhip_conv2d_bwd_weight(const danhip_conv_desc* d, const uint16_t* x, const uint16_t* dy, float* dw_hwio, float* db,
                                         int32_t cin_real, void* stream) {
   return danhip_conv2d_bwd_weight_ws(d, x, dy, dw_hwio, db, cin_real, nullptr, 0, stream);
diff --git a/dan_amd/csrc/conv_wgrad_rows.hip b/dan_amd/csrc/conv_wgrad_rows.hip
--- a/dan_amd/csrc/conv_wgrad_rows.hip
+++ b/dan_amd/csrc/conv_wgrad_rows.hip
@@ -19,6 +19,7 @@
   float* slab;
   int splits;
   FastDiv div_tx, div_h, div_ci, div_pairs;
+  const unsigned char* codes;
 #ifdef WR_TRACE
   unsigned* trace;
 #endif
@@ -80,8 +81,9 @@
   bool xvalid, yvalid;
 };
 
-template <int COT>
-__global__ __launch_bounds__(512, 2) __attribute__((amdgpu_waves_per_eu(2, 2))) void conv_wgrad_rows_kernel(const WgRowsArgs a) {
+template <int COT, bool POOL>
+__device__ __forceinline__ void wg_rows_body(const WgRowsArgs& a) {
+  static_assert(!POOL || COT == 64, "the pooled form is conv1_2's: 64 output channels");
   constexpr int TW = 32;
   constexpr int PITCH = 40;
   constexpr int XS = PITCH * 128;
@@ -124,7 +126,10 @@
   const int V = (steps + DEPTH - 1) / DEPTH * DEPTH;
 
   const wr_u32x4 rsrc_x = wr_make_rsrc(a.x, ((unsigned)(a.N * a.H * a.W - 1) * (unsigned)a.ldx + (unsigned)a.C) * 2u);
-  const wr_u32x4 rsrc_y = wr_make_rsrc(a.dy, ((unsigned)(a.N * a.H * a.W - 1) * (unsigned)a.ldy + (unsigned)a.Co8) * 2u);
+  const int Hp = a.H >> 1, Wp = a.W >> 1;
+  const int yrole = wave & 3;
+  const wr_u32x4 rsrc_y = !POOL ? wr_make_rsrc(a.dy, ((unsigned)(a.N * a.H * a.W - 1) * (unsigned)a.ldy + (unsigned)a.Co8) * 2u)
+                          : yrole < 2 ? wr_make_rsrc(a.dy, (unsigned)(a.N * Hp * Wp) * 128u) : wr_make_rsrc(a.codes, (unsigned)(a.N * Hp * Wp) * 16u);
   const unsigned lds0 = __builtin_amdgcn_readfirstlane((unsigned)(size_t)(LDS_AS char*)smem);
 
   RowGen gen;
@@ -138,6 +143,7 @@
   gen.left = k_end - k_begin;
   gen_strip(gen);
   unsigned long long flags = 0;
+  [[maybe_unused]] unsigned long long pars = 0;
   auto gen_next = [&](RowStep& s, int bit) __attribute__((always_inline)) {
     s.n = gen.n; s.x0 = gen.x0;
     if (gen.left == 0) {
@@ -148,6 +154,7 @@
     } else {
       s.xrow = gen.y + 1; s.yrow = gen.y; s.xvalid = true; s.yvalid = true;
       flags |= 1ull << bit;
+      if constexpr (POOL) pars |= (unsigned long long)(gen.y & 1) << bit;
       gen.y += 1; gen.left -= 1;
       if (gen.y == a.H) { gen.strip += 1; gen.y = 0; gen.warm = 2; gen_strip(gen); }
     }
@@ -169,6 +176,9 @@
     const int ychunk = yB ^ (COT == 128 ? (sb << 3) : (sb << 2));
     vy = __umul24((unsigned)lp, (unsigned)(a.ldy * 2)) + (unsigned)(ychunk << 4);
     if (!(co0 + ychunk * 8 < a.Co8)) vy = 0xFFFFFFFFu;
+    if constexpr (POOL) {
+      vy = yrole < 2 ? (unsigned)(l8 * 128 + (((lane & 7) ^ (wr_f128(yrole * 8 + l8) << 1)) << 4)) : (lane < 16 ? (unsigned)(lane * 16) : 0xFFFFFFFFu);
+    }
   }
   unsigned vxbad = 0, vybad = 0;
   int dma_x0 = -1;
@@ -179,6 +189,7 @@
       const int x = s.x0 - 1 + pc5 * 8 + l8;
       vxbad = (l8 < (pc5 == 4 ? 2 : 8) && (unsigned)x < (unsigned)a.W) ? 0u : 0xFFFFFFFFu;
       vybad = (s.x0 + ypiece * PXP + lp < a.W) ? 0u : 0xFFFFFFFFu;
+      if constexpr (POOL) vybad = ((s.x0 >> 1) + (yrole < 2 ? yrole * 8 + l8 : lane) < Wp) ? 0u : 0xFFFFFFFFu;
     }
     {
       const int xs = s.x0 - 1 + pc5 * 8;
@@ -187,12 +198,18 @@
       const unsigned voff = (vx + sbase) | vxbad | bady;
       wr_dma16(rsrc_x, voff, lds0 + XBASE + SL * XS + pc5 * 1024);
     }
-    {
+    if constexpr (!POOL) {
       const int xs = s.x0 + ypiece * PXP;
       const unsigned bady = (s.yvalid && (unsigned)s.yrow < (unsigned)a.H) ? 0u : 0xFFFFFFFFu;
       const unsigned sbase = (unsigned)(((s.n * a.H + s.yrow) * a.W + xs) * a.ldy + co0) * 2u;
       const unsigned voff = (vy + sbase) | vybad | bady;
       wr_dma16(rsrc_y, voff, lds0 + YBASE + SL * YS + ypiece * 1024);
+    } else {
+      const unsigned bady = (s.yvalid && (unsigned)s.yrow < (unsigned)a.H) ? 0u : 0xFFFFFFFFu;
+      const unsigned w0 = (unsigned)((s.n * Hp + (s.yrow >> 1)) * Wp + (s.x0 >> 1));
+      const unsigned sbase = yrole < 2 ? (w0 + (unsigned)yrole * 8u) * 128u : w0 * 16u;
+      const unsigned voff = (vy + sbase) | vybad | bady;
+      wr_dma16(rsrc_y, voff, lds0 + YBASE + SL * YS + (yrole < 2 ? yrole * 1024 : 2048));
     }
   };
 
@@ -212,7 +229,13 @@
     const int px = 8 * g + q;
     const int ch = ((wco * NO + o) * 2 + (p >> 1)) ^ ((COT == 128 ? wr_f256(px) : wr_f128(px)) << 1);
     yaddr[o] = YBASE + px * RBY + (ch << 4) + (p & 1) * 8;
-  }
+    if constexpr (POOL) {
+      const int wd = 4 * g + q;
+      yaddr[o] = YBASE + wd * 128 + ((((wco * NO + o) * 2 + (p >> 1)) ^ (wr_f128(wd) << 1)) << 4) + (p & 1) * 8;
+    }
+  }
+  [[maybe_unused]] const int caddr = YBASE + 2048 + 4 * g * 16 + wco * 8;
+  [[maybe_unused]] const int cshift = 8 * q + 2 * p;
 
   f32x4 acc[9][NO];
 #pragma unroll
@@ -233,10 +256,30 @@
   };
   auto mem = [&](auto uc) __attribute__((always_inline)) {
     constexpr int U = decltype(uc)::value;
-#pragma unroll
-    for (int o = 0; o < NO; ++o) {
-      const s16x4 lo = tr2(yaddr[o] + U * YS), hi = tr2(yaddr[o] + 4 * RBY + U * YS);
-      yf[o] = __builtin_bit_cast(bf16x8, __builtin_shufflevector(lo, hi, 0, 1, 2, 3, 4, 5, 6, 7));
+    if constexpr (POOL) {
+      const unsigned s0 = (unsigned)(pars & 1ull) * 2u, s1 = s0 + 1u;
+      uint2 ck[4];
+#pragma unroll
+      for (int k = 0; k < 4; ++k) ck[k] = *reinterpret_cast<const uint2*>(smem + caddr + k * 16 + U * YS);
+#pragma unroll
+      for (int o = 0; o < NO; ++o) {
+        const uint2 pv = __builtin_bit_cast(uint2, tr2(yaddr[o] + U * YS));
+        wr_u32x4 e;
+#pragma unroll
+        for (int k = 0; k < 4; ++k) {
+          const unsigned src = k < 2 ? pv.x : pv.y;
+          const unsigned val = (k & 1) ? (src >> 16) : (src & 0xFFFFu);
+          const unsigned c = ((o ? ck[k].y : ck[k].x) >> cshift) & 3u;
+          e[k] = (c == s0 ? val : 0u) | (c == s1 ? val << 16 : 0u);
+        }
+        yf[o] = __builtin_bit_cast(bf16x8, e);
+      }
+    } else {
+#pragma unroll
+      for (int o = 0; o < NO; ++o) {
+        const s16x4 lo = tr2(yaddr[o] + U * YS), hi = tr2(yaddr[o] + 4 * RBY + U * YS);
+        yf[o] = __builtin_bit_cast(bf16x8, __builtin_shufflevector(lo, hi, 0, 1, 2, 3, 4, 5, 6, 7));
+      }
     }
 #pragma unroll
     for (int j = 0; j < 3; ++j) {
@@ -297,6 +340,7 @@
         __builtin_amdgcn_sched_barrier(0);
         if (flags & 1ull) mma(uc);
         flags >>= 1;
+        if constexpr (POOL) pars >>= 1;
         __builtin_amdgcn_sched_barrier(0);
         WR_STAMP(3);
         if (a.b2) __builtin_amdgcn_s_barrier();
@@ -320,6 +364,7 @@
         __builtin_amdgcn_sched_barrier(0);
         if (flags & 1ull) mma(uc);
         flags >>= 1;
+        if constexpr (POOL) pars >>= 1;
         __builtin_amdgcn_sched_barrier(0);
         WR_STAMP(1);
         wr_wait_vmcnt<2 * (P - 1)>();
@@ -388,6 +433,14 @@
   asm volatile("s_waitcnt vmcnt(0)" ::: "memory");
   WR_CLK(3);
 #endif
+}
+
+template <int COT>
+__global__ __launch_bounds__(512, 2) __attribute__((amdgpu_waves_per_eu(2, 2))) void conv_wgrad_rows_kernel(const WgRowsArgs a) {
+  wg_rows_body<COT, false>(a);
+}
+__global__ __launch_bounds__(512, 2) __attribute__((amdgpu_waves_per_eu(2, 2))) void conv_wgrad_rows_pool_kernel(const WgRowsArgs a) {
+  wg_rows_body<64, true>(a);
 }
 
 template <int COT>
@@ -480,12 +533,12 @@
   return p;
 }
 
-template <int COT>
+template <int COT, bool POOL = false>
 int launch_wg_rows(const WgradCall& c, hipStream_t s) {
   const danhip_conv_desc* d = c.d;
   const WgRowsPlan p = plan_wg_rows(d);
   WgRowsArgs a{};
-  a.x = c.x; a.dy = c.dy; a.dw = c.dw; a.db = c.db;
+  a.x = c.x; a.dy = c.dy; a.dw = c.dw; a.db = c.db; a.codes = c.pool_codes;
   a.N = d->N; a.H = d->H; a.W = d->W; a.C = d->Cin; a.Co8 = p.co8; a.Cout = d->Cout; a.cin_real = c.cin_real;
   a.ldx = c.ldx ? c.ldx : d->Cin; a.ldy = c.ldy ? c.ldy : p.co8;
   a.tiles_x = p.tiles_x;
@@ -499,8 +552,8 @@
 #else
   constexpr int LDS = 6 * (32 * COT * 2) + 6 * 40 * 128;
 #endif
-  static const bool attr_ok = hipFuncSetAttribute(reinterpret_cast<const void*>(&conv_wgrad_rows_kernel<COT>),
-                                                  hipFuncAttributeMaxDynamicSharedMemorySize, LDS) == hipSuccess;
+  void (*const kernel)(const WgRowsArgs) = POOL ? &conv_wgrad_rows_pool_kernel : &conv_wgrad_rows_kernel<COT>;
+  static const bool attr_ok = hipFuncSetAttribute(reinterpret_cast<const void*>(kernel), hipFuncAttributeMaxDynamicSharedMemorySize, LDS) == hipSuccess;
   (void)attr_ok;
   a.ci_tiles = p.ci_tiles;
   a.co_tiles = p.co_tiles;
@@ -518,7 +571,7 @@
   g_wr_clock_blocks = pairs * splits;
   g_wr_clock_steps = a.rows_per_split;
 #endif
-  hipLaunchKernelGGL((conv_wgrad_rows_kernel<COT>), dim3(pairs * splits), dim3(512), LDS, s, a);
+  hipLaunchKernelGGL(kernel, dim3(pairs * splits), dim3(512), LDS, s, a);
   DH_LAUNCH_CHECK();
   if (a.slab) {
     const int chunks = pairs * 9 * (COT / 32) * 512 / 64;
@@ -540,6 +593,11 @@
   if (!wg_rows_eligible(c.d)) return {};
   if (c.ldx > 0xFFFF || c.ldy > 0xFFFF) return {};
   WgradInstance i;
+  if (c.pool_codes) {
+    if (c.d->Cin != 64 || c.d->Cout != 64 || (c.d->H | c.d->W) & 1 || c.ldx != 64 || c.ldy != 64) return {};
+    i.label = "conv_wgrad_rows_pool_kernel"; i.launch = &launch_wg_rows<64, true>;
+    return i;
+  }
   if (wg_rows_cot(c.d) == 128) { i.label = "conv_wgrad_rows_kernel<128>"; i.launch = &launch_wg_rows<128>; }
   else { i.label = "conv_wgrad_rows_kernel<64>"; i.launch = &launch_wg_rows<64>; }
   return i;
diff --git a/dan_amd/ops.py b/dan_amd/ops.py
--- a/dan_amd/ops.py
+++ b/dan_amd/ops.py
@@ -9,7 +9,7 @@
 
 
 class OpsContext(object):
-    __slots__ = ("USE_SPLITK", "USE_SLOTS", "USE_RELU_BITS", "USE_POOL_ARG", "USE_JUNCTION", "POOL_ONLY_TRAIN", "KEEP_DEFORM_COL", "WGRAD_STREAM", "WGRAD_FIRST", "FUSE_FIRST_WGRAD", "SPLIT_EVAL", "TRACE",
+    __slots__ = ("USE_SPLITK", "USE_SLOTS", "USE_RELU_BITS", "USE_POOL_ARG", "USE_JUNCTION", "USE_POOL_CODES", "POOL_ONLY_TRAIN", "KEEP_DEFORM_COL", "WGRAD_STREAM", "WGRAD_FIRST", "FUSE_FIRST_WGRAD", "SPLIT_EVAL", "TRACE",
                  "PROFILE", "PROFILE_BYTES", "GRAD_READY_HOOK", "LOSS_SCALE_DEV", "wgrad")
 
     def __init__(self, **overrides):
@@ -19,6 +19,7 @@
         self.USE_RELU_BITS = env("DANHIP_RELU_BITS", "1") == "1"
         self.USE_POOL_ARG = env("DANHIP_POOL_ARG", "1") == "1"
         self.USE_JUNCTION = env("DANHIP_JUNCTION", "1") == "1"
+        self.USE_POOL_CODES = env("DANHIP_POOL_CODES", "0") == "1"
         self.POOL_ONLY_TRAIN = env("DANHIP_POOL_ONLY_TRAIN", "1") == "1"
         self.KEEP_DEFORM_COL = True
         self.WGRAD_STREAM = env("DANHIP_WGRAD_STREAM", "1") == "1"
@@ -173,22 +174,34 @@
     return e
 
 
-def _prof_end(e0, d, which, st=None, wrote_y=True, pooled=False):
+def _prof_end(e0, d, which, st=None, wrote_y=True, pooled=False, pooled_dy=False, folded=None):
     if e0 is None:
         return
     e1 = torch.cuda.Event(enable_timing=True)
     e1.record(st if st is not None else torch.cuda.current_stream())
-    if which == 2:
+    if pooled_dy:
+        L = _lib.lib()
+        label = (L.danhip_conv_wgrad_pooled_kernel_label(ctypes.byref(d)) if which == 2 else
+                 L.danhip_conv_pooled_kernel_label(ctypes.byref(d), 1 if folded else 0)).decode()
+    elif folded:
+        label = "conv3x3_c64_kernel<true, true>"
+    elif which == 2:
         label = _lib.lib().danhip_conv_wgrad_kernel_label(ctypes.byref(d)).decode()
     else:
         label = _lib.lib().danhip_conv_kernel_label(ctypes.byref(d), which).decode()
     cin = d.Cin
     flops = 2.0 * d.N * d.Ho * d.Wo * cin * d.Cout * d.kh * d.kw
+    if folded:
+        flops += 2.0 * d.N * d.H * d.W * 9 * folded * cin
     _CTX.PROFILE.setdefault(label, []).append((e0, e1, flops))
     if _CTX.PROFILE_BYTES is not None:
         co8 = (d.Cout + 7) // 8 * 8
         out_px = (d.Ho * d.Wo if wrote_y else 0) + (((d.Ho + 1) // 2) * ((d.Wo + 1) // 2) if pooled else 0)
         nbytes = 2.0 * d.N * (d.H * d.W * cin + out_px * co8) + 2.0 * d.kh * d.kw * cin * d.Cout
+        if pooled_dy:
+            nbytes -= d.N * (2.0 * d.Ho * d.Wo - 2.25 * (d.Ho // 2) * (d.Wo // 2)) * co8
+        if folded:
+            nbytes += d.N * d.H * d.W * (cin / 8.0 + 16.0)
         _CTX.PROFILE_BYTES.setdefault(label, []).append(nbytes)
 
 
@@ -241,9 +254,16 @@
         self.pending = None
         return p[1], p[3]
 
+    def defer_first(self, kind, alone, payload):
+        assert self.buf is None and self.pending is None
+        self.pending = (kind, 0, alone, payload)
+
     def flush(self):
         p, self.pending = self.pending, None
         if p is not None:
+            if self.buf is None:
+                self.buf = torch.empty(self.shape, dtype=self.dtype, device=self.device)
+                self.count = 1
             p[2](self.buf, p[1])
 
     def target(self):
@@ -264,6 +284,7 @@
 
 
 
+TAP_POOL_CODES = 4
 TAP_L2NORM, TAP_POOL = 1, 2
 
 
@@ -424,7 +445,22 @@
         db = None
         if need_db:
             db = db_sink if db_sink is not None else torch.zeros(d.Cout, dtype=torch.float32, device=x.device)
-        g = ctx.yslot.take() if ctx.yslot is not None else None
+        pool_pair = None
+        ys = ctx.yslot
+        if ys is not None and dy is None and ys.buf is None and ys.pending is not None and ys.pending[0] == TAP_POOL_CODES and _CTX.USE_POOL_CODES:
+            L = _lib.lib()
+            xs, fi = ctx.xslot, ctx.first
+            dx_form = 0
+            if ctx.needs_input_grad[0] and xs is not None and xs.is_relu and ctx.xbits is not None:
+                if (fi is not None and _CTX.FUSE_FIRST_WGRAD and xs.count == 0 and _grad_sink(fi[1]) is not None
+                        and (fi[2] is None or _grad_sink(fi[2]) is not None) and L.danhip_conv2d_bwd_data_first_supported(ctypes.byref(d))):
+                    dx_form = 1 if L.danhip_conv2d_bwd_data_pooled_supported(ctypes.byref(d), 1) else 0
+                elif L.danhip_conv2d_bwd_data_takes_bits(ctypes.byref(d)):
+                    dx_form = 2 if L.danhip_conv2d_bwd_data_pooled_supported(ctypes.byref(d), 0) else 0
+            if ((dx_form or not ctx.needs_input_grad[0]) and (need_dw or not need_db)
+                    and (not need_dw or L.danhip_conv2d_bwd_weight_pooled_supported(ctypes.byref(d)))):
+                pool_pair = ys.pop_pending(TAP_POOL_CODES)[1]
+        g = pool_pair[1] if pool_pair is not None else (ys.take() if ys is not None else None)
         dres = None
         if dy is not None and ctx.y_unwritten:
             raise RuntimeError("conv2d(pool_only=True): the full-resolution activation was never written, but a gradient reached it outside the "
@@ -468,21 +504,28 @@
                         and _grad_sink(fi[1]) is not None and (fi[2] is None or _grad_sink(fi[2]) is not None)
                         and _lib.lib().danhip_conv2d_bwd_data_first_supported(ctypes.byref(d))):
                     e0 = _prof_begin()
-                    call("danhip_conv2d_bwd_data_bits_first", ctypes.byref(d), ptr(g), ptr(wb), ptr(relu_bits(x, ctx.xbits)), ptr(fi[0]), int(fi[3]),
-                         ptr(_grad_sink(fi[1])), ptr(_grad_sink(fi[2])) if fi[2] is not None else None, stream())
-                    _prof_end(e0, d, 5, wrote_y=False)
+                    if pool_pair is not None:
+                        call("danhip_conv2d_bwd_data_bits_first_pooled", ctypes.byref(d), ptr(g), ptr(pool_pair[0]), ptr(wb), ptr(relu_bits(x, ctx.xbits)),
+                             ptr(fi[0]), int(fi[3]), ptr(_grad_sink(fi[1])), ptr(_grad_sink(fi[2])) if fi[2] is not None else None, stream())
+                    else:
+                        call("danhip_conv2d_bwd_data_bits_first", ctypes.byref(d), ptr(g), ptr(wb), ptr(relu_bits(x, ctx.xbits)), ptr(fi[0]), int(fi[3]),
+                             ptr(_grad_sink(fi[1])), ptr(_grad_sink(fi[2])) if fi[2] is not None else None, stream())
+                    _prof_end(e0, d, 5, wrote_y=False, pooled_dy=pool_pair is not None, folded=int(fi[3]))
                     fused_first = True
                     return
                 if xs is not None:
                     buf, acc = xs.target()
                     e0 = _prof_begin()
-                    if xs.is_relu and ctx.xbits is not None and _lib.lib().danhip_conv2d_bwd_data_takes_bits(ctypes.byref(d)):
+                    if pool_pair is not None:
+                        call("danhip_conv2d_bwd_data_bits_pooled", ctypes.byref(d), ptr(g), ptr(pool_pair[0]), ptr(wb), ptr(relu_bits(x, ctx.xbits)),
+                             ptr(buf), acc, stream())
+                    elif xs.is_relu and ctx.xbits is not None and _lib.lib().danhip_conv2d_bwd_data_takes_bits(ctypes.byref(d)):
                         call("danhip_conv2d_bwd_data_bits", ctypes.byref(d), ptr(g), ptr(wb), ptr(relu_bits(x, ctx.xbits)), ptr(buf), acc, stream())
                     else:
                         ws, nws = _conv_scratch(d, 1, g.device)
                         call("danhip_conv2d_bwd_data_ws", ctypes.byref(d), ptr(g), ptr(wb), ptr(x) if xs.is_relu else None, ptr(buf), acc, ptr(ws), nws,
                              stream())
-                    _prof_end(e0, d, 5 if xs.is_relu else 1)
+                    _prof_end(e0, d, 5 if xs.is_relu else 1, pooled_dy=pool_pair is not None)
                 else:
                     dx = torch.empty_like(x)
                     e0 = _prof_begin()
@@ -502,18 +545,26 @@
                     ev.record(torch.cuda.current_stream())
                     side.wait_event(ev)
                     e0 = _prof_begin(side)
-                    call("danhip_conv2d_bwd_weight_ws", ctypes.byref(d), ptr(x), ptr(g), ptr(dw), ptr(db) if db_in_wgrad else None, ctx.cin_real,
-                         ptr(ws), nws, ctypes.c_void_p(side.cuda_stream))
-                    _prof_end(e0, d, 2, side)
+                    if pool_pair is not None:
+                        call("danhip_conv2d_bwd_weight_pooled", ctypes.byref(d), ptr(x), ptr(g), ptr(pool_pair[0]), ptr(dw), ptr(db) if db_in_wgrad else None,
+                             ctx.cin_real, ptr(ws), nws, ctypes.c_void_p(side.cuda_stream))
+                    else:
+                        call("danhip_conv2d_bwd_weight_ws", ctypes.byref(d), ptr(x), ptr(g), ptr(dw), ptr(db) if db_in_wgrad else None, ctx.cin_real,
+                             ptr(ws), nws, ctypes.c_void_p(side.cuda_stream))
+                    _prof_end(e0, d, 2, side, pooled_dy=pool_pair is not None)
                     if _CTX.GRAD_READY_HOOK is not None and wp is not None:
                         _CTX.GRAD_READY_HOOK(wp)
-                    _CTX.wgrad["keep"].append((g, x, ws))
+                    _CTX.wgrad["keep"].append((g, x, ws, pool_pair))
                     hooked = True
                 else:
                     e0 = _prof_begin()
-                    call("danhip_conv2d_bwd_weight_ws", ctypes.byref(d), ptr(x), ptr(g), ptr(dw), ptr(db) if db_in_wgrad else None, ctx.cin_real,
-                         ptr(ws), nws, stream())
-                    _prof_end(e0, d, 2)
+                    if pool_pair is not None:
+                        call("danhip_conv2d_bwd_weight_pooled", ctypes.byref(d), ptr(x), ptr(g), ptr(pool_pair[0]), ptr(dw), ptr(db) if db_in_wgrad else None,
+                             ctx.cin_real, ptr(ws), nws, stream())
+                    else:
+                        call("danhip_conv2d_bwd_weight_ws", ctypes.byref(d), ptr(x), ptr(g), ptr(dw), ptr(db) if db_in_wgrad else None, ctx.cin_real,
+                             ptr(ws), nws, stream())
+                    _prof_end(e0, d, 2, pooled_dy=pool_pair is not None)
                 if sink is not None:
                     dw = None
 
@@ -816,6 +867,10 @@
 
         if ctx.xslot is not None:
             xs = ctx.xslot
+            if (_CTX.USE_POOL_CODES and ctx.arg is not None and dy is None and xs.taps == TAP_POOL and xs.buf is None and xs.pending is None
+                    and tuple(xs.shape) == (N, H, W, C) and g.is_contiguous()):
+                xs.defer_first(TAP_POOL_CODES, scatter, (ctx.arg, g))
+                return None, None, None, None, None
             if ctx.arg is not None and _pool_deliver_ok(ctx, dy) and _junction_ok(xs, dy, C):
                 first = xs.pop_pending(TAP_L2NORM)
                 if first is not None:
diff --git a/include/danhip.h b/include/danhip.h
--- a/include/danhip.h
+++ b/include/danhip.h
@@ -82,6 +82,17 @@
                               int relu, int32_t relu_channels, const danhip_conv_pitch* pitch, void* ws, size_t ws_bytes, void* stream);
 int danhip_conv2d_bwd_data_strided(const danhip_conv_desc* d, const uint16_t* dy, const uint16_t* wb_packed, const uint16_t* relu_mask,
                                    uint16_t* dx, int accumulate, const danhip_conv_pitch* pitch, void* ws, size_t ws_bytes, void* stream);
+int danhip_conv2d_bwd_data_pooled_supported(const danhip_conv_desc* d, int first);
+int danhip_conv2d_bwd_weight_pooled_supported(const danhip_conv_desc* d);
+const char* danhip_conv_pooled_kernel_label(const danhip_conv_desc* d, int first);
+const char* danhip_conv_wgrad_pooled_kernel_label(const danhip_conv_desc* d);
+int danhip_conv2d_bwd_data_bits_pooled(const danhip_conv_desc* d, const uint16_t* pooled_dy, const uint8_t* pool_arg, const uint16_t* wb_packed,
+                                       const uint8_t* relu_bits, uint16_t* dx, int accumulate, void* stream);
+int danhip_conv2d_bwd_data_bits_first_pooled(const danhip_conv_desc* d, const uint16_t* pooled_dy, const uint8_t* pool_arg, const uint16_t* wb_packed,
+                                             const uint8_t* relu_bits, const uint16_t* x8, int32_t cin_real, float* dw8, float* db8, void* stream);
+int danhip_conv2d_bwd_weight_pooled(const danhip_conv_desc* d, const uint16_t* x, const uint16_t* pooled_dy, const uint8_t* pool_arg, float* dw_hwio,
+                                    float* db, int32_t cin_real, void* ws, size_t ws_bytes, void* stream);
+
 int danhip_conv2d_bwd_weight_strided(const danhip_conv_desc* d, const uint16_t* x, const uint16_t* dy, float* dw_hwio, float* db,
                                      int32_t cin_real, const danhip_conv_pitch* pitch, void* ws, size_t ws_bytes, void* stream);
 
```
